# iwbn/flow-supervisor

Hardware: AMD Instinct MI355X
Metric: image-pairs/s fwd+bwd, 12 GRU iters, 436x1024 (higher is better)
Workload: dtype f32 (bf16x3 products); 1 GPU; RAFT full, 440x1024 (Sintel 436x1024 padded), 12 GRU iters, 4 pairs/GPU, train step = fwd + sequence loss + bwd + RCCL all-reduce + clip + AdamW; global_batch=4, parallelism=dp1, launch=hipGraph replay of the whole step

## Files before the change

### flow_supervisor_amd/_lib.py

```python
import ctypes
import functools
import os
from ctypes import POINTER, Structure, c_double, c_float, c_int, c_int64, c_void_p

import torch

_HERE = os.path.dirname(os.path.abspath(__file__))
LIB_PATH = os.environ.get("FSRAFT_LIB_PATH") or os.path.join(_HERE, "libfsraft.so")
_lib = None

c_float_p = c_void_p


class ConvDesc(Structure):
    _fields_ = [
        ("src", c_void_p * 3), ("srcC", c_int * 3), ("srcld", c_int * 3), ("nsrc", c_int),
        ("wpk", c_void_p), ("bias", c_void_p), ("wpk_split", c_void_p),
        ("B", c_int), ("H", c_int), ("W", c_int), ("KH", c_int), ("KW", c_int), ("N", c_int),
        ("dst", c_void_p * 3), ("dst_bs", c_int64 * 3), ("dst_ps", c_int64 * 3), ("dst_cs", c_int64 * 3),
        ("dst_n0", c_int * 3), ("dst_acc", c_int * 3), ("ndst", c_int),
        ("relu", c_int), ("alpha", c_float),
        ("epi", c_int),
        ("h", c_void_p), ("ldh", c_int), ("z", c_void_p), ("ldz", c_int),
        ("aux1", c_void_p), ("ld1", c_int), ("aux2", c_void_p), ("ld2", c_int), ("hid", c_int),
        ("pre", c_void_p), ("ldpre", c_int),
        ("rmask", c_void_p * 3), ("ldmask", c_int * 3), ("maskc", c_int * 3),
        ("wpk_frag", c_void_p), ("pad_h1", c_int), ("pad_w1", c_int),
        ("ws", c_void_p), ("ws_floats", c_int64),
    ]


class PackJob(Structure):
    _fields_ = [
        ("w", c_void_p * 3), ("rows", c_int * 3), ("npiece", c_int),
        ("wpk", c_void_p),
        ("cin_full", c_int), ("kh", c_int), ("kw", c_int),
        ("srcC", c_int * 3), ("srcOff", c_int * 3), ("nsrc", c_int),
        ("mode", c_int), ("flags", c_int),
        ("scale", c_float), ("accumulate", c_int),
    ]


_PP = POINTER(c_void_p)
_IP = POINTER(c_int)
_S = c_void_p

SIGNATURES = {
    "fsraft_corr_build": [c_void_p, c_void_p, _PP, c_int, c_int, c_int, c_int, c_int, _S],
    "fsraft_corr_unpool_bwd": [_PP, c_int, c_int, c_int, c_int, _S],
    "fsraft_corr_lookup_fwd": [_PP, c_int, c_void_p, c_int64, c_int64, c_int64, c_void_p, c_int, c_int, c_int, c_int, c_int, _S],
    "fsraft_corr_lookup_bwd": [_PP, c_int, c_void_p, c_int64, c_int64, c_int64, c_void_p, c_int, c_int, c_int, c_int, c_int, _S],
    "fsraft_altcorr_fwd": [c_void_p, c_void_p, c_void_p, c_void_p, c_int, c_int, c_int, c_int, c_int, c_int, c_int, c_int, _S],
    "fsraft_altcorr_bwd": [c_void_p, c_void_p, c_void_p, c_void_p, c_void_p, c_void_p, c_int, c_int, c_int, c_int, c_int, c_int, c_int, c_int, _S],
    "fsraft_upsample_fwd": [c_void_p, c_int64, c_int64, c_int64, c_void_p, c_void_p, c_int, c_int, c_int, _S],
    "fsraft_upsample_bwd": [c_void_p, c_int64, c_int64, c_int64, c_void_p, c_void_p, c_void_p, c_void_p, c_void_p, c_int, c_int, c_int, _S],
    "fsraft_upflow8_fwd": [c_void_p, c_void_p, c_int, c_int, c_int, c_int, _S],
    "fsraft_upflow8_bwd": [c_void_p, c_void_p, c_int, c_int, c_int, c_int, _S],
    "fsraft_conv_ktot": [_IP, c_int, c_int, c_int],
    "fsraft_conv_forward": [POINTER(ConvDesc), _S],
    "fsraft_conv_forward_stats": [POINTER(ConvDesc), c_void_p, c_void_p, c_int, POINTER(c_int), _S],
    "fsraft_conv_wgrad": [c_void_p, c_int, c_int, _PP, _IP, _IP, c_int, c_void_p, c_void_p, c_int, c_int, c_int, c_int, c_int, _S],
    "fsraft_conv_wgrad_multi": [_PP, c_int, c_int, c_int, _PP, _IP, _IP, c_int, c_void_p, c_void_p, c_int, c_int, c_int, c_int, c_int, _S],
    "fsraft_conv_small_fwd": [c_void_p, c_int, c_int, c_void_p, c_void_p, c_void_p, c_int64, c_int64, c_int64, c_int, c_int, c_int, c_int, c_int, c_int, _S],
    "fsraft_conv_small_wgrad": [_PP, _PP, c_int, c_int, c_int, c_int, c_void_p, c_void_p, c_int, c_int, c_int, c_int, c_int, c_int, _S],
    "fsraft_conv_small_dgrad": [c_void_p, c_int, c_void_p, c_void_p, c_int, c_void_p, c_int, c_int, c_int, c_int, c_int, c_int, c_int, c_int, _S],
    "fsraft_pack_conv_weights": [POINTER(PackJob), c_int, _S],
    "fsraft_pack_conv_weight": [c_void_p, c_void_p, c_int, c_int, c_int, c_int, _IP, c_int, c_int, c_int, _S],
    "fsraft_set_rec_mfma16": [c_int],
    "fsraft_set_build_kernel": [c_int],
    "fsraft_set_dvol_policy": [c_int],
    "fsraft_set_dvol_box": [c_int],
    "fsraft_set_ktile_exact": [c_int],
    "fsraft_set_lookup_policy": [c_int],
    "fsraft_set_upsample_kernel": [c_int],
    "fsraft_conv_workspace": [c_void_p, c_int64],
    "fsraft_set_arithmetic": [c_int],
    "fsraft_get_arithmetic": [],
    "fsraft_set_tuning": [c_int, c_int],
    "fsraft_adamw_flat": [c_void_p, c_void_p, c_void_p, c_void_p, c_int64, c_void_p, c_void_p, c_float, c_void_p, c_double, c_double, c_float,
                          c_float, c_void_p, c_void_p, _S],
    "fsraft_stream_capture_id": [_S, c_void_p],
    "fsraft_stem_slots": [],
    "fsraft_stem7x7s2_fwd": [c_void_p, c_void_p, c_void_p, c_void_p, c_int, c_int, c_int, c_int, _S],
    "fsraft_stem7x7s2_wgrad": [c_void_p, c_void_p, c_void_p, c_void_p, c_int, c_int, c_int, c_int, _S],
    "fsraft_set_lookup_qb": [c_int],
    "fsraft_set_build_split": [c_int],
    "fsraft_set_gemm_split": [c_int],
    "fsraft_gemm_tn_split": [c_void_p, c_int64, c_int64, c_void_p, c_int64, c_int64, c_void_p, c_int64, c_int64, c_int, c_int, c_int, c_int, c_float, c_int, _S],
    "fsraft_gemm_f32": [c_void_p, c_int64, c_int64, c_void_p, c_int64, c_int64, c_void_p, c_int64, c_int64, c_int, c_int, c_int, c_int, c_int, c_float, c_int, _S],
    "fsraft_nchw_to_nhwc": [c_void_p, c_void_p, c_int, c_int, c_int, c_int, c_int, c_int, _S],
    "fsraft_nhwc_to_nchw": [c_void_p, c_void_p, c_int, c_int, c_int, c_int, c_int, c_int, _S],
    "fsraft_im2col7": [c_void_p, c_int64, c_int64, c_int64, c_void_p, c_int, c_int, c_int, c_int, _S],
    "fsraft_col2im7": [c_void_p, c_int, c_void_p, c_int, c_int, c_int, c_int, _S],
    "fsraft_flow_to_nhwc": [c_void_p, c_int64, c_int64, c_int64, c_void_p, c_int, c_int, c_int, c_int, _S],
    "fsraft_nhwc_to_flow": [c_void_p, c_int, c_int, c_void_p, c_int, c_int, c_int, _S],
    "fsraft_relu_bwd": [c_void_p, c_int, c_void_p, c_int, c_int64, c_int, _S],
    "fsraft_gru_bwd1": [c_void_p, c_void_p, c_void_p, c_void_p, c_void_p, c_void_p, c_int, c_void_p, c_void_p, c_void_p, c_void_p, c_int64, c_int, _S],
    "fsraft_gru_bwd2": [c_void_p, c_void_p, c_void_p, c_void_p, c_int, c_void_p, c_void_p, c_int64, c_int, _S],
    "fsraft_col_sum": [c_void_p, c_int, c_int64, c_int, c_void_p, c_float, _S],
    "fsraft_softmax_rows": [c_void_p, c_int64, c_int, _S],
    "fsraft_softmax_rows_bwd": [c_void_p, c_void_p, c_int64, c_int, _S],
    "fsraft_softmax_rows_rec": [c_void_p, c_int64, c_int, _S],
    "fsraft_softmax_rows_bwd_rec": [c_void_p, c_void_p, c_int64, c_int, _S],
    "fsraft_softmax_rows_pos": [c_void_p, c_void_p, c_int64, c_int64, c_int, c_int, c_int, c_int, c_int, _S],
    "fsraft_softmax_rows_pos_bwd": [c_void_p, c_void_p, c_void_p, c_int64, c_int64, c_int, c_int, c_int, c_int, _S],
    "fsraft_gma_mix_fwd": [c_void_p, c_int, c_void_p, c_int, c_void_p, c_void_p, c_int, c_int64, c_int, _S],
    "fsraft_gma_mix_bwd": [c_void_p, c_int, c_void_p, c_int, c_void_p, c_void_p, c_int, c_void_p, c_int, c_void_p, c_int64, c_int, _S],
    "fsraft_inorm_relu_fwd": [c_void_p, c_void_p, c_void_p, c_int64, c_int, c_float, c_int, _S],
    "fsraft_inorm_relu_bwd": [c_void_p, c_void_p, c_void_p, c_void_p, c_int64, c_int, c_int, _S],
    "fsraft_affine_relu_fwd": [c_void_p, c_void_p, c_void_p, c_void_p, c_int64, c_int, c_int, c_int, _S],
    "fsraft_affine_relu_bwd": [c_void_p, c_void_p, c_void_p, c_void_p, c_void_p, c_void_p, c_void_p, c_int64, c_int, c_int, c_int, _S],
    "fsraft_sequence_loss": [_PP, _PP, POINTER(c_float), c_int, c_int, c_void_p, c_void_p, c_float, c_float, c_int, c_int, c_int, c_void_p, _S],
    "fsraft_corr_pool_pyramid": [_PP, c_int, c_int64, c_int, c_int, _S],
    "fsraft_corr_pool_pyramid_same": [_PP, c_int, c_int64, c_int, c_int, _S],
    "fsraft_corr_lookup_fwd_same": [_PP, c_int, c_void_p, c_int64, c_int64, c_int64, c_void_p, c_int, c_int, c_int, c_int, c_int, _S],
    "fsraft_corr_unpool_same_bwd": [_PP, c_int, c_int64, c_int, c_int, _S],
    "fsraft_corr_lookup_bwd_same": [_PP, c_int, c_void_p, c_int64, c_int64, c_int64, c_void_p, c_int, c_int, c_int, c_int, c_int, _S],
    "fsraft_corr_lookup_dcoords_same": [_PP, c_int, c_void_p, c_int64, c_int64, c_int64, c_void_p, c_int, c_void_p, c_int64, c_int64, c_int64,
                                        c_int, c_int, c_int, c_int, _S],
    "fsraft_set_norm_blocks": [c_int],
    "fsraft_get_tuning": [c_int],
    "fsraft_conv_last_route": [c_int],
    "fsraft_set_wgrad_wide": [c_int],
    "fsraft_conv_wgrad_last_tile": [],
    "fsraft_space_to_depth2": [c_void_p, c_void_p, c_int, c_int, c_int, c_int, c_int, _S],
    "fsraft_forward_interpolate": [c_void_p, c_void_p, c_int, c_int, _S],
    "fsraft_flow_metrics_scratch_bytes": [c_int, c_int, c_int],
    "fsraft_flow_metrics": [c_void_p, c_int64, c_int64, c_int64, c_void_p, c_int64, c_int64, c_int64, c_void_p, c_int64, c_int64,
                            c_int, c_int, c_int, c_void_p, c_void_p, c_void_p, c_int64, _S],
    "fsraft_inorm_relu_cl_fwd": [c_void_p, c_void_p, c_void_p, c_void_p, c_void_p, c_void_p, c_int, c_int, c_int, c_float, c_int, c_int, c_int, _S],
    "fsraft_inorm_relu_cl_bwd": [c_void_p, c_void_p, c_void_p, c_void_p, c_void_p, c_void_p, c_void_p, c_void_p, c_int, c_int, c_int,
                                 c_int, c_int, _S],
    "fsraft_affine_relu_cl_fwd": [c_void_p, c_void_p, c_void_p, c_void_p, c_void_p, c_int64, c_int, c_int, c_int, c_int, _S],
    "fsraft_affine_relu_cl_bwd": [c_void_p, c_void_p, c_void_p, c_void_p, c_void_p, c_void_p, c_void_p, c_void_p, c_void_p, c_int, c_int,
                                  c_int, c_int, c_int, _S],
    "fsraft_axpby": [c_void_p, c_void_p, c_float, c_float, c_int64, _S],
    "fsraft_sum_n": [_PP, c_int, c_void_p, c_int64, c_int, _S],
    "fsraft_bn_fold": [c_void_p, c_void_p, c_void_p, c_void_p, c_void_p, c_float, c_int, c_void_p, c_void_p, c_void_p, c_void_p, _S],
    "fsraft_bn_fold_bwd": [c_void_p, c_int, c_int, c_void_p, c_void_p, c_void_p, c_void_p, c_void_p, c_void_p, _S],
    "fsraft_vol_layout": [c_int, c_int, c_int, _IP],
    "fsraft_corr_build_tiled": [c_void_p, c_void_p, c_void_p, c_int, c_int, c_int, c_int, c_int, _S],
    "fsraft_corr_build_rec": [c_void_p, c_void_p, c_void_p, c_int, c_int, c_int, c_int, c_int, _S],
    "fsraft_corr_lookup_tiled_fwd": [c_void_p, c_int, c_void_p, c_int64, c_int64, c_int64, c_void_p, c_int, c_int, c_int, c_int, c_int, _S],
    "fsraft_corr_lookup_tiled_dcoords": [c_void_p, c_int, c_void_p, c_int64, c_int64, c_int64, c_void_p, c_void_p, c_int64, c_int64, c_int64,
                                         c_int, c_int, c_int, c_int, c_int, _S],
    "fsraft_corr_lookup_dcoords": [_PP, c_int, c_void_p, c_int64, c_int64, c_int64, c_void_p, c_int, c_void_p, c_int64, c_int64, c_int64,
                                   c_int, c_int, c_int, c_int, _S],
    "fsraft_corr_dvol_build": [_PP, _PP, POINTER(c_int64), c_int, c_void_p, c_int, c_int, c_int, c_int, c_int, c_int, c_int, c_int, c_int64,
                               c_int64, c_void_p, c_void_p, _S],
    "fsraft_set_alt_tile": [c_int],
    "fsraft_altcorr_fused_fwd": [c_void_p, _PP, c_int, c_void_p, c_int64, c_int64, c_int64, c_int, c_void_p, c_int, c_int, c_int, c_int, c_int, _S],
    "fsraft_altcorr_fused_dcoords": [c_void_p, _PP, c_int, c_void_p, c_int64, c_int64, c_int64, c_int, c_void_p, c_void_p, c_int64, c_int64,
                                     c_int64, c_int, c_int, c_int, c_int, c_int, _S],
    "fsraft_altcorr_mfma_fwd": [c_void_p, _PP, c_void_p, _PP, c_int, c_void_p, c_int64, c_int64, c_int64, c_int, c_void_p, c_int, c_int, c_int, c_int, c_int, _S],
    "fsraft_corr_f2cat": [c_void_p, c_void_p, c_int, c_int, c_int, c_int, c_int, _S],
    "fsraft_corr_dfmap2": [c_void_p, c_void_p, c_int, c_int, c_int, c_int, c_int, _S],
    "fsraft_corr_f2cat_rec": [c_void_p, c_void_p, c_int, c_int, c_int, c_int, c_int, _S],
    "fsraft_to_records": [c_void_p, c_int64, c_void_p, c_int64, c_int64, c_int, _S],
    "fsraft_gemm_rec_tn": [c_void_p, c_int64, c_int64, c_void_p, c_int64, c_int64, c_void_p, c_int64, c_int64, c_int, c_int, c_int, c_int,
                           c_float, c_int, c_int, _S],
    "fsraft_gemm_rec_nt": [c_void_p, c_int64, c_int64, c_void_p, c_int64, c_int64, c_void_p, c_int64, c_int64, c_int, c_int, c_int, c_int,
                           c_float, c_int, c_int, _S],
    "fsraft_gemm_rec_nt_list": [c_void_p, c_int64, c_int64, c_void_p, c_int64, c_int64, c_void_p, c_int64, c_int64, c_int, c_int, c_int, c_int,
                                c_float, c_int, c_int, c_void_p, c_void_p, c_int, c_int, _S],
    "fsraft_gemm_rec_tn_list": [c_void_p, c_int64, c_int64, c_void_p, c_int64, c_int64, c_void_p, c_int64, c_int64, c_int, c_int, c_int, c_int,
                                c_float, c_int, c_int, c_void_p, c_void_p, c_int, c_int, _S],
    "fsraft_corr_bwd_ktiles": [_PP, POINTER(c_int64), c_int, c_int, c_int, c_int, c_int, c_int, c_int, c_int64, c_int64, c_void_p, c_void_p,
                               c_int, c_void_p, c_void_p, c_void_p, c_int, c_void_p, _S],
}

CONV_ROUTES = {
    1: ("fwd.gemm32", "fp32"), 2: ("fwd.gemm64", "fp32"), 3: ("fwd.gemm64x128", "fp32"), 4: ("fwd.gemm128", "fp32"),
    5: ("fwd.gemm64x64", "fp32"), 6: ("fwd.gemm64x64k16", "fp32"), 7: ("fwd.gemm64x128k16", "fp32"),
    10: ("fwd.patch128x128", "bf16x3"), 11: ("fwd.patch256x128", "bf16x3"), 12: ("fwd.patch128x64", "bf16x3"),
    13: ("fwd.patch256x64", "bf16x3"), 20: ("fwd.halo21", "bf16x3"), 21: ("fwd.halo22", "bf16x3"),
    30: ("fwd.split64x256", "bf16x3"), 31: ("fwd.split256x64", "bf16x3"), 32: ("fwd.split256x128w16", "bf16x3"),
    33: ("fwd.split128x128w8", "bf16x3"), 34: ("fwd.split64x128", "bf16x3"), 35: ("fwd.split128x128", "bf16x3"),
}
CONV_ROUTES.update({c + 100: (n + "+ksplit", a) for c, (n, a) in list(CONV_ROUTES.items()) if c >= 30})
WGRAD_ROUTES = {
    1: ("wgrad.exact32", "fp32"), 2: ("wgrad.exact64x64", "fp32"), 3: ("wgrad.exact128", "fp32"),
    4: ("wgrad.split128", "bf16x3"), 5: ("wgrad.split128S", "bf16x3"), 6: ("wgrad.pack", "bf16x3"),
    7: ("wgrad.patch", "bf16x3"), 8: ("wgrad.multi", "bf16x3"), 9: ("wgrad.multi_w8", "bf16x3"),
}


def load():
    global _lib
    if _lib is not None:
        return _lib
    if not os.path.exists(LIB_PATH):
        raise RuntimeError(
            f"{LIB_PATH} not found: build it with `python -c 'import __graft_entry__ as g; g.build()'` "
            "(or `make -C flow_supervisor_amd/csrc`). There is no CPU/eager fallback for the RAFT hot path.")
    lib = ctypes.CDLL(LIB_PATH)
    for name, argtypes in SIGNATURES.items():
        fn = getattr(lib, name)
        fn.argtypes = argtypes
        fn.restype = c_int
    _lib = lib
    arith = os.environ.get("FSRAFT_ARITHMETIC")
    if arith is not None:
        lib.fsraft_set_arithmetic(int(arith))
    split = os.environ.get("FSRAFT_CONV_SPLIT")
    if split is not None:
        lib.fsraft_set_tuning(3, int(split))
    bsplit = os.environ.get("FSRAFT_BUILD_SPLIT")
    if bsplit is not None:
        lib.fsraft_set_build_split(int(bsplit))
    for kv in filter(None, os.environ.get("FSRAFT_TUNING", "").split(",")):
        key, val = (int(v) for v in kv.split("="))
        if lib.fsraft_set_tuning(key, val) != 0:
            raise RuntimeError(f"FSRAFT_TUNING: key {key} is not a tuning key of this libfsraft (include/fsraft_tuning.h)")
    wsplit = os.environ.get("FSRAFT_WGRAD_SPLIT")
    if wsplit is not None:
        lib.fsraft_set_tuning(4, int(wsplit))
    return lib


def stream():
    return c_void_p(torch.cuda.current_stream().cuda_stream)


def check(rc, what):
    if rc != 0:
        raise RuntimeError(f"libfsraft: {what} failed with status {rc} "
                           f"({'bad argument' if rc == 1 else 'kernel launch error'})")


def ptr(t):
    return c_void_p(t.data_ptr()) if t is not None else c_void_p(0)


def ptr_array(tensors):
    arr = (c_void_p * len(tensors))(*[t.data_ptr() for t in tensors])
    return ctypes.cast(arr, _PP), arr


def int_array(vals):
    return (c_int * len(vals))(*vals)


def require_cuda_f32(*tensors):
    dev = None
    for t in tensors:
        if t is None:
            continue
        if not t.is_cuda:
            raise RuntimeError("fsraft ops need CUDA (ROCm) tensors; the hot path has no CPU implementation")
        if t.dtype != torch.float32:
            raise RuntimeError(f"fsraft ops are fp32-only, got {t.dtype}")
        if dev is None:
            dev = t.device
        elif t.device != dev:
            raise RuntimeError(f"fsraft ops need all tensors on one device, got {dev} and {t.device}")
    if dev is not None and dev.index != torch.cuda.current_device():
        raise RuntimeError(f"fsraft op called with tensors on {dev} while cuda:{torch.cuda.current_device()} is the current device; "
                           f"wrap the call in `with torch.cuda.device({dev.index}):`")


def _first_cuda_device(values):
    for v in values:
        if isinstance(v, torch.Tensor):
            if v.is_cuda:
                return v.device
        elif isinstance(v, (list, tuple)):
            d = _first_cuda_device(v)
            if d is not None:
                return d
    return None


def on_tensor_device(fn):
    @functools.wraps(fn)
    def guarded(*args, **kwargs):
        dev = _first_cuda_device(args)
        if dev is None and kwargs:
# ... 7 lines not shown
```

### flow_supervisor_amd/core/extractor.py

```python
import torch
import torch.nn as nn
import torch.nn.functional as F

from .. import ops
from .._lib import on_tensor_device


class _InstNormRelu(torch.autograd.Function):

    @staticmethod
    def forward(ctx, x, eps, relu):
        from .. import _lib as L
        x = x.contiguous()
        N, C, H, W = x.shape
        y = torch.empty_like(x)
        stats = torch.empty(N * C, 2, device=x.device, dtype=torch.float32)
        L.check(L.load().fsraft_inorm_relu_fwd(L.ptr(x), L.ptr(y), L.ptr(stats), N * C, H * W, float(eps), int(relu),
                                               L.stream()), "inorm_relu_fwd")
        ctx.save_for_backward(x, stats)
        ctx.relu = relu
        return y

    @staticmethod
    def backward(ctx, g):
# ... 81 lines not shown
    @staticmethod
    def backward(ctx, g):
        return _as_cl(g)


class _ResLink:
    __slots__ = ("dres", "armed")

    def __init__(self):
        self.dres = None
        self.armed = False


class _InstNormReluCL(torch.autograd.Function):

    @staticmethod
    def forward(ctx, x, eps, relu, res=None, link=None, sums=None, s2d=False):
        from .. import _lib as L
        ctx.in_cl = _is_cl(x)
        ctx.link = link
        x = _as_cl(x)
        N, C, H, W = x.shape
        if res is not None:
            res = _as_cl(res)
        ctx.s2w = W if s2d else 0
        y = (torch.empty(N, H // 2, W // 2, 4 * C, device=x.device, dtype=torch.float32).permute(0, 3, 1, 2) if s2d
             else torch.empty_like(x))
        have = sums is not None and sums.acc is not None and tuple(sums.acc.shape) == (2, N * 8, C)
        acc = sums.acc if have else ops.zeros(2, N * 8, C, device=x.device)
        stats = torch.empty(N, C, 2, device=x.device, dtype=torch.float32)
        L.check(L.load().fsraft_inorm_relu_cl_fwd(L.ptr(x), L.ptr(res), L.ptr(y), L.ptr(acc[0]), L.ptr(acc[1]), L.ptr(stats), N, H * W,
                                                  C, float(eps), int(relu), int(have), ctx.s2w, L.stream()), "inorm_relu_cl_fwd")
        ctx.fused = res is not None
        ctx.save_for_backward(x, stats, y if ctx.fused else None)
        ctx.relu = relu
        return y

    @staticmethod
    def backward(ctx, g):
        from .. import _lib as L
        x, stats, out = ctx.saved_tensors
        N, C, H, W = x.shape
        g = _as_cl(g)
        dx = torch.empty_like(x)
        dres = torch.empty_like(x) if ctx.fused else None
        acc = ops.zeros(2, N * 8, C, device=x.device)
        L.check(L.load().fsraft_inorm_relu_cl_bwd(L.ptr(g), L.ptr(x), L.ptr(stats), L.ptr(out), L.ptr(acc[0]), L.ptr(acc[1]), L.ptr(dx),
                                                  L.ptr(dres), N, H * W, C, int(ctx.relu), ctx.s2w, L.stream()), "inorm_relu_cl_bwd")
        if ctx.link is not None and ctx.link.armed:
            ctx.link.dres, dres = dres, None
        return dx if ctx.in_cl else _as_nchw(dx), None, None, dres, None, None, None


class _FrozenBNReluCL(torch.autograd.Function):

    @staticmethod
    def forward(ctx, x, cbias, weight, bias, rm, rv, eps, relu, res=None, link=None, s2d=False):
        from .. import _lib as L
        ctx.in_cl = _is_cl(x)
        ctx.link = link
        x = _as_cl(x)
        N, C, H, W = x.shape
        ctx.s2w = W if s2d else 0
        if res is not None:
            res = _as_cl(res)
        fold = torch.empty(4, C, device=x.device, dtype=torch.float32)
        scale, shift, rs, rmc = fold[0], fold[1], fold[2], fold[3]
        L.check(L.load().fsraft_bn_fold(L.ptr(weight.detach().float().contiguous()), L.ptr(bias.detach().float().contiguous()),
                                        L.ptr(rm.float().contiguous()), L.ptr(rv.float().contiguous()),
                                        L.ptr(cbias.detach().float().contiguous()) if cbias is not None else None, float(eps), C,
                                        L.ptr(scale), L.ptr(shift), L.ptr(rs), L.ptr(rmc), L.stream()), "bn_fold")
        y = torch.empty(N, H // 2, W // 2, 4 * C, device=x.device, dtype=torch.float32).permute(0, 3, 1, 2) if s2d else torch.empty_like(x)
        L.check(L.load().fsraft_affine_relu_cl_fwd(L.ptr(x), L.ptr(res), L.ptr(scale), L.ptr(shift), L.ptr(y), N * H * W, C, int(relu),
                                                   H * W, ctx.s2w, L.stream()), "affine_relu_cl_fwd")
        ctx.fused = res is not None
        ctx.save_for_backward(x, scale, shift, rs, rmc, y if ctx.fused else None)
        ctx.relu = relu
        ctx.has_cbias = cbias is not None
        return y

    @staticmethod
    def backward(ctx, g):
        from .. import _lib as L
        x, scale, shift, rs, rm, out = ctx.saved_tensors
        N, C, H, W = x.shape
        g = _as_cl(g)
        dx = torch.empty_like(x)
        dres = torch.empty_like(x) if ctx.fused else None
        part = ops.zeros(2, N * 8, C, device=x.device)
        L.check(L.load().fsraft_affine_relu_cl_bwd(L.ptr(g), L.ptr(x), L.ptr(scale), L.ptr(shift), L.ptr(out), L.ptr(dx), L.ptr(dres),
                                                   L.ptr(part[0]), L.ptr(part[1]), N, H * W, C, int(ctx.relu), ctx.s2w, L.stream()),
                "affine_relu_cl_bwd")
        dpar = torch.empty(3, C, device=x.device, dtype=torch.float32)
        L.check(L.load().fsraft_bn_fold_bwd(L.ptr(part), N * 8, C, L.ptr(rs), L.ptr(rm), L.ptr(scale), L.ptr(dpar[0]), L.ptr(dpar[1]),
                                            L.ptr(dpar[2]) if ctx.has_cbias else None, L.stream()), "bn_fold_bwd")
        if ctx.link is not None and ctx.link.armed:
            ctx.link.dres, dres = dres, None
        return (dx if ctx.in_cl else _as_nchw(dx), dpar[2] if ctx.has_cbias else None, dpar[0], dpar[1], None, None, None, None, dres,
                None, None)


def _conv_key(conv):
    from .. import ops
    w = conv.weight
    return (w.data_ptr(), w._version, ops.exact_mode())


def _queue_conv_packs(plan, conv):
    from .. import ops
    wd = conv.weight.detach()
    N, C, KH, KW = wd.shape
    exact = ops.exact_mode()
    fs = plan.pack([wd], [C], 10)
    f = plan.pack([wd], [C], 0) if (exact or N <= 32) else fs
    ds = plan.pack([wd], [C], 11)
    d = plan.pack([wd], [C], 1) if (exact or C <= 32) else ds
    ff = plan.pack([wd], [C], 10, frag=True) if (KH, KW) == (3, 3) and 32 < C <= 64 else None
    df = plan.pack([wd], [C], 11, frag=True) if (KH, KW) == (3, 3) and 32 < N <= 64 else None
    return (f, fs, d, ds, ff, df)


def _prepare_packs(root):
    from .. import ops
    todo = []
    for m in root.modules():
        if isinstance(m, _Block) and _pair_shape_ok(m):
            w3, wsc = m.conv1.weight, m.downsample[0].weight
            key = (w3.data_ptr(), w3._version, wsc.data_ptr(), wsc._version, ops.exact_mode())
            c = m.__dict__.get("_fs_pair_packs")
            if (c is None or c[0] != key) and w3.is_cuda and w3.dtype == torch.float32:
                todo.append(("pair", m, key))
        if (isinstance(m, nn.Conv2d) and m.stride == (1, 1) and m.kernel_size in ((1, 1), (3, 3)) and m.groups == 1
                and m.weight.is_cuda and m.weight.dtype == torch.float32):
            c = m.__dict__.get("_fs_packs")
            key = _conv_key(m)
            if c is None or c[0] != key:
                todo.append(("conv", m, key))
    if not todo:
        return
    with torch.no_grad():
        plan = ops.PackPlan(todo[0][1].conv1.weight.device if todo[0][0] == "pair" else todo[0][1].weight.device)
        hs = []
        exact = ops.exact_mode()
        for kind, m, key in todo:
            if kind == "conv":
                hs.append(_queue_conv_packs(plan, m))
                continue
            w3, ws = m.conv1.weight.detach(), m.downsample[0].weight.detach()
            N, C = w3.shape[:2]
            a = plan.pack([w3], [4 * C], 10, cin_full=C, s2d=True)
            b = plan.pack([w3], [4 * C], 11, cin_full=C, s2d=True)
            a0 = plan.pack([w3], [4 * C], 0, cin_full=C, s2d=True) if (exact or N <= 32) else a
            b0 = plan.pack([w3], [4 * C], 1, cin_full=C, s2d=True) if (exact or 4 * C <= 32) else b
            Ns, Cs = ws.shape[:2]
            c_ = plan.pack([ws], [Cs], 10)
            d_ = plan.pack([ws], [Cs], 11)
            c0 = plan.pack([ws], [Cs], 0) if (exact or Ns <= 32) else c_
            d0 = plan.pack([ws], [Cs], 1) if (exact or Cs <= 32) else d_
            hs.append(((a0, a, b0, b), (c0, c_, d0, d_)))
        out = plan.run()
        for (kind, m, key), h in zip(todo, hs):
            if kind == "conv":
                m.__dict__["_fs_packs"] = (key,) + tuple(None if i is None else out[i] for i in h)
            else:
                m.__dict__["_fs_pair_packs"] = (key, tuple(out[i] for i in h[0]), tuple(out[i] for i in h[1]))


def _weight_packs(conv):
    c = conv.__dict__.get("_fs_packs")
    if c is None or c[0] != _conv_key(conv):
        _prepare_packs(conv)
        c = conv.__dict__["_fs_packs"]
    return c


class _ConvCL(torch.autograd.Function):

    @staticmethod
    def forward(ctx, x, weight, bias, packs, link=None, sums=None):
        from .. import ops
        ctx.link = link if _is_cl(x) else None
        if ctx.link is not None:
            ctx.link.armed = True
        x = _as_cl(x)
        B, C, H, W = x.shape
        N, _, KH, KW = weight.shape
        out = torch.empty(B, H, W, N, device=x.device, dtype=torch.float32)
        acc = ops.zeros(2, B * 8, N, device=x.device) if (sums is not None and bias is None and STATS_IN_EPILOGUE) else None
        carried = ops.conv_forward([ops.V(x.permute(0, 2, 3, 1), C)], packs[1], bias, B, H, W, KH, KW, N, [ops.Dst.nhwc(out)],
                                   wpk_split=packs[2], wpk_frag=packs[5], stats=acc)
        if sums is not None:
            sums.acc = acc if carried else None
        ctx.save_for_backward(x, weight)
        ctx.packs = packs
        ctx.has_bias = bias is not None
        return out.permute(0, 3, 1, 2)

    @staticmethod
    def backward(ctx, g):
        from .. import ops
        x, weight = ctx.saved_tensors
        B, C, H, W = x.shape
        N, _, KH, KW = weight.shape
        g = _as_cl(g)
        gv = ops.V(g.permute(0, 2, 3, 1), N)
        dx = dw = db = None
        if ctx.needs_input_grad[0]:
            dres = ctx.link.dres if ctx.link is not None else None
            if dres is not None and dres.shape == x.shape and _is_cl(dres) and dres.dtype == torch.float32:
                ctx.link.dres = None
                ops.conv_forward([gv], ctx.packs[3], None, B, H, W, KH, KW, C, [ops.Dst.nhwc(dres.permute(0, 2, 3, 1), acc=True)],
                                 wpk_split=ctx.packs[4], wpk_frag=ctx.packs[6])
                dx = dres
            else:
                if dres is not None:
                    ctx.link.dres = None
                dxb = torch.empty(B, H, W, C, device=x.device, dtype=torch.float32)
                ops.conv_forward([gv], ctx.packs[3], None, B, H, W, KH, KW, C, [ops.Dst.nhwc(dxb)], wpk_split=ctx.packs[4],
                                 wpk_frag=ctx.packs[6])
                dx = dxb.permute(0, 3, 1, 2)
                if dres is not None:
                    dx = dx + dres
        elif ctx.link is not None:
            ctx.link.dres = None
        want_b = ctx.has_bias and ctx.needs_input_grad[2]
        if ctx.needs_input_grad[1] or want_b:
            dwpk = ops.zeros(N, ops.conv_ktot([C], KH, KW), device=x.device)
            db = ops.zeros(N, device=x.device) if want_b else None
            ops.conv_wgrad(gv, [ops.V(x.permute(0, 2, 3, 1), C)], dwpk, B, H, W, KH, KW, dbias=db)
            dw = ops.unpack_weight_grad(dwpk, tuple(weight.shape), [C])
        return dx, dw, db, None, None, None


class _StemFn(torch.autograd.Function):

    @staticmethod
    def forward(ctx, x, w):
        from .. import ops
        x = x.contiguous()
        ctx.save_for_backward(x)
        return ops.stem_fwd(x, w.detach()).permute(0, 3, 1, 2)

    @staticmethod
    def backward(ctx, g):
        from .. import ops
        (x,) = ctx.saved_tensors
        return None, ops.stem_wgrad(x, _as_cl(g).permute(0, 2, 3, 1))


def _stem_ok(conv, x):
    import os
    return (STEM_KERNEL and conv.kernel_size == (7, 7) and conv.stride == (2, 2) and conv.padding == (3, 3)
            and conv.dilation == (1, 1) and conv.groups == 1 and conv.padding_mode == "zeros" and conv.in_channels == 3
            and conv.out_channels in (32, 64) and _fast(x) and not x.requires_grad and not torch.is_autocast_enabled()
            and x.shape[2] >= 7 and x.shape[3] >= 7)


STATS_IN_EPILOGUE = True
STEM_KERNEL = True
S2D_UNITS = True


class _NormSums:
    __slots__ = ("acc",)

    def __init__(self):
        self.acc = None


def _conv(conv, x, bias, link=None, stem_cl=False, sums=None):
    k = conv.kernel_size
    if (_is_cl(x) and x.is_cuda and x.dtype == torch.float32 and k in ((3, 3), (1, 1)) and conv.stride == (1, 1)
            and conv.padding == (k[0] // 2, k[1] // 2) and conv.dilation == (1, 1) and conv.groups == 1
            and conv.padding_mode == "zeros" and x.shape[1] % 4 == 0 and not torch.is_autocast_enabled()):
        return _ConvCL.apply(x, conv.weight, bias, _weight_packs(conv), link, sums)
    if stem_cl and bias is None and _stem_ok(conv, x):
        return _StemFn.apply(x, conv.weight)
    return F.conv2d(_ToNCHW.apply(x) if _is_cl(x) else x, conv.weight, bias, conv.stride, conv.padding, conv.dilation, conv.groups)


_S2D_TAP = ((0, 1), (1, 0), (1, 1))


def _s2d_weight(w3):
    N, C = w3.shape[:2]
    w = w3.new_zeros(N, 2, 2, C, 2, 2)
    for ky, (ty, sy) in enumerate(_S2D_TAP):
        for kx, (tx, sx) in enumerate(_S2D_TAP):
            w[:, sy, sx, :, ty, tx] = w3[:, :, ky, kx]
    return w.reshape(N, 4 * C, 2, 2)


def _s2d_weight_grad(dw, C):
    N = dw.shape[0]
    d = dw.reshape(N, 2, 2, C, 2, 2)
    out = dw.new_empty(N, C, 3, 3)
    for ky, (ty, sy) in enumerate(_S2D_TAP):
        for kx, (tx, sx) in enumerate(_S2D_TAP):
            out[:, :, ky, kx] = d[:, sy, sx, :, ty, tx]
    return out


def _pair_shape_ok(block):
    c1 = getattr(block, "conv1", None)
    ds = block.downsample[0] if getattr(block, "downsample", None) is not None else None
    return (block.n == 2 and c1 is not None and ds is not None and c1.kernel_size == (3, 3) and c1.stride == (2, 2)
            and c1.padding == (1, 1) and c1.dilation == (1, 1) and c1.groups == 1 and ds.kernel_size == (1, 1)
            and ds.stride == (2, 2) and ds.padding == (0, 0) and ds.groups == 1)


def _pair_packs(block):
    from .. import ops
    w3, wsc = block.conv1.weight, block.downsample[0].weight
    key = (w3.data_ptr(), w3._version, wsc.data_ptr(), wsc._version, ops.exact_mode())
    c = block.__dict__.get("_fs_pair_packs")
    if c is None or c[0] != key:
        _prepare_packs(block)
        c = block.__dict__["_fs_pair_packs"]
    return c


class _StridedPairFn(torch.autograd.Function):

    @staticmethod
    def forward(ctx, x, w3, wsc, packs, pre=False):
        from .. import ops
        x = _as_cl(x)
        ctx.pre = pre
        if pre:
            B, C4, h, w = x.shape
            C, H, W = C4 // 4, 2 * h, 2 * w
            xs = x.permute(0, 2, 3, 1)
        else:
            B, C, H, W = x.shape
            h, w = H // 2, W // 2
            xs = ops.space_to_depth2(x.permute(0, 2, 3, 1))
        N, Ns = w3.shape[0], wsc.shape[0]
        y1 = torch.empty(B, h, w, N, device=x.device, dtype=torch.float32)
        ys = torch.empty(B, h, w, Ns, device=x.device, dtype=torch.float32)
        p, q = packs[1], packs[2]
        ops.conv_forward([ops.V(xs, 4 * C)], p[0], None, B, h, w, 2, 2, N, [ops.Dst.nhwc(y1)], wpk_split=p[1])
        ops.conv_forward([ops.V(xs, C, 0)], q[0], None, B, h, w, 1, 1, Ns, [ops.Dst.nhwc(ys)], wpk_split=q[1])
        ctx.save_for_backward(xs, w3, wsc)
        ctx.packs = packs
        return y1.permute(0, 3, 1, 2), ys.permute(0, 3, 1, 2)

    @staticmethod
    def backward(ctx, g1, gs):
        from .. import ops
        xs, w3, wsc = ctx.saved_tensors
        B, h, w, C4 = xs.shape
        C, N, Ns = C4 // 4, w3.shape[0], wsc.shape[0]
        p, q = ctx.packs[1], ctx.packs[2]
        g1v = ops.V(_as_cl(g1).permute(0, 2, 3, 1), N)
        gsv = ops.V(_as_cl(gs).permute(0, 2, 3, 1), Ns)
        dx = dw3 = dwsc = None
        if ctx.needs_input_grad[0]:
            dxs = torch.empty(B, h, w, C4, device=xs.device, dtype=torch.float32)
            ops.conv_forward([g1v], p[2], None, B, h, w, 2, 2, C4, [ops.Dst.nhwc(dxs)], wpk_split=p[3], pad=(0, 0))
            ops.conv_forward([gsv], q[2], None, B, h, w, 1, 1, C, [ops.Dst.nhwc(dxs, 0, 0, True)], wpk_split=q[3])
            dx = (dxs if ctx.pre else ops.space_to_depth2(dxs, inverse=True)).permute(0, 3, 1, 2)
        items = []
        if ctx.needs_input_grad[1]:
            dwpk = ops.zeros(N, ops.conv_ktot([C4], 2, 2), device=xs.device)
            ops.conv_wgrad(g1v, [ops.V(xs, C4)], dwpk, B, h, w, 2, 2)
            dw3 = torch.empty(N, C, 3, 3, device=xs.device, dtype=torch.float32)
            items.append((dwpk, [dw3], [C4], [0], C, 2, 2, 1.0, True))
        if ctx.needs_input_grad[2]:
            dwpk = ops.zeros(Ns, ops.conv_ktot([C], 1, 1), device=xs.device)
            ops.conv_wgrad(gsv, [ops.V(xs, C, 0)], dwpk, B, h, w, 1, 1)
            dwsc = torch.empty(Ns, C, 1, 1, device=xs.device, dtype=torch.float32)
            items.append((dwpk, [dwsc], [C], [0], C, 1, 1, 1.0, False))
        ops.unpack_weight_grads(items, xs.device)
        return dx, dw3, dwsc, None, None


def _norm_act(norm, y, cbias, relu, res=None):
    if isinstance(norm, nn.InstanceNorm2d):
        return _InstNormReluCL.apply(y, norm.eps, relu, res)
    return _FrozenBNReluCL.apply(y, cbias, norm.weight, norm.bias, norm.running_mean, norm.running_var, norm.eps, relu, res)


def _pair_ok_shape(block, C, H, W):
    import os
    return (S2D_UNITS and _pair_shape_ok(block) and H % 2 == 0
            and W % 2 == 0 and C % 4 == 0 and _cl_norm_ok(torch.empty(0, block.conv1.out_channels)))


def _pair_ok(block, x):
    return _pair_ok_shape(block, x.shape[1], x.shape[2], x.shape[3])


S2D_EMIT = True


class _S2D:
    __slots__ = ("t",)

    def __init__(self, t):
        self.t = t


def _conv_norm(conv, norm, x, relu, to_cl=False, res=None, link=None, res_link=None, s2d=False):
    fused = x.is_cuda and x.dtype == torch.float32 and not torch.is_autocast_enabled()
    if isinstance(norm, nn.InstanceNorm2d) and not norm.affine and not norm.track_running_stats:
        if fused:
            sums = _NormSums() if (to_cl or _is_cl(x)) else None
            y = _conv(conv, x, None, link, stem_cl=to_cl, sums=sums)
            if (to_cl or _is_cl(x)) and _cl_norm_ok(y):
                return _InstNormReluCL.apply(y, norm.eps, relu, res, res_link, sums, s2d)
            assert not s2d
            y = _InstNormRelu.apply(y, norm.eps, relu)
            return y if res is None else F.relu(res + y)
        y = F.conv2d(x, conv.weight, None, conv.stride, conv.padding, conv.dilation, conv.groups) if conv.bias is not None else conv(x)
        y = norm(y)
    elif isinstance(norm, nn.BatchNorm2d) and not norm.training and norm.track_running_stats and norm.affine and fused:
        y = _conv(conv, x, None, link, stem_cl=to_cl)
        if (to_cl or _is_cl(x)) and _cl_norm_ok(y):
            return _FrozenBNReluCL.apply(y, conv.bias, norm.weight, norm.bias, norm.running_mean, norm.running_var, norm.eps, relu, res,
                                         res_link, s2d)
        assert not s2d
        y = _FrozenBNRelu.apply(y, conv.bias, norm.weight, norm.bias, norm.running_mean, norm.running_var, norm.eps, relu)
        return y if res is None else F.relu(res + y)
    else:
        y = norm(conv(x))
    assert not s2d, "space-to-depth output is a feature of the fused channels_last norm kernels"
    y = F.relu(y, inplace=True) if relu else y
    return y if res is None else F.relu(res + y)


def _make_norm(kind, ch, groups):
    if kind == "group":
        return nn.GroupNorm(num_groups=groups, num_channels=ch)
    if kind == "batch":
        return nn.BatchNorm2d(ch)
    if kind == "instance":
        return nn.InstanceNorm2d(ch)
    if kind == "none":
        return nn.Sequential()
    raise ValueError(kind)


class _Block(nn.Module):

    def __init__(self, cin, cout, norm_fn, stride, bottleneck):
        super().__init__()
        mid = cout // 4
        if bottleneck:
            spec = [(cin, mid, 1, 1), (mid, mid, 3, stride), (mid, cout, 1, 1)]
        else:
            spec = [(cin, cout, 3, stride), (cout, cout, 3, 1)]
        groups = cout // 8
        self.n = len(spec)
        for i, (a, b, k, s) in enumerate(spec, 1):
            setattr(self, f"conv{i}", nn.Conv2d(a, b, kernel_size=k, padding=k // 2, stride=s))
        for i, (a, b, k, s) in enumerate(spec, 1):
            setattr(self, f"norm{i}", _make_norm(norm_fn, b, groups))
        self.relu = nn.ReLU(inplace=True)
        self.downsample = None
        if stride != 1:
            short = _make_norm(norm_fn, cout, groups)
            setattr(self, f"norm{self.n + 1}", short)
            self.downsample = nn.Sequential(nn.Conv2d(cin, cout, kernel_size=1, stride=stride), short)

    def forward(self, x, emit_for=None):
        if isinstance(x, _S2D):
            y1, ys = _StridedPairFn.apply(x.t, self.conv1.weight, self.downsample[0].weight, _pair_packs(self), True)
            y = _norm_act(self.norm1, y1, self.conv1.bias, True)
            xs = _norm_act(self.downsample[1], ys, self.downsample[0].bias, False)
            return _conv_norm(self.conv2, self.norm2, y, True, to_cl=True, res=xs)
        cl = _is_cl(x)
        if cl and self.downsample is not None and _pair_ok(self, x):
            y1, ys = _StridedPairFn.apply(x, self.conv1.weight, self.downsample[0].weight, _pair_packs(self))
            y = _norm_act(self.norm1, y1, self.conv1.bias, True)
            xs = _norm_act(self.downsample[1], ys, self.downsample[0].bias, False)
            return _conv_norm(self.conv2, self.norm2, y, True, to_cl=True, res=xs)
        if cl and self.downsample is not None:
            x = _ToNCHW.apply(x)
        y = x
        link = _ResLink() if (cl and self.downsample is None and self.n >= 2 and torch.is_grad_enabled() and x.requires_grad) else None
        if self.downsample is not None:
            x = _conv_norm(self.downsample[0], self.downsample[1], x, False, to_cl=cl)
        for i in range(1, self.n):
            y = _conv_norm(getattr(self, f"conv{i}"), getattr(self, f"norm{i}"), y, True, to_cl=cl, link=link if i == 1 else None)
        last = getattr(self, f"conv{self.n}")
        emit = bool(cl and S2D_EMIT and emit_for is not None and self.downsample is None and _is_cl(y) and _cl_norm_ok(torch.empty(0, last.out_channels))
                    and _pair_ok_shape(emit_for, last.out_channels, y.shape[2], y.shape[3])
                    and isinstance(getattr(self, f"norm{self.n}"), (nn.InstanceNorm2d, nn.BatchNorm2d)))
        out = _conv_norm(last, getattr(self, f"norm{self.n}"), y, True, to_cl=cl, res=x, res_link=link, s2d=emit)
        return _S2D(out) if emit else out


class ResidualBlock(_Block):
    def __init__(self, in_planes, planes, norm_fn="group", stride=1):
# ... 88 lines not shown
```

### flow_supervisor_amd/csrc/conv_common.hpp

```cpp
#pragma once
#include "gemm_core.hpp"
#include "gemm_core_split.hpp"
#include "gemm_rec.hpp"
#include <cstddef>
#include <type_traits>

struct ConvKnobs {
  int conv_tile = 0;
  int wgrad_tile = 0;
  int wgrad_blocks = 512;
  int conv_split = 1;
  int wgrad_split = 2;
  int conv_buf = 1;
  int xcd_swizzle = 0;
  int wgrad_buf = 1;
  int conv_n256 = 0;
  int wgrad_multi = 1;
  int wgrad_blocks_multi = 2048;
  int conv_uniform = 1;
  int conv_w8 = 1;
  int conv_w8_min = 64;
  int wgrad_w8 = 0;
  int wgrad_pack = 1;
  int wgrad_blocks_pack = 1024;
  int conv_n64 = 1;
  int conv_n64_min_m = 65536;
  int conv_halo = 1;
  int conv_halo_min_m = 65536;
  int wgrad_xcd = 1;
  int conv_patch = 1;
  int wgrad_patch = 1;
  int conv_patch64 = 1;
  int wgrad_patch1 = 8192;
  int conv_patch_min_m = 8192;
  int conv_ksplit = -1;
};
__attribute__((visibility("hidden"))) extern ConvKnobs knob;
__attribute__((visibility("hidden"))) extern __thread int t_route[2];

namespace {
struct Src { const float* p; int C; int ld; };
struct Dst { float* p; int64_t bs, ps, cs; int n0; int accumulate; };

struct ConvArgs {
  Src src[3]; int nsrc;
  const float* wpk; int Ktot;
  const float* bias;
  int B, H, W, KH, KW, N;
  int PH, PW;
  Dst dst[3]; int ndst;
  int relu; float alpha;
  const float* h; int ldh;
  const float* z; int ldz;
  float* aux1; int ld1;
  float* aux2; int ld2;
  int hid;
  const float* pre; int ldpre;
  const float* rmask[3]; int ldmask[3]; int maskc[3];
  float* st_sum; float* st_sq; int st_slots;
  int swz;
  int ksplit;
};

constexpr int KTAB_MAX = 512;
struct ConvArgsT {
  ConvArgs a;
  const float* ubase; int uld;
  unsigned ktab[KTAB_MAX];
};

enum { EPI_PLAIN = 0, EPI_ZR = 2, EPI_Q = 3 };

#define FS_RSRC_FLAGS 0x00020000
#define FS_OOB 0x80000000u

__device__ __forceinline__ unsigned uni(unsigned v) { return __builtin_amdgcn_readfirstlane(v); }
template <class T>
__device__ __forceinline__ const T* uni_ptr(const T* p) {
  const uint64_t u = reinterpret_cast<uint64_t>(p);
  return reinterpret_cast<const T*>((uint64_t)uni((unsigned)(u >> 32)) << 32 | uni((unsigned)u));
}
__device__ __forceinline__ __amdgpu_buffer_rsrc_t make_rsrc(const void* p, unsigned bytes) {
  const uint64_t u = reinterpret_cast<uint64_t>(p);
  const unsigned lo = __builtin_amdgcn_readfirstlane((unsigned)u), hi = __builtin_amdgcn_readfirstlane((unsigned)(u >> 32));
  void* q = reinterpret_cast<void*>((uint64_t)hi << 32 | lo);
  return __builtin_amdgcn_make_buffer_rsrc(q, 0, __builtin_amdgcn_readfirstlane(bytes), FS_RSRC_FLAGS);
}

using SWCfg128 = SplitTnCfg<128, 128, 2, 2, 2>;
using SWCfg128S = SplitTnCfg<128, 128, 2, 2, 1>;
using SWCfg128W8 = SplitTnCfg<128, 128, 2, 4, 1, 512>;
using SWCfgPack = SplitTnCfg<64, 192, 2, 2, 1>;
using SWCfgW256 = SplitTnCfg<256, 256, 2, 4, 2, 512>;
using SWCfgW128 = SplitTnCfg<128, 256, 2, 4, 2, 512>;
using Cfg128 = GemmCfg<128, 128, 32, 2, 2, 2, 2>;
using Cfg64 = GemmCfg<128, 64, 32, 4, 1, 2, 2>;
using CfgM64 = GemmCfg<64, 128, 32, 1, 4, 2, 2>;
using Cfg6464 = GemmCfg<64, 64, 32, 2, 2, 2, 2>;
using WCfg6464 = GemmCfg<64, 64, 32, 2, 2, 0, 0>;
using Cfg6464K16 = GemmCfg<64, 64, 16, 2, 2, 2, 2>;
using CfgM64K16 = GemmCfg<64, 128, 16, 1, 4, 2, 2>;

using SCfg128 = SplitCfg<128, 128, 2, 2>;
using SCfgN256 = SplitCfg<64, 256, 1, 4, 2, true>;
using SCfg256W16 = SplitCfg<256, 128, 4, 4, 2, true, 1024>;
using SCfg128W8 = SplitCfg<128, 128, 2, 4, 2, true, 512>;
using SCfg256N64 = SplitCfg<256, 64, 4, 2, 2, true, 512>;
using SCfgM64 = SplitCfg<64, 128, 1, 4, 2, true>;
using Cfg32 = GemmCfg<128, 32, 32, 4, 1, 2, 2>;
using WCfg128 = GemmCfg<128, 128, 32, 2, 2, 0, 0>;
using WCfg32 = GemmCfg<32, 128, 32, 1, 4, 0, 0>;

template <class Cfg>
constexpr int route_gemm() {
  return std::is_same_v<Cfg, Cfg32> ? 1 : std::is_same_v<Cfg, Cfg64> ? 2 : std::is_same_v<Cfg, CfgM64> ? 3 :
         std::is_same_v<Cfg, Cfg128> ? 4 : std::is_same_v<Cfg, Cfg6464> ? 5 : std::is_same_v<Cfg, Cfg6464K16> ? 6 :
         std::is_same_v<Cfg, CfgM64K16> ? 7 : 0;
}
template <class Cfg>
constexpr int route_split() {
  return std::is_same_v<Cfg, SCfgN256> ? 30 : std::is_same_v<Cfg, SCfg256N64> ? 31 : std::is_same_v<Cfg, SCfg256W16> ? 32 :
         std::is_same_v<Cfg, SCfg128W8> ? 33 : std::is_same_v<Cfg, SCfgM64> ? 34 : std::is_same_v<Cfg, SCfg128> ? 35 : 0;
}

int conv_ktot(const int* C, int nsrc, int taps) {
  int k = 0;
  for (int s = 0; s < nsrc; ++s) k += taps * (((C[s] + 31) / 32) * 32);
  return k;
}

template <class F>
void with_epi(int epi, F&& f) {
  if (epi == EPI_PLAIN) f(std::integral_constant<int, EPI_PLAIN>{});
  else if (epi == EPI_ZR) f(std::integral_constant<int, EPI_ZR>{});
  else f(std::integral_constant<int, EPI_Q>{});
}

bool fill_srcs(Src (&dst)[3], const float* const* p, const int* C, const int* ld, int nsrc) {
  for (int s = 0; s < 3; ++s) {
    dst[s] = Src{s < nsrc ? p[s] : p[0], s < nsrc ? C[s] : 0, s < nsrc ? ld[s] : 4};
    if (s < nsrc && (!p[s] || ld[s] % 4 != 0)) return false;
  }
  return true;
}

int64_t wgrad_chunk(int target, int64_t tiles, int64_t M, int words) {
  int64_t want = (target + tiles - 1) / tiles;
  if (want < 1) want = 1;
  int64_t chunk = (M + want - 1) / want;
  if (chunk < 256) chunk = 256;
  if (chunk > 32 * (words - 2)) chunk = 32 * (words - 2);
  return (chunk + 31) / 32 * 32;
}

}
```

### flow_supervisor_amd/csrc/conv_igemm.hip

```cpp
#include "conv_common.hpp"

namespace {

__device__ __forceinline__ void tile_of_block(int swz, int& bx, int& by) {
  if (!swz) return;
  const int nx = gridDim.x, T = nx * gridDim.y, i = by * nx + bx;
  const int x = i & 7, q = T >> 3, r = T & 7;
  const int t = x * q + (x < r ? x : r) + (i >> 3);
  bx = t % nx; by = t / nx;
}

template <class Cfg>
struct ConvALoader {
  static constexpr int BM = Cfg::BM, BK = Cfg::BK, LD = Cfg::LDA;
  static constexpr int F4 = BK / 4;
  static constexpr int NF4 = BM * F4 / 256;
  static constexpr int NREG = NF4 * 4;
  static constexpr int NCH = NF4;
  const float* p0; const float* p1; const float* p2;
  int C0, C1, C2, ld0, ld1, ld2;
  int cpt0, cpt1, cpt2;
  int taps, KW, PH, PW, H, W;
  int py[NF4], px[NF4];
  int64_t pb[NF4];
// ... 138 lines not shown
  int64_t row_bytes;
  int rows_valid;
  __device__ __forceinline__ void fetch_chunk(int kt, float (&r)[NREG], int j) const {
    const int e = threadIdx.x + 256 * j;
    const int row = e >> 3, part = e & 7;
    const char* src = (row < rows_valid && kt >= 0) ? base + row * row_bytes + (int64_t)kt * 128 + part * 16
                                                    : reinterpret_cast<const char*>(g_fsraft_zero16);
    const f32x4 v = gload4(src);
    r[4 * j + 0] = v[0]; r[4 * j + 1] = v[1]; r[4 * j + 2] = v[2]; r[4 * j + 3] = v[3];
  }
  __device__ __forceinline__ void stage_chunk(char* tile, const float* r4, int j) const {
    stage_copy<Cfg::PITCH>(tile, threadIdx.x + 256 * j, r4);
  }
};

template <class Cfg, int EPI>
__device__ __forceinline__ void conv_epilogue(const ConvArgs& a, f32x16 (&acc)[Cfg::TM][Cfg::TN], int m0, int n0) {
  const int HW = a.H * a.W;
  const int M = a.B * HW;
  const int lane = threadIdx.x & 63, wave = threadIdx.x >> 6;
#pragma unroll
  for (int nt = 0; nt < Cfg::TN; ++nt) {
    const int n = n0 + acc_col<Cfg>(nt);
    const bool nok = n < a.N;
    const float bias = (nok && a.bias) ? a.bias[n] : 0.f;
    int di = 0;
    if (a.ndst > 1 && n >= a.dst[1].n0) di = 1;
    if (a.ndst > 2 && n >= a.dst[2].n0) di = 2;
    float* dp = di == 0 ? a.dst[0].p : di == 1 ? a.dst[1].p : a.dst[2].p;
    const int64_t dbs = di == 0 ? a.dst[0].bs : di == 1 ? a.dst[1].bs : a.dst[2].bs;
    const int64_t dps = di == 0 ? a.dst[0].ps : di == 1 ? a.dst[1].ps : a.dst[2].ps;
    const int64_t dcs = di == 0 ? a.dst[0].cs : di == 1 ? a.dst[1].cs : a.dst[2].cs;
    const int dn0 = di == 0 ? a.dst[0].n0 : di == 1 ? a.dst[1].n0 : a.dst[2].n0;
    const bool dacc = (di == 0 ? a.dst[0].accumulate : di == 1 ? a.dst[1].accumulate : a.dst[2].accumulate) != 0;
    const float* mk = di == 0 ? a.rmask[0] : di == 1 ? a.rmask[1] : a.rmask[2];
    const int ldm = di == 0 ? a.ldmask[0] : di == 1 ? a.ldmask[1] : a.ldmask[2];
    const int mkc = di == 0 ? a.maskc[0] : di == 1 ? a.maskc[1] : a.maskc[2];
#pragma unroll
    for (int mt = 0; mt < Cfg::TM; ++mt) {
      const int mbase = m0 + (wave / Cfg::WN) * (Cfg::TM * 32) + mt * 32 + 4 * (lane >> 5);
      const int b0 = mbase / HW, pix0 = mbase - b0 * HW;
      if (EPI == EPI_PLAIN) {
#pragma unroll
        for (int hb = 0; hb < 2; ++hb) {
          int off[8];
#pragma unroll
          for (int q = 0; q < 8; ++q) {
            const int r = hb * 8 + q;
            const int d = (r & 3) + 8 * (r >> 2);
            int pix = pix0 + d, b = b0;
            if (pix >= HW) { pix -= HW; ++b; }
            const bool ok = nok && (mbase + d < M);
            off[q] = ok ? (int)(b * dbs + pix * dps + (n - dn0) * dcs) : -1;
          }
          float old[8];
#pragma unroll
          for (int q = 0; q < 8; ++q) old[q] = (dacc && off[q] >= 0) ? dp[off[q]] : 0.f;
#pragma unroll
          for (int q = 0; q < 8; ++q) {
            float v = (acc[mt][nt][hb * 8 + q] + bias) * a.alpha;
            if (a.relu) v = fmaxf(v, 0.f);
            v += old[q];
            if (off[q] >= 0 && mk && n - dn0 < mkc) {
              const int r = hb * 8 + q;
              const int64_t m = mbase + (r & 3) + 8 * (r >> 2);
              if (mk[m * ldm + (n - dn0)] <= 0.f) v = 0.f;
            }
            if (off[q] >= 0) dp[off[q]] = v;
          }
        }
      } else if (EPI == EPI_ZR) {
        const bool isz = n < a.hid;
        const int c = isz ? n : n - a.hid;
        float hh[16];
        bool ok[16];
#pragma unroll
        for (int r = 0; r < 16; ++r) {
          const int m = mbase + (r & 3) + 8 * (r >> 2);
          ok[r] = nok && m < M;
          hh[r] = (ok[r] && !isz) ? a.h[(int64_t)m * a.ldh + c] : 0.f;
        }
#pragma unroll
        for (int r = 0; r < 16; ++r) {
          const int64_t m = mbase + (r & 3) + 8 * (r >> 2);
          const float pre = (a.pre && ok[r]) ? a.pre[m * a.ldpre + n] : 0.f;
          const float sg = 1.0f / (1.0f + expf(-(acc[mt][nt][r] + bias + pre)));
          if (ok[r]) {
            if (isz) {
              a.dst[0].p[m * a.dst[0].ps + c] = sg;
            } else {
              a.aux2[m * a.ld2 + c] = sg;
              a.aux1[m * a.ld1 + c] = sg * hh[r];
            }
          }
        }
      } else {
        float hh[16], zz[16];
        bool ok[16];
#pragma unroll
        for (int r = 0; r < 16; ++r) {
          const int64_t m = mbase + (r & 3) + 8 * (r >> 2);
          ok[r] = nok && m < M;
          hh[r] = ok[r] ? a.h[m * a.ldh + n] : 0.f;
          zz[r] = ok[r] ? a.z[m * a.ldz + n] : 0.f;
        }
#pragma unroll
        for (int r = 0; r < 16; ++r) {
          const int64_t m = mbase + (r & 3) + 8 * (r >> 2);
          const float pre = (a.pre && ok[r]) ? a.pre[m * a.ldpre + n] : 0.f;
          const float q = tanhf(acc[mt][nt][r] + bias + pre);
          if (ok[r]) {
            a.aux1[m * a.ld1 + n] = q;
            a.dst[0].p[m * a.dst[0].ps + n] = (1.f - zz[r]) * hh[r] + zz[r] * q;
          }
        }
      }
    }
  }
}

template <class Cfg, int EPI, int NTW = Cfg::NT, bool PATCH = false>
__device__ __forceinline__ void conv_epilogue_lds(const ConvArgs& a, f32x16 (&acc)[Cfg::TM][Cfg::TN], int m0, int n0,
                                                  float* __restrict__ tile, bool owner = true, int pb = 0, int py0 = 0, int px0 = 0,
                                                  int64_t mofs = 0) {
  constexpr int LD = Cfg::BN + 4;
  const int HW = a.H * a.W;
  const int M = a.B * HW;
  const int lane = threadIdx.x & 63, wave = threadIdx.x >> 6;
  auto row_m = [&](int row) -> int64_t {
    if constexpr (PATCH) {
      const int y = py0 + (row >> 5), x = px0 + (row & 31);
      return (y < a.H && x < a.W) ? (int64_t)(pb * a.H + y) * a.W + x : -1;
    } else {
      return m0 + row < M ? (int64_t)m0 + row : -1;
    }
  };
  __syncthreads();
#pragma unroll
  for (int nt = 0; nt < Cfg::TN; ++nt) {
    const int nl = acc_col<Cfg>(nt);
    const float bias = (n0 + nl < a.N && a.bias) ? a.bias[n0 + nl] : 0.f;
#pragma unroll
    for (int mt = 0; mt < Cfg::TM; ++mt) {
      const int rbase = (wave / Cfg::WN) * (Cfg::TM * 32) + mt * 32 + 4 * (lane >> 5);
#pragma unroll
      for (int r = 0; r < 16; ++r) tile[(rbase + (r & 3) + 8 * (r >> 2)) * LD + nl] = acc[mt][nt][r] + bias;
    }
  }
  __syncthreads();
  constexpr int C4 = Cfg::BN / 4;
  constexpr int RPP = NTW / C4;
  (void)owner;
  const int c4 = threadIdx.x % C4, rsub = threadIdx.x / C4;
  const int n = n0 + c4 * 4;
  const bool stats = PATCH && EPI == EPI_PLAIN && a.st_sum != nullptr;
  if (n >= a.N && !stats) return;
  if (EPI == EPI_PLAIN) {
    f32x4 ssum = {0.f, 0.f, 0.f, 0.f}, ssq = {0.f, 0.f, 0.f, 0.f};
    if (n < a.N) {
    int di = 0;
    if (a.ndst > 1 && n >= a.dst[1].n0) di = 1;
    if (a.ndst > 2 && n >= a.dst[2].n0) di = 2;
    float* dp = di == 0 ? a.dst[0].p : di == 1 ? a.dst[1].p : a.dst[2].p;
    const int64_t dps = di == 0 ? a.dst[0].ps : di == 1 ? a.dst[1].ps : a.dst[2].ps;
    const int dn0 = di == 0 ? a.dst[0].n0 : di == 1 ? a.dst[1].n0 : a.dst[2].n0;
    const bool dacc = (di == 0 ? a.dst[0].accumulate : di == 1 ? a.dst[1].accumulate : a.dst[2].accumulate) != 0;
    const float* mk = di == 0 ? a.rmask[0] : di == 1 ? a.rmask[1] : a.rmask[2];
    const int ldm = di == 0 ? a.ldmask[0] : di == 1 ? a.ldmask[1] : a.ldmask[2];
    const int mkc = di == 0 ? a.maskc[0] : di == 1 ? a.maskc[1] : a.maskc[2];
    const int nv = a.N - n < 4 ? a.N - n : 4;
#pragma unroll 4
    for (int row = rsub; row < Cfg::BM; row += RPP) {
      const int64_t m = row_m(row);
      if (m < 0) { if (PATCH) continue; else break; }
      f32x4 v = *reinterpret_cast<const f32x4*>(tile + row * LD + c4 * 4);
      float* o = dp + (int64_t)(m + mofs) * dps + (n - dn0);
#pragma unroll
      for (int i = 0; i < 4; ++i) {
        v[i] *= a.alpha;
        if (a.relu) v[i] = fmaxf(v[i], 0.f);
      }
      if (nv == 4) {
        if (stats) { ssum += v; ssq += v * v; }
        if (dacc) {
          const f32x4 old = gload4(o);
#pragma unroll
          for (int i = 0; i < 4; ++i) v[i] += old[i];
        }
        if (mk) {
          const f32x4 y = gload4(mk + (int64_t)m * ldm + (n - dn0));
#pragma unroll
          for (int i = 0; i < 4; ++i) if (n - dn0 + i < mkc && y[i] <= 0.f) v[i] = 0.f;
        }
        gstore4(o, v);
      } else {
        for (int i = 0; i < nv; ++i) {
          float r = dacc ? gload1(o + i) + v[i] : v[i];
          if (mk && n - dn0 + i < mkc && gload1(mk + (int64_t)m * ldm + (n - dn0) + i) <= 0.f) r = 0.f;
          gstore1(o + i, r);
        }
      }
    }
    }
    if constexpr (PATCH) {
      if (stats) {
        __syncthreads();
        float* red = tile;
        *reinterpret_cast<f32x4*>(red + (rsub * Cfg::BN) + c4 * 4) = ssum;
        *reinterpret_cast<f32x4*>(red + ((RPP + rsub) * Cfg::BN) + c4 * 4) = ssq;
        __syncthreads();
        if (threadIdx.x < Cfg::BN && n0 + (int)threadIdx.x < a.N) {
          float t1 = 0.f, t2 = 0.f;
#pragma unroll 4
          for (int g = 0; g < RPP; ++g) { t1 += red[g * Cfg::BN + threadIdx.x]; t2 += red[(RPP + g) * Cfg::BN + threadIdx.x]; }
          const int64_t o = ((int64_t)pb * a.st_slots + (int)(blockIdx.y % (unsigned)a.st_slots)) * a.N + n0 + threadIdx.x;
          atomicAdd(a.st_sum + o, t1);
          atomicAdd(a.st_sq + o, t2);
        }
      }
    }
  } else if (EPI == EPI_ZR) {
    const bool isz = n < a.hid;
    const int c = isz ? n : n - a.hid;
#pragma unroll 4
    for (int row = rsub; row < Cfg::BM; row += RPP) {
      const int64_t mr = row_m(row);
      if (mr < 0 && !PATCH) break;
      const int64_t m = mr < 0 ? 0 : mr;
      f32x4 v = *reinterpret_cast<const f32x4*>(tile + row * LD + c4 * 4);
      if (a.pre) v += gload4(a.pre + m * a.ldpre + n);
      f32x4 hh = {0.f, 0.f, 0.f, 0.f};
      if (!isz) hh = gload4(a.h + m * a.ldh + c);
#pragma unroll
      for (int i = 0; i < 4; ++i) v[i] = 1.0f / (1.0f + expf(-v[i]));
      if (mr < 0) continue;
      if (isz) {
        *reinterpret_cast<f32x4*>(a.dst[0].p + m * a.dst[0].ps + c) = v;
      } else {
        *reinterpret_cast<f32x4*>(a.aux2 + m * a.ld2 + c) = v;
        f32x4 rh;
#pragma unroll
        for (int i = 0; i < 4; ++i) rh[i] = v[i] * hh[i];
        *reinterpret_cast<f32x4*>(a.aux1 + m * a.ld1 + c) = rh;
      }
    }
  } else {
#pragma unroll 4
    for (int row = rsub; row < Cfg::BM; row += RPP) {
      const int64_t m = row_m(row);
      if (m < 0) { if (PATCH) continue; else break; }
      f32x4 v = *reinterpret_cast<const f32x4*>(tile + row * LD + c4 * 4);
      if (a.pre) v += gload4(a.pre + m * a.ldpre + n);
      const f32x4 hh = gload4(a.h + m * a.ldh + n);
      const f32x4 zz = gload4(a.z + m * a.ldz + n);
      f32x4 hn;
#pragma unroll
      for (int i = 0; i < 4; ++i) {
        v[i] = tanhf(v[i]);
        hn[i] = (1.f - zz[i]) * hh[i] + zz[i] * v[i];
      }
      *reinterpret_cast<f32x4*>(a.aux1 + m * a.ld1 + n) = v;
      *reinterpret_cast<f32x4*>(a.dst[0].p + m * a.dst[0].ps + n) = hn;
    }
  }
}

__device__ __forceinline__ bool epilogue_rows_ok(const ConvArgs& a) {
  bool ok = true;
  for (int i = 0; i < a.ndst; ++i)
    ok = ok && a.dst[i].cs == 1 && (a.dst[i].ps & 3) == 0 && (a.dst[i].n0 & 3) == 0 && ((uintptr_t)a.dst[i].p & 15) == 0 &&
         a.dst[i].bs == a.dst[i].ps * (int64_t)(a.H * a.W);
  return ok;
}

bool epilogue_rows_ok_host(const ConvArgs& a) {
  bool ok = true;
  for (int i = 0; i < a.ndst; ++i)
    ok = ok && a.dst[i].cs == 1 && (a.dst[i].ps & 3) == 0 && (a.dst[i].n0 & 3) == 0 && ((uintptr_t)a.dst[i].p & 15) == 0 &&
         a.dst[i].bs == a.dst[i].ps * (int64_t)(a.H * a.W);
  return ok;
}

template <class Cfg, int EPI>
__global__ __launch_bounds__(256) void conv_igemm_kernel(ConvArgs a) {
  __shared__ __attribute__((aligned(16))) float lds[Cfg::LDS_FLOATS];
  const int HW = a.H * a.W;
  const int M = a.B * HW;
  const int n0 = blockIdx.x * Cfg::BN, m0 = blockIdx.y * Cfg::BM;
  ConvALoader<Cfg> la;
  la.p0 = a.src[0].p; la.C0 = a.src[0].C; la.ld0 = a.src[0].ld; la.cpt0 = (a.src[0].C + 31) / 32 * (32 / Cfg::BK);
  la.p1 = a.src[1].p; la.C1 = a.src[1].C; la.ld1 = a.src[1].ld; la.cpt1 = a.nsrc > 1 ? (a.src[1].C + 31) / 32 * (32 / Cfg::BK) : 0;
  la.p2 = a.src[2].p; la.C2 = a.src[2].C; la.ld2 = a.src[2].ld; la.cpt2 = a.nsrc > 2 ? (a.src[2].C + 31) / 32 * (32 / Cfg::BK) : 0;
  if (a.nsrc < 2) { la.p1 = a.src[0].p; la.C1 = 0; la.ld1 = 4; la.cpt1 = 1; }
  if (a.nsrc < 3) { la.p2 = a.src[0].p; la.C2 = 0; la.ld2 = 4; la.cpt2 = 1; }
  la.taps = a.KH * a.KW; la.KW = a.KW; la.PH = a.PH; la.PW = a.PW; la.H = a.H; la.W = a.W;
#pragma unroll
  for (int j = 0; j < ConvALoader<Cfg>::NF4; ++j) {
    const int row = (threadIdx.x + 256 * j) / ConvALoader<Cfg>::F4;
    const int m = m0 + row;
    if (m < M) {
      const int b = m / HW, pix = m % HW;
      la.py[j] = pix / a.W; la.px[j] = pix % a.W; la.pb[j] = (int64_t)b * HW;
    } else {
      la.py[j] = -1; la.px[j] = 0; la.pb[j] = 0;
    }
  }
  RowMajorTileLoader<Cfg::BN, Cfg::BK, Cfg::LDB> lb{a.wpk + (int64_t)n0 * a.Ktot, a.Ktot, a.N - n0, a.Ktot};
  f32x16 acc[Cfg::TM][Cfg::TN];
#pragma unroll
  for (int i = 0; i < Cfg::TM; ++i)
#pragma unroll
    for (int j = 0; j < Cfg::TN; ++j)
#pragma unroll
      for (int r = 0; r < 16; ++r) acc[i][j][r] = 0.f;
  gemm_mainloop<Cfg>(lds, a.Ktot / Cfg::BK, la, lb, acc);
  conv_epilogue<Cfg, EPI>(a, acc, m0, n0);
}

template <class Cfg, int EPI, int BUF = 0>
__global__ __launch_bounds__(Cfg::NT) void conv_igemm_split_kernel(const std::conditional_t<BUF != 0, ConvArgsT, ConvArgs> args) {
  static_assert(Cfg::NT == 256 || BUF != 0, "wider workgroups use the buffer-addressed loaders");
  __shared__ __attribute__((aligned(16))) char lds[Cfg::LDS_ALLOC];
  const ConvArgs& a = [&]() -> const ConvArgs& { if constexpr (BUF != 0) return args.a; else return args; }();
  const int HW = a.H * a.W;
  const int M = a.B * HW;
  int bx = blockIdx.x, by = blockIdx.y;
  tile_of_block(a.swz, bx, by);
  const int n0 = bx * Cfg::BN, m0 = by * Cfg::BM;
  f32x16 acc[Cfg::TM][Cfg::TN];
#pragma unroll
  for (int i = 0; i < Cfg::TM; ++i)
#pragma unroll
    for (int j = 0; j < Cfg::TN; ++j)
#pragma unroll
      for (int r = 0; r < 16; ++r) acc[i][j][r] = 0.f;
  if constexpr (BUF != 0) {
    const int PH = a.PH, PW = a.PW, taps = a.KH * a.KW;
    const auto* ktab = (const unsigned __attribute__((address_space(4)))*)(
        (const char __attribute__((address_space(4)))*)__builtin_amdgcn_kernarg_segment_ptr() + offsetof(ConvArgsT, ktab));
    int kt0 = 0, KTs = a.Ktot / 32;
    if (a.ksplit > 1) {
      const int per = (KTs + a.ksplit - 1) / a.ksplit;
      kt0 = (int)blockIdx.z * per;
      KTs = min(per, KTs - kt0);
      ktab += kt0 * (BUF >= 2 ? 2 : 1);
    }
    unsigned tapmask[Cfg::NCH_A], pofs[Cfg::NCH_A];
#pragma unroll
    for (int j = 0; j < Cfg::NCH_A; ++j) {
      const int m = m0 + ((threadIdx.x + Cfg::NT * j) >> 3);
      unsigned mask = 0;
      if (m < M) {
        const int pix = m % HW, y = pix / a.W, x = pix % a.W;
        for (int t = 0; t < taps; ++t) {
          const int yy = y + t / a.KW - PH, xx = x + t % a.KW - PW;
          if ((unsigned)yy < (unsigned)a.H && (unsigned)xx < (unsigned)a.W) mask |= 1u << t;
        }
      }
      tapmask[j] = mask; pofs[j] = m < M ? m : 0;
    }
    BufWeightLoader<Cfg> lb;
    lb.base = uni_ptr(reinterpret_cast<const char*>(a.wpk) + (int64_t)n0 * a.Ktot * 4 + (int64_t)kt0 * 128);
    lb.nbytes = 0x7fffffffu;
#pragma unroll
    for (int j = 0; j < BufWeightLoader<Cfg>::NCH; ++j) {
      const int e = threadIdx.x + Cfg::NT * j;
      lb.voff[j] = (e >> 3) < a.N - n0 ? (unsigned)((e >> 3) * a.Ktot * 4 + (e & 7) * 16) : FS_OOB;
    }
    if constexpr (BUF >= 2) {
      BufConvALoaderU<Cfg> la;
      la.base = uni_ptr(args.ubase); la.ktab = ktab; la.kq16 = (threadIdx.x & 7) * 16;
      const unsigned ldb = uni((unsigned)args.uld * 4u);
#pragma unroll
      for (int j = 0; j < Cfg::NCH_A; ++j) { la.tapmask[j] = tapmask[j]; la.voff0[j] = pofs[j] * ldb + la.kq16; }
      split_mainloop<Cfg, BufConvALoaderU<Cfg>, BufWeightLoader<Cfg>, true>(lds, KTs, la, lb, acc);
    } else {
      BufConvALoader<Cfg> la;
      la.ld0x4 = uni(a.src[0].ld * 4); la.ld1x4 = uni(a.src[1].ld * 4); la.ld2x4 = uni(a.src[2].ld * 4);
      la.b0 = uni_ptr(a.src[0].p - (int64_t)(PH * a.W + PW) * a.src[0].ld); la.nb0 = 0x7fffffffu;
      la.b1 = uni_ptr(a.src[1].p - (int64_t)(PH * a.W + PW) * a.src[1].ld); la.nb1 = 0x7fffffffu;
      la.b2 = uni_ptr(a.src[2].p - (int64_t)(PH * a.W + PW) * a.src[2].ld); la.nb2 = 0x7fffffffu;
      la.ktab = ktab;
      la.kq16 = (threadIdx.x & 7) * 16;
#pragma unroll
      for (int j = 0; j < Cfg::NCH_A; ++j) { la.tapmask[j] = tapmask[j]; la.pofs[j] = pofs[j]; }
      split_mainloop<Cfg, BufConvALoader<Cfg>, BufWeightLoader<Cfg>, true>(lds, KTs, la, lb, acc);
    }
    if constexpr (EPI == EPI_PLAIN && Cfg::LDS_ALLOC >= Cfg::BM * (Cfg::BN + 4) * 4) {
      if (a.ksplit > 1) {
        conv_epilogue_lds<Cfg, EPI_PLAIN>(a, acc, m0, n0, reinterpret_cast<float*>(lds), true, 0, 0, 0, (int64_t)blockIdx.z * M);
        return;
      }
    }
  } else {
  SplitConvALoader<Cfg> la;
  la.p0 = a.src[0].p; la.C0 = a.src[0].C; la.ld0 = a.src[0].ld; la.cpt0 = (a.src[0].C + 31) / 32;
  la.p1 = a.src[1].p; la.C1 = a.src[1].C; la.ld1 = a.src[1].ld; la.cpt1 = a.nsrc > 1 ? (a.src[1].C + 31) / 32 : 0;
  la.p2 = a.src[2].p; la.C2 = a.src[2].C; la.ld2 = a.src[2].ld; la.cpt2 = a.nsrc > 2 ? (a.src[2].C + 31) / 32 : 0;
  if (a.nsrc < 2) { la.p1 = a.src[0].p; la.C1 = 0; la.ld1 = 4; la.cpt1 = 1; }
  if (a.nsrc < 3) { la.p2 = a.src[0].p; la.C2 = 0; la.ld2 = 4; la.cpt2 = 1; }
  la.taps = a.KH * a.KW; la.KW = a.KW; la.PH = a.PH; la.PW = a.PW; la.H = a.H; la.W = a.W;
// ... 46 lines not shown
    const int ku = __builtin_amdgcn_readfirstlane(kt < KT ? kt : KT - 1);
    const __amdgpu_buffer_rsrc_t rs = make_rsrc(wbase, 0x7fffffffu);
#pragma unroll
    for (int nt = 0; nt < TN; ++nt) {
      const int nb = wn * TN + nt;
      const unsigned soff = (unsigned)((ku * NB + (nb < NB ? nb : 0)) * 4096);
      const unsigned voff = nb < NB ? (unsigned)lane * 16u : FS_OOB;
#pragma unroll
      for (int q = 0; q < 4; ++q) f.v[nt][q] = __builtin_amdgcn_raw_buffer_load_b128(rs, voff, soff + 1024u * q, 0);
    }
  };
  BFrag f[4];
  fetch_b(0, f[0]);
  fetch_b(1, f[1]);
  fetch_b(2, f[2]);

  {
    const float* img = uni_ptr(a.x + (int64_t)b * a.H * a.W * a.ldx);
    const __amdgpu_buffer_rsrc_t rs = make_rsrc(img, 0x7fffffffu);
    float rh[NCHH * 4];
#pragma unroll
    for (int j = 0; j < NCHH; ++j) {
      const int e = threadIdx.x + 256 * j;
      const int row = e / (CG * 8), rem = e % (CG * 8), ch = (rem >> 3) * 32 + (rem & 7) * 4;
      const int y = y0 - 1 + row / HALO_PW, x = x0 - 1 + row % HALO_PW;
      const bool ok = row < HALO_ROWS && (unsigned)y < (unsigned)a.H && (unsigned)x < (unsigned)a.W && ch < a.C;
      const unsigned voff = ok ? (unsigned)((y * a.W + x) * a.ldx + ch) * 4u : FS_OOB;
      const f32x4 f = __builtin_bit_cast(f32x4, __builtin_amdgcn_raw_buffer_load_b128(rs, voff, 0, 0));
      rh[4 * j + 0] = f[0]; rh[4 * j + 1] = f[1]; rh[4 * j + 2] = f[2]; rh[4 * j + 3] = f[3];
    }
#pragma unroll
    for (int j = 0; j < NCHH; ++j) {
      const int e = threadIdx.x + 256 * j;
      const int row = e / (CG * 8), rem = e % (CG * 8);
      if (row < HALO_ROWS) stage_convert<128>(lds + (rem >> 3) * PLANE, row * 8 + (rem & 7), rh + 4 * j);
    }
  }
  __syncthreads();

  f32x16 acc[2][TN];
#pragma unroll
  for (int i = 0; i < 2; ++i)
#pragma unroll
    for (int j = 0; j < TN; ++j)
#pragma unroll
      for (int r = 0; r < 16; ++r) acc[i][j][r] = 0.f;

  auto compute = [&](int kt, const BFrag& f) {
    const int ku = __builtin_amdgcn_readfirstlane(kt);
    const int tap = ku / CG, g = ku - tap * CG, dy = tap / 3, dx = tap - dy * 3;
    const char* Ap = lds + g * PLANE;
    const int rowa = (2 * wm + dy) * HALO_PW + dx + l31;
#pragma unroll
    for (int s = 0; s < 2; ++s) {
      bf16x8 ah[2], al[2];
#pragma unroll
      for (int mt = 0; mt < 2; ++mt) {
        const int row = rowa + mt * HALO_PW;
        ah[mt] = *reinterpret_cast<const bf16x8*>(Ap + slot_offset<128>(row, 2 * s + lh));
        al[mt] = *reinterpret_cast<const bf16x8*>(Ap + slot_offset<128>(row, 4 + 2 * s + lh));
      }
#pragma unroll
      for (int mt = 0; mt < 2; ++mt)
#pragma unroll
        for (int nt = 0; nt < TN; ++nt) {
          const bf16x8 bh = __builtin_bit_cast(bf16x8, f.v[nt][s]), bl = __builtin_bit_cast(bf16x8, f.v[nt][2 + s]);
          acc[mt][nt] = __builtin_amdgcn_mfma_f32_32x32x16_bf16(al[mt], bh, acc[mt][nt], 0, 0, 0);
          acc[mt][nt] = __builtin_amdgcn_mfma_f32_32x32x16_bf16(ah[mt], bl, acc[mt][nt], 0, 0, 0);
          acc[mt][nt] = __builtin_amdgcn_mfma_f32_32x32x16_bf16(ah[mt], bh, acc[mt][nt], 0, 0, 0);
        }
    }
  };
  for (int kt = 0; kt < KT; kt += 4) {
#pragma unroll
    for (int i = 0; i < 4; ++i)
      if (kt + i < KT) {
        fetch_b(kt + i + 3, f[(i + 3) & 3]);
        compute(kt + i, f[i]);
      }
  }

  if (a.st_sum) {
    __syncthreads();
    float* red = reinterpret_cast<float*>(lds);
#pragma unroll
    for (int nt = 0; nt < TN; ++nt) {
      float s1 = 0.f, s2 = 0.f;
#pragma unroll
      for (int mt = 0; mt < 2; ++mt) {
        const int py = y0 + 2 * wm + mt;
#pragma unroll
        for (int r = 0; r < 16; ++r) {
          const int px = x0 + (r & 3) + 8 * (r >> 2) + 4 * lh;
          const float v = (py < a.H && px < a.W) ? acc[mt][nt][r] : 0.f;
          s1 += v; s2 += v * v;
        }
      }
      s1 += __shfl_xor(s1, 32, 64); s2 += __shfl_xor(s2, 32, 64);
      const int col = wn * (32 * TN) + nt * 32 + l31;
      if (lh == 0) { red[(wm * 2 + 0) * (64 * TN) + col] = s1; red[(wm * 2 + 1) * (64 * TN) + col] = s2; }
    }
    __syncthreads();
    if ((int)threadIdx.x < 64 * TN && (int)threadIdx.x < a.N) {
      const int col = threadIdx.x;
      const int slot = (int)((blockIdx.y * gridDim.x + blockIdx.x) % (unsigned)a.st_slots);
      const int64_t o = ((int64_t)b * a.st_slots + slot) * a.N + col;
      atomicAdd(a.st_sum + o, red[col] + red[2 * (64 * TN) + col]);
      atomicAdd(a.st_sq + o, red[(64 * TN) + col] + red[3 * (64 * TN) + col]);
    }
  }
  float* outb = a.out + (int64_t)b * a.obs;
#pragma unroll
  for (int mt = 0; mt < 2; ++mt) {
    const int py = y0 + 2 * wm + mt;
    if (py >= a.H) continue;
#pragma unroll
    for (int nt = 0; nt < TN; ++nt) {
      const int n = wn * (32 * TN) + nt * 32 + l31;
      if (n >= a.N) continue;
      const float bv = a.bias ? a.bias[n] : 0.f;
      float old[16];
#pragma unroll
      for (int r = 0; r < 16; ++r) {
        const int px = x0 + (r & 3) + 8 * (r >> 2) + 4 * lh, pc = px < a.W ? px : a.W - 1;
        old[r] = a.acc ? outb[(int64_t)(py * a.W + pc) * a.ops + n] : 0.f;
      }
#pragma unroll
      for (int r = 0; r < 16; ++r) {
        const int px = x0 + (r & 3) + 8 * (r >> 2) + 4 * lh;
        if (px >= a.W) continue;
        float v = acc[mt][nt][r] + bv;
        if (a.relu) v = fmaxf(v, 0.f);
        outb[(int64_t)(py * a.W + px) * a.ops + n] = v + old[r];
      }
    }
  }
}

template <int CG, int TN>
int launch_halo(const HaloArgs& h, hipStream_t s) {
  dim3 grid(ceil_div(h.W, HALO_TW), ceil_div(h.H, HALO_TH), h.B);
  hipLaunchKernelGGL((conv3x3_halo_kernel<CG, TN>), grid, dim3(256), 0, s, h);
  return fs_launch_status();
}

bool build_ktab(const ConvArgs& a, ConvArgsT& t) {
  const int taps = a.KH * a.KW, KT = a.Ktot / 32;
  const int64_t M = (int64_t)a.B * a.H * a.W;
  if (KT > KTAB_MAX || taps > 15) return false;
  int kt = 0;
  for (int s = 0; s < a.nsrc; ++s) {
    const int C = a.src[s].C, ld = a.src[s].ld, cpt = (C + 31) / 32;
    if (M * ld * 4 >= (int64_t)FS_OOB) return false;
    for (int i = 0; i < taps * cpt; ++i, ++kt) {
        const int tap = i / cpt, c = i % cpt;
        const int64_t soff = ((int64_t)((tap / a.KW) * a.W + tap % a.KW) * ld + c * 32) * 4;
        if (soff % 16 != 0 || soff / 16 > 0xffff) return false;
        const int crem = C - c * 32 < 32 ? C - c * 32 : 32;
        t.ktab[kt] = (unsigned)(soff / 16) | (unsigned)tap << 16 | (unsigned)s << 20 | (unsigned)crem << 22;
      }
  }
  if (kt != KT) return false;
  t.a = a;
  return true;
}

bool build_ktab_uniform(const ConvArgs& a, ConvArgsT& t) {
  const int taps = a.KH * a.KW, KT = a.Ktot / 32, PH = a.PH, PW = a.PW;
  const int64_t M = (int64_t)a.B * a.H * a.W;
  if (!knob.conv_uniform || 2 * KT > KTAB_MAX || taps > 15) return false;
  const int ld = a.src[0].ld;
  const float* lo = a.src[0].p;
  for (int s = 0; s < a.nsrc; ++s) {
    if (a.src[s].ld != ld) return false;
    if (a.src[s].p < lo) lo = a.src[s].p;
  }
  const float* base = lo - (int64_t)(PH * a.W + PW) * ld;
  int kt = 0;
  for (int s = 0; s < a.nsrc; ++s) {
    const int C = a.src[s].C, cpt = (C + 31) / 32;
    const int64_t delta = (a.src[s].p - lo) * 4;
    for (int tap = 0; tap < taps; ++tap)
      for (int c = 0; c < cpt; ++c, ++kt) {
        const int64_t soff = delta + ((int64_t)((tap / a.KW) * a.W + tap % a.KW) * ld + c * 32) * 4;
        if (soff + M * ld * 4 + 256 >= (int64_t)FS_OOB) return false;
        const int crem = C - c * 32 < 32 ? C - c * 32 : 32;
        t.ktab[2 * kt] = (unsigned)soff;
        t.ktab[2 * kt + 1] = (unsigned)tap | (unsigned)crem << 4;
      }
  }
  if (kt != KT) return false;
  t.a = a; t.ubase = base; t.uld = ld;
  return true;
}


template <int EPI>
__global__ __launch_bounds__(256) void conv_finish_kernel(const ConvArgs a, const float* __restrict__ ws, int S, int ldw) {
  const int HW = a.H * a.W;
  const int64_t M = (int64_t)a.B * HW;
  const int C4 = (a.N + 3) / 4;
  for (int64_t e = (int64_t)blockIdx.x * 256 + threadIdx.x; e < M * C4; e += (int64_t)gridDim.x * 256) {
    const int64_t m = e / C4;
    const int n = (int)(e % C4) * 4;
    const int nv = a.N - n < 4 ? a.N - n : 4;
    f32x4 v = {0.f, 0.f, 0.f, 0.f};
    if (a.bias) {
#pragma unroll
      for (int i = 0; i < 4; ++i) v[i] = i < nv ? a.bias[n + i] : 0.f;
    }
    for (int s = 0; s < S; ++s) {
      const f32x4 p = gload4(ws + ((int64_t)s * M + m) * ldw + n);
#pragma unroll
      for (int i = 0; i < 4; ++i) v[i] += p[i];
    }
    if (EPI == EPI_PLAIN) {
      int di = 0;
      if (a.ndst > 1 && n >= a.dst[1].n0) di = 1;
      if (a.ndst > 2 && n >= a.dst[2].n0) di = 2;
      float* dp = di == 0 ? a.dst[0].p : di == 1 ? a.dst[1].p : a.dst[2].p;
      const int64_t dbs = di == 0 ? a.dst[0].bs : di == 1 ? a.dst[1].bs : a.dst[2].bs;
      const int64_t dps = di == 0 ? a.dst[0].ps : di == 1 ? a.dst[1].ps : a.dst[2].ps;
      const int64_t dcs = di == 0 ? a.dst[0].cs : di == 1 ? a.dst[1].cs : a.dst[2].cs;
      const int dn0 = di == 0 ? a.dst[0].n0 : di == 1 ? a.dst[1].n0 : a.dst[2].n0;
      const bool dacc = (di == 0 ? a.dst[0].accumulate : di == 1 ? a.dst[1].accumulate : a.dst[2].accumulate) != 0;
      const float* mk = di == 0 ? a.rmask[0] : di == 1 ? a.rmask[1] : a.rmask[2];
      const int ldm = di == 0 ? a.ldmask[0] : di == 1 ? a.ldmask[1] : a.ldmask[2];
      const int mkc = di == 0 ? a.maskc[0] : di == 1 ? a.maskc[1] : a.maskc[2];
      const int64_t b = m / HW, pix = m - b * HW;
      float* o = dp + b * dbs + pix * dps + (int64_t)(n - dn0) * dcs;
      for (int i = 0; i < nv; ++i) {
        float r = v[i] * a.alpha;
        if (a.relu) r = fmaxf(r, 0.f);
        if (dacc) r += o[i * dcs];
        if (mk && n - dn0 + i < mkc && mk[m * ldm + (n - dn0) + i] <= 0.f) r = 0.f;
        o[i * dcs] = r;
      }
    } else if (EPI == EPI_ZR) {
      const bool isz = n < a.hid;
      const int c = isz ? n : n - a.hid;
      if (a.pre) v += gload4(a.pre + m * a.ldpre + n);
#pragma unroll
      for (int i = 0; i < 4; ++i) v[i] = 1.0f / (1.0f + expf(-v[i]));
      if (isz) {
        *reinterpret_cast<f32x4*>(a.dst[0].p + m * a.dst[0].ps + c) = v;
      } else {
        const f32x4 hh = gload4(a.h + m * a.ldh + c);
        *reinterpret_cast<f32x4*>(a.aux2 + m * a.ld2 + c) = v;
        f32x4 rh;
#pragma unroll
        for (int i = 0; i < 4; ++i) rh[i] = v[i] * hh[i];
        *reinterpret_cast<f32x4*>(a.aux1 + m * a.ld1 + c) = rh;
      }
    } else {
      if (a.pre) v += gload4(a.pre + m * a.ldpre + n);
      const f32x4 hh = gload4(a.h + m * a.ldh + n);
      const f32x4 zz = gload4(a.z + m * a.ldz + n);
      f32x4 hn;
#pragma unroll
      for (int i = 0; i < 4; ++i) {
        v[i] = tanhf(v[i]);
        hn[i] = (1.f - zz[i]) * hh[i] + zz[i] * v[i];
      }
      *reinterpret_cast<f32x4*>(a.aux1 + m * a.ld1 + n) = v;
      *reinterpret_cast<f32x4*>(a.dst[0].p + m * a.dst[0].ps + n) = hn;
    }
  }
}

thread_local float* t_reg_ws = nullptr;
thread_local int64_t t_reg_ws_floats = 0;
thread_local float* g_conv_ws = nullptr;
thread_local int64_t g_conv_ws_floats = 0;

int pick_ksplit(int64_t tiles, int KT, int N, int64_t M, int ldw, int bm) {
  int S = 1;
  if (knob.conv_ksplit >= 2) S = knob.conv_ksplit;
  else if (knob.conv_ksplit == -1 && bm == 64 && tiles <= 150 && N <= 256 && KT >= 16) S = (int)((400 + tiles - 1) / tiles);
  else if (knob.conv_ksplit == -1 && bm == 128 && tiles <= 120 && N <= 256 && KT >= (N <= 128 ? 36 : 48)) S = tiles <= 115 ? (int)(230 / tiles) : 2;
  if (S > KT / 6) S = KT / 6;
  if (S > 6) S = 6;
  while (S > 1 && (int64_t)S * M * ldw > g_conv_ws_floats) --S;
  if (S > 1) {
    const int per = (KT + S - 1) / S;
    S = (KT + per - 1) / per;
  }
  return S < 2 ? 1 : S;
}

template <class Cfg>
int launch_conv_split(const ConvArgs& a, int epi, hipStream_t s) {
  const int M = a.B * a.H * a.W;
  dim3 grid(ceil_div(a.N, Cfg::BN), ceil_div(M, Cfg::BM));
  ConvArgsT t;
  const int swz = knob.xcd_swizzle || (grid.x >= 2 && (int64_t)grid.x * grid.y >= 2048);
  const bool buf = knob.conv_buf == 2 || (knob.conv_buf == 1 && Cfg::BM == 64) || Cfg::BN == 256 || Cfg::NT != 256;
  if constexpr (Cfg::LDS_ALLOC >= Cfg::BM * (Cfg::BN + 4) * 4) {
    const int ldw = (a.N + 3) / 4 * 4;
    const bool gru_ok = epi == EPI_PLAIN || (a.N % 4 == 0 && (!a.pre || a.ldpre % 4 == 0));
    const int S = (buf && g_conv_ws && gru_ok && (Cfg::BM == 64 || (Cfg::BM == 128 && Cfg::NT == 512) || knob.conv_ksplit >= 2)) ? pick_ksplit((int64_t)grid.x * grid.y, a.Ktot / 32, a.N, M, ldw, Cfg::BM) : 1;
    if (S > 1) {
      const bool uni_tab = build_ktab_uniform(a, t);
      if (uni_tab || build_ktab(a, t)) {
        ConvArgs& p = t.a;
        p.swz = 0;
        p.ksplit = S;
        p.dst[0] = Dst{g_conv_ws, (int64_t)a.H * a.W * ldw, ldw, 1, 0, 0};
        p.dst[1] = p.dst[2] = p.dst[0];
        p.ndst = 1; p.bias = nullptr; p.relu = 0; p.alpha = 1.0f;
        for (int i = 0; i < 3; ++i) p.rmask[i] = nullptr;
        dim3 g3(grid.x, grid.y, S);
        t_route[0] = route_split<Cfg>() + 100;
        if (uni_tab) hipLaunchKernelGGL((conv_igemm_split_kernel<Cfg, EPI_PLAIN, 2>), g3, dim3(Cfg::NT), 0, s, t);
        else hipLaunchKernelGGL((conv_igemm_split_kernel<Cfg, EPI_PLAIN, 1>), g3, dim3(Cfg::NT), 0, s, t);
        int rc = fs_launch_status();
        if (rc) return rc;
        const int64_t work = (int64_t)M * (ldw / 4);
        const int fb = (int)((work + 255) / 256 < 4096 ? (work + 255) / 256 : 4096);
        with_epi(epi, [&](auto e) { hipLaunchKernelGGL(conv_finish_kernel<decltype(e)::value>, dim3(fb), dim3(256), 0, s, a, g_conv_ws, S, ldw); });
        return fs_launch_status();
      }
    }
  }
  if (buf && build_ktab_uniform(a, t)) {
    t.a.swz = swz;
    t_route[0] = route_split<Cfg>();
    with_epi(epi, [&](auto e) { hipLaunchKernelGGL((conv_igemm_split_kernel<Cfg, decltype(e)::value, 2>), grid, dim3(Cfg::NT), 0, s, t); });
    return fs_launch_status();
  }
  if (buf && build_ktab(a, t)) {
    t.a.swz = swz;
    t_route[0] = route_split<Cfg>();
    with_epi(epi, [&](auto e) { hipLaunchKernelGGL((conv_igemm_split_kernel<Cfg, decltype(e)::value, 1>), grid, dim3(Cfg::NT), 0, s, t); });
    return fs_launch_status();
  }
  if constexpr (Cfg::NT != 256) {
    return -1;
  } else {
  t_route[0] = route_split<Cfg>();
  with_epi(epi, [&](auto e) { hipLaunchKernelGGL((conv_igemm_split_kernel<Cfg, decltype(e)::value>), grid, dim3(256), 0, s, a); });
  return fs_launch_status();
  }
}

template <class Cfg>
int launch_conv_split_plain(const ConvArgs& a, hipStream_t s) {
  const int M = a.B * a.H * a.W;
  dim3 grid(ceil_div(a.N, Cfg::BN), ceil_div(M, Cfg::BM));
  ConvArgsT t;
  if (build_ktab_uniform(a, t)) {
    t_route[0] = route_split<Cfg>();
    hipLaunchKernelGGL((conv_igemm_split_kernel<Cfg, EPI_PLAIN, 2>), grid, dim3(Cfg::NT), 0, s, t);
    return fs_launch_status();
  }
  if (build_ktab(a, t)) {
    t_route[0] = route_split<Cfg>();
    hipLaunchKernelGGL((conv_igemm_split_kernel<Cfg, EPI_PLAIN, 1>), grid, dim3(Cfg::NT), 0, s, t);
    return fs_launch_status();
  }
  return -1;
}

template <class Cfg>
int launch_conv(const ConvArgs& a, int epi, hipStream_t s) {
  const int M = a.B * a.H * a.W;
  dim3 grid(ceil_div(a.N, Cfg::BN), ceil_div(M, Cfg::BM));
  t_route[0] = route_gemm<Cfg>();
  with_epi(epi, [&](auto e) { hipLaunchKernelGGL((conv_igemm_kernel<Cfg, decltype(e)::value>), grid, dim3(256), 0, s, a); });
  return fs_launch_status();
}

#include "conv_patch.inc"

}

extern "C" int fsraft_conv_ktot(const int* srcC, int nsrc, int KH, int KW) {
  if (!srcC || nsrc < 1 || nsrc > 3) return -1;
  return conv_ktot(srcC, nsrc, KH * KW);
}

namespace {
struct StatReq { float* sum; float* sq; int slots; bool done; };
thread_local StatReq t_stat{nullptr, nullptr, 0, false};
template <class Args>
void attach_stats(Args& p, bool want) {
  if (want) { p.st_sum = t_stat.sum; p.st_sq = t_stat.sq; p.st_slots = t_stat.slots; }
}
}

extern "C" int fsraft_conv_forward(const fsraft_conv_desc* d, hipStream_t stream) {
  if (!d || d->nsrc < 1 || d->nsrc > 3 || d->ndst < 1 || d->ndst > 3 || !d->wpk || d->N < 1) return FS_ERR_ARG;
  const bool want_stats = t_stat.sum != nullptr && d->epi == EPI_PLAIN && d->ndst == 1 && !d->relu && d->alpha == 1.0f && !d->dst_acc[0] &&
                          !d->rmask[0] && !d->bias && d->dst_n0[0] == 0 && d->N % 4 == 0;
  if (d->ws && (((uintptr_t)d->ws & 15) || d->ws_floats < 0)) return FS_ERR_ARG;
  t_route[0] = 0;
  g_conv_ws = d->ws ? d->ws : t_reg_ws;
  g_conv_ws_floats = d->ws ? d->ws_floats : t_reg_ws_floats;
  ConvArgs a{};
  if (!fill_srcs(a.src, d->src, d->srcC, d->srcld, d->nsrc)) return FS_ERR_ARG;
  for (int s = 0; s < d->nsrc; ++s) if (d->srcC[s] < 1) return FS_ERR_ARG;
  a.nsrc = d->nsrc;
  a.wpk = d->wpk; a.Ktot = conv_ktot(d->srcC, d->nsrc, d->KH * d->KW); a.bias = d->bias;
  a.B = d->B; a.H = d->H; a.W = d->W; a.KH = d->KH; a.KW = d->KW; a.N = d->N;
  a.PH = d->pad_h1 ? d->pad_h1 - 1 : d->KH / 2; a.PW = d->pad_w1 ? d->pad_w1 - 1 : d->KW / 2;
  if (a.PH < 0 || a.PH >= d->KH || a.PW < 0 || a.PW >= d->KW) return FS_ERR_ARG;
  for (int i = 0; i < 3; ++i) {
    const int j = i < d->ndst ? i : 0;
    a.dst[i] = Dst{d->dst[j], d->dst_bs[j], d->dst_ps[j], d->dst_cs[j], d->dst_n0[j], d->dst_acc[j]};
    if (i < d->ndst && !d->dst[i]) return FS_ERR_ARG;
  }
  a.ndst = d->ndst; a.relu = d->relu; a.alpha = d->alpha;
  a.h = d->h; a.ldh = d->ldh; a.z = d->z; a.ldz = d->ldz; a.aux1 = d->aux1; a.ld1 = d->ld1; a.aux2 = d->aux2; a.ld2 = d->ld2;
  a.hid = d->hid;
  a.pre = d->epi == EPI_PLAIN ? nullptr : d->pre; a.ldpre = d->ldpre;
  if (a.pre && (d->ldpre % 4 != 0 || ((uintptr_t)d->pre & 15))) return FS_ERR_ARG;
  for (int i = 0; i < 3; ++i) {
    const bool on = d->epi == EPI_PLAIN && i < d->ndst && d->rmask[i] != nullptr;
    a.rmask[i] = on ? d->rmask[i] : nullptr; a.ldmask[i] = d->ldmask[i]; a.maskc[i] = d->maskc[i];
    if (on && (d->ldmask[i] % 4 != 0 || ((uintptr_t)d->rmask[i] & 15))) return FS_ERR_ARG;
  }
  a.swz = knob.xcd_swizzle;
  if (d->epi == EPI_ZR && (!d->h || !d->aux1 || !d->aux2 || d->hid * 2 != d->N)) return FS_ERR_ARG;
  if (d->epi == EPI_Q && (!d->h || !d->z || !d->aux1)) return FS_ERR_ARG;
  if (d->epi != EPI_PLAIN && d->epi != EPI_ZR && d->epi != EPI_Q) return FS_ERR_ARG;
  if (knob.conv_patch && knob.conv_patch64 && knob.conv_split == 1 && d->wpk_split && d->epi == EPI_PLAIN && d->KH == 3 && d->KW == 3 &&
      d->N > 32 && d->N <= 64 && (int64_t)d->B * d->H * d->W >= knob.conv_patch_min_m) {
    ConvArgs p = a;
    p.wpk = d->wpk_split;
    attach_stats(p, want_stats);
    const int rc = launch_conv_patch(p, d->epi, stream);
    if (rc >= 0) { t_stat.done = want_stats; return rc; }
  }
  if (knob.conv_halo && knob.conv_split == 1 && d->wpk_frag && d->epi == EPI_PLAIN && d->nsrc == 1 && d->KH == 3 && d->KW == 3 &&
      a.PH == 1 && a.PW == 1 &&
      d->srcC[0] % 4 == 0 && d->srcC[0] > 32 && d->srcC[0] <= 64 && d->N <= 128 && d->N > 32 && d->ndst == 1 &&
      d->dst_cs[0] == 1 && d->dst_n0[0] == 0 && !(d->dst_acc[0] && d->relu) && !a.rmask[0] && d->alpha == 1.0f &&
      (int64_t)d->B * d->H * d->W >= knob.conv_halo_min_m && (int64_t)d->H * d->W * d->srcld[0] * 4 < 0x7fffffff) {
    HaloArgs h{d->src[0], d->srcld[0], d->srcC[0], reinterpret_cast<const char*>(d->wpk_frag), d->bias,
               d->dst[0], d->dst_bs[0], d->dst_ps[0], d->N, d->B, d->H, d->W, d->relu, d->dst_acc[0], nullptr, nullptr, 0};
    attach_stats(h, want_stats);
    t_stat.done = want_stats;
    t_route[0] = d->N > 64 ? 21 : 20;
    return d->N > 64 ? launch_halo<2, 2>(h, stream) : launch_halo<2, 1>(h, stream);
  }
  if (d->N <= 32 && d->epi == EPI_PLAIN) return launch_conv<Cfg32>(a, d->epi, stream);
  if (d->N <= 64 && d->epi == EPI_PLAIN && !(knob.conv_split && d->wpk_split && knob.conv_buf)) return launch_conv<Cfg64>(a, d->epi, stream);
  const int M = d->B * d->H * d->W;
  if (knob.conv_split && d->wpk_split && d->N > 32) {
    a.wpk = d->wpk_split;
    const bool narrow = knob.conv_buf != 0 || (int64_t)ceil_div(d->N, 128) * ceil_div(M, 128) < 400;
    if (knob.conv_patch && knob.conv_split == 1 && d->KH * d->KW > 1 && d->N > 64 && M >= knob.conv_patch_min_m) {
      ConvArgs p = a;
      attach_stats(p, want_stats);
      const int rc = launch_conv_patch(p, d->epi, stream);
      if (rc >= 0) { t_stat.done = want_stats; return rc; }
    }
    if (knob.conv_split == 5 || (knob.conv_split == 1 && knob.conv_n256 && d->N >= 256 &&
                              ceil_div(d->N, 256) * 256 <= ceil_div(d->N, 128) * 128))
      return launch_conv_split<SCfgN256>(a, d->epi, stream);
    if (knob.conv_split == 1 && knob.conv_n64 && d->N <= 64 && d->epi == EPI_PLAIN && M >= knob.conv_n64_min_m) {
      const int rc = launch_conv_split_plain<SCfg256N64>(a, stream);
      if (rc >= 0) return rc;
    }
    if (knob.conv_split == 1 && ((knob.conv_w8 == 1 && d->N >= 192 && d->N <= 512 && M >= 16384) || knob.conv_w8 == 2) && d->N >= 192) {
      const int rc = launch_conv_split<SCfg256W16>(a, d->epi, stream);
      if (rc >= 0) return rc;
    }
    if (knob.conv_w8 && knob.conv_split == 1 && (int64_t)ceil_div(d->N, 128) * ceil_div(M, 128) >= knob.conv_w8_min) {
      const int rc = launch_conv_split<SCfg128W8>(a, d->epi, stream);
      if (rc >= 0) return rc;
    }
    if (knob.conv_split == 3) return launch_conv_split<SCfgM64>(a, d->epi, stream);
    if (knob.conv_split == 4) return launch_conv_split<SCfg128>(a, d->epi, stream);
    return narrow ? launch_conv_split<SCfgM64>(a, d->epi, stream) : launch_conv_split<SCfg128>(a, d->epi, stream);
  }
  if (knob.conv_tile == 3) return launch_conv<Cfg6464>(a, d->epi, stream);
  if (knob.conv_tile == 4) return launch_conv<Cfg6464K16>(a, d->epi, stream);
  if (knob.conv_tile == 5) return launch_conv<CfgM64K16>(a, d->epi, stream);
  if (knob.conv_tile == 2) return launch_conv<CfgM64>(a, d->epi, stream);
  if (knob.conv_tile == 1) return launch_conv<Cfg128>(a, d->epi, stream);
  if ((int64_t)ceil_div(d->N, 128) * ceil_div(M, 128) < 512) return launch_conv<CfgM64>(a, d->epi, stream);
  return launch_conv<Cfg128>(a, d->epi, stream);
}

extern "C" int fsraft_conv_forward_stats(const fsraft_conv_desc* d, float* sum, float* sq, int slots, int* done, hipStream_t stream) {
  if (!sum || !sq || slots < 1 || !done) return FS_ERR_ARG;
  t_stat = StatReq{sum, sq, slots, false};
  const int rc = fsraft_conv_forward(d, stream);
  *done = (rc == FS_OK && t_stat.done) ? 1 : 0;
  t_stat = StatReq{nullptr, nullptr, 0, false};
  return rc;
}


extern "C" int fsraft_conv_workspace(float* ws, int64_t floats) {
  if (ws && (((uintptr_t)ws & 15) || floats < 0)) return FS_ERR_ARG;
  t_reg_ws = ws;
  t_reg_ws_floats = ws ? floats : 0;
  return FS_OK;
}
```

### flow_supervisor_amd/csrc/conv_pack.hip

```cpp
#include "conv_common.hpp"

namespace {

struct PackArgs {
  float* w;
  float* wpk;
  int Cout, Cin, taps;
  int C[3]; int nsrc;
  int Ktot, rows;
  int mode, accumulate;
  int split;
};

__device__ __forceinline__ void store_packed(const PackArgs& a, int64_t e, float v) {
  if (!a.split) { a.wpk[e] = v; return; }
  const __bf16 h = (__bf16)v;
  const __bf16 l = (__bf16)(v - (float)h);
  __bf16* rec = reinterpret_cast<__bf16*>(a.wpk) + (e >> 5) * 64;
  rec[e & 31] = h;
  rec[32 + (e & 31)] = l;
}

__global__ __launch_bounds__(256) void pack_weight_kernel(PackArgs a) {
  const int64_t total = (int64_t)a.rows * a.Ktot;
  for (int64_t e = (int64_t)blockIdx.x * 256 + threadIdx.x; e < total; e += (int64_t)gridDim.x * 256) {
    const int n = (int)(e / a.Ktot);
    int k = (int)(e % a.Ktot);
    if (a.mode == 1) {
      const int cpad = ((a.Cout + 31) / 32) * 32;
      const int tp = k / cpad, c = k % cpad;
      float v = 0.f;
      if (c < a.Cout && n < a.Cin) v = a.w[((int64_t)c * a.Cin + n) * a.taps + (a.taps - 1 - tp)];
      store_packed(a, e, v);
    } else {
      int s = 0, coff = 0;
      for (; s < a.nsrc; ++s) {
        const int span = a.taps * (((a.C[s] + 31) / 32) * 32);
        if (k < span) break;
        k -= span; coff += a.C[s];
      }
      const int cpad = ((a.C[s] + 31) / 32) * 32;
      const int t = k / cpad, c = k % cpad;
      const bool ok = c < a.C[s] && n < a.Cout;
      if (a.mode == 0) {
        store_packed(a, e, ok ? a.w[((int64_t)n * a.Cin + coff + c) * a.taps + t] : 0.f);
      } else if (ok) {
        float* d = a.w + ((int64_t)n * a.Cin + coff + c) * a.taps + t;
        *d = a.accumulate ? *d + a.wpk[e] : a.wpk[e];
      }
    }
  }
}

using PackJob = fsraft_pack_job;
constexpr int PACK_JOBS = 16;
struct PackJobs { fsraft_pack_job j[PACK_JOBS]; };

__device__ __forceinline__ float* pack_elem(const PackJob& j, int n, int s, int c, int t) {
  int p = 0;
  while (p + 1 < j.npiece && n >= j.rows[p]) { n -= j.rows[p]; ++p; }
  float* w = j.w[p];
  if (j.flags & 2) {
    const int C = j.cin_full;
    const int sp = c / C, c0 = c % C;
    const int ky = 2 * (t >> 1) + (sp >> 1) - 1, kx = 2 * (t & 1) + (sp & 1) - 1;
    if (ky < 0 || kx < 0) return nullptr;
    return w + ((int64_t)n * C + c0) * 9 + ky * 3 + kx;
  }
  return w + ((int64_t)n * j.cin_full + j.srcOff[s] + c) * (j.kh * j.kw) + t;
}

__device__ __forceinline__ void pack_store(const PackJob& j, int Ktot, int rows, int n, int k, float v) {
  const int64_t e = (int64_t)n * Ktot + k;
  if (j.mode < 10) { j.wpk[e] = v; return; }
  const __bf16 h = (__bf16)v;
  const __bf16 l = (__bf16)(v - (float)h);
  __bf16* out = reinterpret_cast<__bf16*>(j.wpk);
  if (!(j.flags & 1)) {
    __bf16* rec = out + (e >> 5) * 64;
    rec[e & 31] = h;
    rec[32 + (e & 31)] = l;
    return;
  }
  const int nb = (rows + 31) / 32, kt = k >> 5, q = k & 31;
  const int64_t base = (((int64_t)kt * nb + (n >> 5)) * 2) ;
  const int sidx = (q >> 4) & 1, kh2 = (q >> 3) & 1, dw = (q >> 1) & 3, half = q & 1;
  const int64_t dh = ((((base + 0) * 2 + sidx) * 2 + kh2) * 32 + (n & 31)) * 4 + dw;
  const int64_t dl = ((((base + 1) * 2 + sidx) * 2 + kh2) * 32 + (n & 31)) * 4 + dw;
  out[dh * 2 + half] = h;
  out[dl * 2 + half] = l;
}

__global__ __launch_bounds__(256) void pack_jobs_kernel(PackJobs tab) {
  const PackJob& j = tab.j[blockIdx.y];
  const int taps = j.kh * j.kw;
  int cout = 0;
  for (int p = 0; p < j.npiece; ++p) cout += j.rows[p];
  if (j.mode == 3) {
    for (int e = blockIdx.x * 256 + threadIdx.x; e < cout; e += gridDim.x * 256) {
      int n = e, p = 0;
      while (p + 1 < j.npiece && n >= j.rows[p]) { n -= j.rows[p]; ++p; }
      j.wpk[e] = j.w[p][n];
    }
    return;
  }
  int cin = 0;
  for (int s = 0; s < j.nsrc; ++s) cin += j.srcC[s];
  const int m = j.mode % 10;
  int Ktot, rows;
  if (m == 1) { Ktot = taps * ((cout + 31) / 32 * 32); rows = cin; }
  else { Ktot = 0; for (int s = 0; s < j.nsrc; ++s) Ktot += taps * ((j.srcC[s] + 31) / 32 * 32); rows = cout; }
  const int rows_out = (j.flags & 1) ? (rows + 31) / 32 * 32 : rows;
  const int64_t total = (int64_t)rows_out * Ktot;
  for (int64_t e = (int64_t)blockIdx.x * 256 + threadIdx.x; e < total; e += (int64_t)gridDim.x * 256) {
    const int n = (int)(e / Ktot);
    int k = (int)(e % Ktot);
    if (m == 1) {
      const int cpad = (cout + 31) / 32 * 32;
      const int tp = k / cpad, c = k % cpad;
      float v = 0.f;
      if (c < cout && n < rows) {
        int s = 0, cs = n;
        while (s + 1 < j.nsrc && cs >= j.srcC[s]) { cs -= j.srcC[s]; ++s; }
        const float* q = pack_elem(j, c, s, cs, taps - 1 - tp);
        if (q) v = *q;
      }
      pack_store(j, Ktot, rows, n, k, v);
    } else {
      const int k0 = k;
      int s = 0;
      for (; s < j.nsrc; ++s) {
        const int span = taps * ((j.srcC[s] + 31) / 32 * 32);
        if (k < span) break;
        k -= span;
      }
      const int cpad = (j.srcC[s] + 31) / 32 * 32;
      const int t = k / cpad, c = k % cpad;
      const bool ok = c < j.srcC[s] && n < rows;
      float* q = ok ? pack_elem(j, n, s, c, t) : nullptr;
      if (m == 0) pack_store(j, Ktot, rows, n, k0, q ? *q : 0.f);
      else if (q) *q = j.accumulate ? *q + j.scale * j.wpk[e] : j.scale * j.wpk[e];
    }
  }
}

}

extern "C" int fsraft_pack_conv_weights(const fsraft_pack_job* jobs, int njobs, hipStream_t stream) {
  if (njobs < 0 || (njobs && !jobs)) return FS_ERR_ARG;
  for (int i = 0; i < njobs; ++i) {
    const fsraft_pack_job& j = jobs[i];
    const int m = j.mode;
    if (!(m == 0 || m == 1 || m == 2 || m == 3 || m == 10 || m == 11) || !j.wpk || j.npiece < 1 || j.npiece > 3) return FS_ERR_ARG;
    for (int p = 0; p < j.npiece; ++p) if (!j.w[p] || j.rows[p] < 1) return FS_ERR_ARG;
    if (m == 3) continue;
    if (j.nsrc < 1 || j.nsrc > 3 || j.kh < 1 || j.kw < 1 || j.cin_full < 1) return FS_ERR_ARG;
    if ((j.flags & 1) && m < 10) return FS_ERR_ARG;
    if ((j.flags & 2) && (j.kh != 2 || j.kw != 2 || j.nsrc != 1 || j.srcC[0] != 4 * j.cin_full || j.srcOff[0] != 0)) return FS_ERR_ARG;
    if (!(j.flags & 2)) for (int s = 0; s < j.nsrc; ++s) if (j.srcC[s] < 1 || j.srcOff[s] < 0 || j.srcOff[s] + j.srcC[s] > j.cin_full) return FS_ERR_ARG;
  }
  for (int i0 = 0; i0 < njobs; i0 += PACK_JOBS) {
    PackJobs tab{};
    const int n = njobs - i0 < PACK_JOBS ? njobs - i0 : PACK_JOBS;
    int64_t most = 0;
    for (int i = 0; i < n; ++i) {
      tab.j[i] = jobs[i0 + i];
      const fsraft_pack_job& j = tab.j[i];
      int64_t cout = 0, cin = 0;
      for (int p = 0; p < j.npiece; ++p) cout += j.rows[p];
      for (int s = 0; s < j.nsrc; ++s) cin += (j.srcC[s] + 31) / 32 * 32;
      const int64_t tot = j.mode == 3 ? cout : ((cout + 31) / 32 * 32) * ((cin + 31) / 32 * 32) * j.kh * j.kw;
      most = tot > most ? tot : most;
    }
    int blocks = (int)((most + 1023) / 1024);
    blocks = blocks < 1 ? 1 : (blocks > 512 ? 512 : blocks);
    hipLaunchKernelGGL(pack_jobs_kernel, dim3(blocks, n), dim3(256), 0, stream, tab);
  }
  return fs_launch_status();
}

extern "C" int fsraft_pack_conv_weight(float* w_oihw, float* wpk, int Cout, int Cin, int KH, int KW, const int* srcC,
                                       int nsrc, int mode, int accumulate, hipStream_t stream) {
  if (!w_oihw || !wpk || mode < 0 || (mode > 2 && mode != 10 && mode != 11)) return FS_ERR_ARG;
  PackArgs a{};
  a.split = mode >= 10;
  if (mode >= 10) mode -= 10;
  if (a.split && mode > 1) return FS_ERR_ARG;
  a.w = w_oihw; a.wpk = wpk; a.Cout = Cout; a.Cin = Cin; a.taps = KH * KW; a.mode = mode; a.accumulate = accumulate;
  if (mode == 1) {
    a.nsrc = 1; a.C[0] = Cout; a.C[1] = a.C[2] = 0;
    a.Ktot = a.taps * (((Cout + 31) / 32) * 32);
    a.rows = Cin;
  } else {
    if (!srcC || nsrc < 1 || nsrc > 3) return FS_ERR_ARG;
    int tot = 0;
    for (int s = 0; s < 3; ++s) { a.C[s] = s < nsrc ? srcC[s] : 0; tot += a.C[s]; }
    if (tot != Cin) return FS_ERR_ARG;
    a.nsrc = nsrc;
    a.Ktot = conv_ktot(srcC, nsrc, a.taps);
    a.rows = Cout;
  }
  const int64_t total = (int64_t)a.rows * a.Ktot;
  int blocks = (int)((total + 255) / 256 < 4096 ? (total + 255) / 256 : 4096);
  hipLaunchKernelGGL(pack_weight_kernel, dim3(blocks), dim3(256), 0, stream, a);
  return fs_launch_status();
}
```

### flow_supervisor_amd/csrc/conv_patch.inc

```
constexpr int PT_TW = 32, PT_BN = 128;
constexpr int PT_GMAX = 32;

struct PatchArgs {
  ConvArgs a;
  int ngroups;
  int tx;
  unsigned gtab[PT_GMAX];
  int cpt[3];
};

template <int EPI, int KH, int KW, int PT_TH, int BN = PT_BN>
__global__ __launch_bounds__(PT_TH * 64) void conv_patch_kernel(const PatchArgs args) {
  constexpr int PT_NT = PT_TH * 64, TN = BN / 64;
  using PCfg = SplitCfg<PT_TH * 32, BN, PT_TH / 2, 2, 2, true, PT_NT>;
  constexpr int TAPS = KH * KW, PHh = KH / 2, PWh = KW / 2;
  constexpr int PH = PT_TH + KH - 1, PW = PT_TW + KW - 1, ROWS = PH * PW;
  constexpr int PPITCH = 144;
  constexpr int PT_PLANE = ROWS * PPITCH;
  constexpr int PT_NCHP = (ROWS * 8 + PT_NT - 1) / PT_NT;
  constexpr int EPI_BYTES = PT_TH * 32 * (BN + 4) * 4, RING = 2 * PT_PLANE + 2 * BN * 128;
  __shared__ __attribute__((aligned(16))) char lds[RING > EPI_BYTES ? RING : EPI_BYTES];
  const ConvArgs& a = args.a;
  const int lane = threadIdx.x & 63, wave = __builtin_amdgcn_readfirstlane((int)(threadIdx.x >> 6));
  const int wm = wave >> 1, wn = wave & 1, l31 = lane & 31, lh = lane >> 5;
  const int n0 = blockIdx.x * BN;
  const int tile = blockIdx.y, tpi = args.tx * ((a.H + PT_TH - 1) / PT_TH);
  const int b = tile / tpi, trem = tile % tpi;
  const int y0 = (trem / args.tx) * PT_TH, x0 = (trem % args.tx) * PT_TW;
  const auto* gtab = (const unsigned __attribute__((address_space(4)))*)(
      (const char __attribute__((address_space(4)))*)__builtin_amdgcn_kernarg_segment_ptr() + offsetof(PatchArgs, gtab));
  const int NG = args.ngroups;

  unsigned ppix[PT_NCHP];
  const unsigned part16 = (threadIdx.x & 7) * 16;
#pragma unroll
  for (int j = 0; j < PT_NCHP; ++j) {
    const int row = (threadIdx.x + PT_NT * j) >> 3;
    const int y = y0 - PHh + row / PW, x = x0 - PWh + row % PW;
    const bool ok = row < ROWS && (unsigned)y < (unsigned)a.H && (unsigned)x < (unsigned)a.W;
    ppix[j] = ok ? (unsigned)((b * a.H + y) * a.W + x) : 0x7fffffffu;
  }
  constexpr int NCHW = BN * 8 / PT_NT;
  unsigned vbw[NCHW];
#pragma unroll
  for (int j = 0; j < NCHW; ++j) {
    const int e = threadIdx.x + PT_NT * j;
    vbw[j] = (e >> 3) < a.N - n0 ? (unsigned)((e >> 3) * a.Ktot * 4 + (e & 7) * 16) : FS_OOB;
  }
  const char* wbase = uni_ptr(reinterpret_cast<const char*>(a.wpk) + (int64_t)n0 * a.Ktot * 4);

  struct Group { const float* base; unsigned ld4, soff, crem4; int kt0, step; };
  auto group = [&](int g) {
    const unsigned e = gtab[__builtin_amdgcn_readfirstlane(g < NG ? g : NG - 1)];
    const unsigned src = e & 3u, c = (e >> 2) & 255u, crem = (e >> 10) & 63u;
    const bool s1 = src >= 1, s2 = src >= 2;
    Group r;
    r.base = uni_ptr(a.src[0].p + (s1 ? a.src[1].p - a.src[0].p : 0) + (s2 ? a.src[2].p - a.src[1].p : 0));
    r.ld4 = uni((unsigned)(a.src[0].ld + (s1 ? a.src[1].ld - a.src[0].ld : 0) + (s2 ? a.src[2].ld - a.src[1].ld : 0)) * 4u);
    r.soff = c * 128u; r.crem4 = crem * 4u;
    r.kt0 = (int)(e >> 16);
    r.step = args.cpt[0] + (s1 ? args.cpt[1] - args.cpt[0] : 0) + (s2 ? args.cpt[2] - args.cpt[1] : 0);
    return r;
  };
  float rp[PT_NCHP * 4];
  auto fetch_patch = [&](const Group& gr) {
    const __amdgpu_buffer_rsrc_t rs = make_rsrc(gr.base, 0x7fffffffu);
    const unsigned cok = part16 < gr.crem4 ? 0u : 0x80000000u;
#pragma unroll
    for (int j = 0; j < PT_NCHP; ++j) {
      const unsigned voff = ppix[j] == 0x7fffffffu ? FS_OOB : ((ppix[j] * gr.ld4 + part16) | cok);
      const f32x4 f = __builtin_bit_cast(f32x4, __builtin_amdgcn_raw_buffer_load_b128(rs, voff, gr.soff, 0));
      rp[4 * j] = f[0]; rp[4 * j + 1] = f[1]; rp[4 * j + 2] = f[2]; rp[4 * j + 3] = f[3];
    }
  };
  auto stage_patch = [&](char* plane) {
#pragma unroll
    for (int j = 0; j < PT_NCHP; ++j) {
      const int e = threadIdx.x + PT_NT * j;
      if ((e >> 3) < ROWS) stage_convert<PPITCH>(plane, e, rp + 4 * j);
    }
  };
  const __amdgpu_buffer_rsrc_t rsW = make_rsrc(wbase, 0x7fffffffu);
  float rw[NCHW * 4];
  auto fetch_w = [&](int kt) {
    const int ku = __builtin_amdgcn_readfirstlane(kt);
#pragma unroll
    for (int j = 0; j < NCHW; ++j) {
      const f32x4 f = __builtin_bit_cast(f32x4, __builtin_amdgcn_raw_buffer_load_b128(rsW, ku < 0 ? FS_OOB : vbw[j], ku < 0 ? 0u : (unsigned)ku * 128u, 0));
      rw[4 * j] = f[0]; rw[4 * j + 1] = f[1]; rw[4 * j + 2] = f[2]; rw[4 * j + 3] = f[3];
    }
  };
  auto stage_w = [&](char* bt) {
#pragma unroll
    for (int j = 0; j < NCHW; ++j) stage_copy<128>(bt, threadIdx.x + PT_NT * j, rw + 4 * j);
  };

  f32x16 acc[2][TN];
#pragma unroll
  for (int i = 0; i < 2; ++i)
#pragma unroll
    for (int j = 0; j < TN; ++j)
#pragma unroll
      for (int r = 0; r < 16; ++r) acc[i][j][r] = 0.f;
  char* plane0 = lds;
  char* plane1 = lds + PT_PLANE;
  char* bt0 = lds + 2 * PT_PLANE;
  char* bt1 = bt0 + BN * 128;

  const int rb = wn * (BN / 2) + l31;
  const int la_off = (2 * wm * PW + l31) * PPITCH + lh * 16;
  auto compute = [&](const char* plane, const char* bt, int dy, int dx) {
    const char* Bs = bt + rb * 128;
#pragma unroll
    for (int s = 0; s < 2; ++s) {
      bf16x8 ah[2], al[2], bh[TN], bl[TN];
#pragma unroll
      for (int mt = 0; mt < 2; ++mt) {
        ah[mt] = *reinterpret_cast<const bf16x8*>(plane + la_off + ((dy + mt) * PW + dx) * PPITCH + (2 * s) * 16);
        al[mt] = *reinterpret_cast<const bf16x8*>(plane + la_off + ((dy + mt) * PW + dx) * PPITCH + (4 + 2 * s) * 16);
      }
      const int obh = slot_offset<128>(rb, 2 * s + lh) - rb * 128, obl = slot_offset<128>(rb, 4 + 2 * s + lh) - rb * 128;
#pragma unroll
      for (int nt = 0; nt < TN; ++nt) {
        bh[nt] = *reinterpret_cast<const bf16x8*>(Bs + nt * 32 * 128 + obh);
        bl[nt] = *reinterpret_cast<const bf16x8*>(Bs + nt * 32 * 128 + obl);
      }
#pragma unroll
      for (int mt = 0; mt < 2; ++mt)
#pragma unroll
        for (int nt = 0; nt < TN; ++nt) acc[mt][nt] = __builtin_amdgcn_mfma_f32_32x32x16_bf16(al[mt], bh[nt], acc[mt][nt], 0, 0, 0);
#pragma unroll
      for (int mt = 0; mt < 2; ++mt)
#pragma unroll
        for (int nt = 0; nt < TN; ++nt) acc[mt][nt] = __builtin_amdgcn_mfma_f32_32x32x16_bf16(ah[mt], bl[nt], acc[mt][nt], 0, 0, 0);
#pragma unroll
      for (int mt = 0; mt < 2; ++mt)
#pragma unroll
        for (int nt = 0; nt < TN; ++nt) acc[mt][nt] = __builtin_amdgcn_mfma_f32_32x32x16_bf16(ah[mt], bh[nt], acc[mt][nt], 0, 0, 0);
    }
  };

  Group gc = group(0);
  fetch_patch(gc);
  fetch_w(gc.kt0);
  stage_patch(plane0);
  stage_w(bt0);
  Group gn = group(1);
  if (NG > 1) fetch_patch(gn);
  fetch_w(TAPS > 1 ? gc.kt0 + gc.step : (NG > 1 ? gn.kt0 : -1));
  __syncthreads();
  for (int g = 0; g < NG; ++g) {
#pragma unroll
    for (int t = 0; t < TAPS; ++t) {
      const int i = g * TAPS + t;
      char* btc = (i & 1) ? bt1 : bt0;
      char* btn = (i & 1) ? bt0 : bt1;
      compute((g & 1) ? plane1 : plane0, btc, t / KW, t % KW);
      stage_w(btn);
      {
        const int t2 = t + 2;
        int kt;
        if (t2 < TAPS) kt = gc.kt0 + t2 * gc.step;
        else kt = g + 1 < NG ? gn.kt0 + (t2 - TAPS) * gn.step : -1;
        if (TAPS == 1) {
          const Group g2 = group(g + 2);
          kt = g + 2 < NG ? g2.kt0 : -1;
        }
        fetch_w(kt);
      }
      if (t == TAPS - 1 && g + 1 < NG) {
        stage_patch((g & 1) ? plane0 : plane1);
        gc = gn;
        gn = group(g + 2);
        if (g + 2 < NG) fetch_patch(gn);
      }
      __syncthreads();
    }
  }
  conv_epilogue_lds<PCfg, EPI, PT_NT, true>(a, acc, 0, n0, reinterpret_cast<float*>(lds), true, b, y0, x0);
}

template <int KH, int KW, int TH>
int launch_conv_patch_t(const PatchArgs& p, int epi, dim3 grid, hipStream_t s) {
  t_route[0] = (TH == 8 ? 11 : 10) + (KH == 3 && KW == 3 && p.a.N <= 64 ? 2 : 0);
  if constexpr (KH == 3 && KW == 3) {
    if (p.a.N <= 64) {
      hipLaunchKernelGGL((conv_patch_kernel<EPI_PLAIN, 3, 3, TH, 64>), grid, dim3(TH * 64), 0, s, p);
      return fs_launch_status();
    }
  }
  with_epi(epi, [&](auto e) { hipLaunchKernelGGL((conv_patch_kernel<decltype(e)::value, KH, KW, TH>), grid, dim3(TH * 64), 0, s, p); });
  return fs_launch_status();
}

int launch_conv_patch(const ConvArgs& a, int epi, hipStream_t s) {
  const bool k33 = a.KH == 3 && a.KW == 3, k15 = a.KH == 1 && a.KW == 5, k51 = a.KH == 5 && a.KW == 1;
  if (!(k33 || k15 || k51) || a.PH != a.KH / 2 || a.PW != a.KW / 2 || !epilogue_rows_ok_host(a)) return -1;
  PatchArgs p;
  p.a = a; p.a.swz = 0;
  int ng = 0, kt = 0;
  const int taps = a.KH * a.KW;
  for (int sidx = 0; sidx < 3; ++sidx) p.cpt[sidx] = 1;
  for (int sidx = 0; sidx < a.nsrc; ++sidx) {
    const int C = a.src[sidx].C, cpt = (C + 31) / 32;
    p.cpt[sidx] = cpt;
    if ((int64_t)a.B * a.H * a.W * a.src[sidx].ld * 4 >= (int64_t)0x7fffffff) return -1;
    for (int c = 0; c < cpt; ++c) {
      if (ng >= PT_GMAX || kt + c >= (1 << 16)) return -1;
      const int crem = C - c * 32 < 32 ? C - c * 32 : 32;
      p.gtab[ng++] = (unsigned)sidx | (unsigned)c << 2 | (unsigned)crem << 10 | (unsigned)(kt + c) << 16;
    }
    kt += taps * cpt;
  }
  if (kt * 32 != a.Ktot || ng < 1) return -1;
  for (int g = ng; g < PT_GMAX; ++g) p.gtab[g] = p.gtab[ng - 1];
  p.ngroups = ng;
  p.tx = ceil_div(a.W, PT_TW);
  const int bn = a.N <= 64 ? 64 : PT_BN;
  if (bn == 64 && !(k33 && epi == EPI_PLAIN)) return -1;
  const int64_t wg8 = (int64_t)ceil_div(a.N, bn) * p.tx * ceil_div(a.H, 8) * a.B;
  if (bn == 64 && wg8 >= 200 && knob.conv_patch64 == 1) return -1;
  if (wg8 >= 200 && !(bn == 64 && knob.conv_patch64 == 2)) {
    dim3 grid(ceil_div(a.N, bn), p.tx * ceil_div(a.H, 8) * a.B);
    if (k33) return launch_conv_patch_t<3, 3, 8>(p, epi, grid, s);
    if (k15) return launch_conv_patch_t<1, 5, 8>(p, epi, grid, s);
    return launch_conv_patch_t<5, 1, 8>(p, epi, grid, s);
  }
  const bool small_grid_33 = k33 && a.N > 128 && (int64_t)ceil_div(a.N, 128) * ceil_div(a.B * a.H * a.W, 128) > 120;
  if (knob.conv_patch != 2 && bn != 64 && !small_grid_33) return -1;
  dim3 grid(ceil_div(a.N, bn), p.tx * ceil_div(a.H, 4) * a.B);
  if (k33) return launch_conv_patch_t<3, 3, 4>(p, epi, grid, s);
  if (k15) return launch_conv_patch_t<1, 5, 4>(p, epi, grid, s);
  return launch_conv_patch_t<5, 1, 4>(p, epi, grid, s);
}
```

### flow_supervisor_amd/csrc/conv_tuning.hip

```cpp
#include "conv_common.hpp"
#include <climits>

ConvKnobs knob;
__thread int t_route[2] = {0, 0};

namespace {
const struct { int key; int ConvKnobs::*member; } KNOB_TABLE[] = {
    {FSRAFT_KEY_CONV_TILE, &ConvKnobs::conv_tile},
    {FSRAFT_KEY_WGRAD_TILE, &ConvKnobs::wgrad_tile},
    {FSRAFT_KEY_WGRAD_BLOCKS, &ConvKnobs::wgrad_blocks},
    {FSRAFT_KEY_CONV_ARITH, &ConvKnobs::conv_split},
    {FSRAFT_KEY_WGRAD_ARITH, &ConvKnobs::wgrad_split},
    {FSRAFT_KEY_CONV_BUF, &ConvKnobs::conv_buf},
    {FSRAFT_KEY_XCD_SWIZZLE, &ConvKnobs::xcd_swizzle},
    {FSRAFT_KEY_WGRAD_BUF, &ConvKnobs::wgrad_buf},
    {FSRAFT_KEY_CONV_N256, &ConvKnobs::conv_n256},
    {FSRAFT_KEY_WGRAD_MULTI, &ConvKnobs::wgrad_multi},
    {FSRAFT_KEY_WGRAD_BLOCKS_MULTI, &ConvKnobs::wgrad_blocks_multi},
    {FSRAFT_KEY_CONV_UNIFORM, &ConvKnobs::conv_uniform},
    {FSRAFT_KEY_CONV_W8, &ConvKnobs::conv_w8},
    {FSRAFT_KEY_CONV_W8_MIN, &ConvKnobs::conv_w8_min},
    {FSRAFT_KEY_WGRAD_W8, &ConvKnobs::wgrad_w8},
    {FSRAFT_KEY_WGRAD_PACK, &ConvKnobs::wgrad_pack},
    {FSRAFT_KEY_WGRAD_BLOCKS_PACK, &ConvKnobs::wgrad_blocks_pack},
    {FSRAFT_KEY_CONV_N64, &ConvKnobs::conv_n64},
    {FSRAFT_KEY_CONV_N64_MIN_M, &ConvKnobs::conv_n64_min_m},
    {FSRAFT_KEY_CONV_HALO, &ConvKnobs::conv_halo},
    {FSRAFT_KEY_CONV_HALO_MIN_M, &ConvKnobs::conv_halo_min_m},
    {FSRAFT_KEY_WGRAD_XCD, &ConvKnobs::wgrad_xcd},
    {FSRAFT_KEY_CONV_PATCH, &ConvKnobs::conv_patch},
    {FSRAFT_KEY_WGRAD_PATCH, &ConvKnobs::wgrad_patch},
    {FSRAFT_KEY_CONV_PATCH64, &ConvKnobs::conv_patch64},
    {FSRAFT_KEY_WGRAD_PATCH1, &ConvKnobs::wgrad_patch1},
    {FSRAFT_KEY_CONV_PATCH_MIN_M, &ConvKnobs::conv_patch_min_m},
    {FSRAFT_KEY_CONV_KSPLIT, &ConvKnobs::conv_ksplit},
};

int* knob_of(int key) {
  for (const auto& e : KNOB_TABLE)
    if (e.key == key) return &(knob.*e.member);
  return nullptr;
}
}

extern "C" int fsraft_set_tuning(int key, int value) {
  int* k = knob_of(key);
  if (!k) return FS_ERR_ARG;
  *k = value;
  return FS_OK;
}

extern "C" int fsraft_get_tuning(int key) {
  const int* k = knob_of(key);
  return k ? *k : INT_MIN;
}

extern "C" int fsraft_conv_last_route(int which) {
  return which == 0 || which == 1 ? t_route[which] : -1;
}

extern "C" int fsraft_set_arithmetic(int mode) {
  if (mode != 0 && mode != 1) return FS_ERR_ARG;
  knob.conv_split = mode ? 1 : 0;
  knob.wgrad_split = mode ? 2 : 0;
  fsraft_set_build_split(mode);
  fsraft_set_gemm_split(mode);
  return FS_OK;
}
extern "C" int fsraft_get_arithmetic(void) { return knob.conv_split != 0 ? 1 : 0; }
```

### flow_supervisor_amd/ops.py

```python
import ctypes
import math
import os

import torch
import torch.optim.optimizer as _optimizer_module

from . import _lib as L


def _lib():
    return L.load()


def parameters_updated(params):
    ps = [p for p in params if isinstance(p, torch.Tensor)]
    if ps:
        torch._C._autograd._unsafe_set_version_counter(ps, [p._version + 1 for p in ps])


def _after_optimizer_step(opt, args, kwargs):
    parameters_updated([p for g in opt.param_groups if g.get("fused") for p in g["params"]])


_optimizer_module.register_optimizer_step_post_hook(_after_optimizer_step)
# ... 856 lines not shown
    scratch = torch.empty(N * H * W * 18, device=flow.device, dtype=torch.float32)
    L.check(_lib().fsraft_upsample_bwd(L.ptr(flow), bs, cs, ps, L.ptr(mask_nhwc), L.ptr(dup), L.ptr(dmask),
                                       L.ptr(dflow), L.ptr(scratch), N, H, W, L.stream()), "upsample_bwd")
    return dflow, dmask


def upflow8_fwd(flow):
    L.require_cuda_f32(flow)
    flow = flow.contiguous()
    N, C, H, W = flow.shape
    up = torch.empty(N, C, 8 * H, 8 * W, device=flow.device, dtype=torch.float32)
    L.check(_lib().fsraft_upflow8_fwd(L.ptr(flow), L.ptr(up), N, C, H, W, L.stream()), "upflow8_fwd")
    return up


def upflow8_bwd(dup, H, W):
    dup = dup.contiguous()
    N, C = dup.shape[:2]
    dflow = torch.empty(N, C, H, W, device=dup.device, dtype=torch.float32)
    L.check(_lib().fsraft_upflow8_bwd(L.ptr(dup), L.ptr(dflow), N, C, H, W, L.stream()), "upflow8_bwd")
    return dflow


def nchw_to_nhwc(src, dst=None, coff=0, accumulate=False):
    L.require_cuda_f32(src)
    src = src.contiguous()
    B, C, H, W = src.shape
    if dst is None:
        dst = (torch.empty if C % 4 == 0 else torch.zeros)(B, H, W, (C + 3) // 4 * 4, device=src.device, dtype=torch.float32)
    ld = dst.shape[-1]
    L.check(_lib().fsraft_nchw_to_nhwc(L.ptr(src), L.ptr(dst), B, C, H * W, ld, coff, int(accumulate), L.stream()),
            "nchw_to_nhwc")
    return dst


def nhwc_to_nchw(src, C=None, coff=0, dst=None, accumulate=False):
    L.require_cuda_f32(src)
    B, H, W, ld = src.shape
    C = ld if C is None else C
    if dst is None:
        dst = torch.empty(B, C, H, W, device=src.device, dtype=torch.float32)
    L.check(_lib().fsraft_nhwc_to_nchw(L.ptr(src), L.ptr(dst), B, C, H * W, ld, coff, int(accumulate), L.stream()),
            "nhwc_to_nchw")
    return dst


def im2col7(flow, cols):
    B, _, H, W = flow.shape
    bs, cs, ps = _planar2_strides(flow)
    L.check(_lib().fsraft_im2col7(L.ptr(flow), bs, cs, ps, L.ptr(cols), cols.shape[-1], B, H, W, L.stream()), "im2col7")
    return cols


def col2im7(dcols, dflow, accumulate):
    B, _, H, W = dflow.shape
    L.check(_lib().fsraft_col2im7(L.ptr(dcols), dcols.shape[-1], L.ptr(dflow), B, H, W, int(accumulate), L.stream()),
            "col2im7")


def flow_to_nhwc(flow, dst, coff):
    B, _, H, W = flow.shape
    bs, cs, ps = _planar2_strides(flow)
    L.check(_lib().fsraft_flow_to_nhwc(L.ptr(flow), bs, cs, ps, L.ptr(dst), dst.shape[-1], coff, B, H * W, L.stream()),
            "flow_to_nhwc")


def nhwc_to_flow(src, coff, dflow, accumulate):
    B, _, H, W = dflow.shape
    L.check(_lib().fsraft_nhwc_to_flow(L.ptr(src), src.shape[-1], coff, L.ptr(dflow), B, H * W, int(accumulate),
                                       L.stream()), "nhwc_to_flow")


def relu_bwd_(g, y, C):
    M = g.numel() // g.shape[-1]
    L.check(_lib().fsraft_relu_bwd(L.ptr(g), g.shape[-1], L.ptr(y), y.shape[-1], M, C, L.stream()), "relu_bwd")


def gru_bwd1(dhn, z, q, h, dzr, dq, dh, hid, dzr_sum=None, dq_sum=None, dhn2=None):
    M = dhn.numel() // hid
    L.check(_lib().fsraft_gru_bwd1(L.ptr(dhn), L.ptr(dhn2), L.ptr(z), L.ptr(q), L.ptr(h), L.ptr(dzr), dzr.shape[-1], L.ptr(dq),
                                   L.ptr(dh), L.ptr(dzr_sum), L.ptr(dq_sum), M, hid, L.stream()), "gru_bwd1")


def gru_bwd2(drh, r, h, dzr, dh, hid, dzr_sum=None):
    M = drh.numel() // hid
    L.check(_lib().fsraft_gru_bwd2(L.ptr(drh), L.ptr(r), L.ptr(h), L.ptr(dzr), dzr.shape[-1], L.ptr(dh), L.ptr(dzr_sum), M, hid,
                                   L.stream()), "gru_bwd2")


def col_sum_(x, C, out, scale=1.0):
    M = x.numel() // x.shape[-1]
    L.check(_lib().fsraft_col_sum(L.ptr(x), x.shape[-1], M, C, L.ptr(out), float(scale), L.stream()), "col_sum")


def sum_n_(tensors, out, accumulate=False):
    n = tensors[0].numel()
    for t in tensors:
        L.require_cuda_f32(t)
        if t.numel() != n or not t.is_contiguous():
            raise ValueError("sum_n_: contiguous tensors of one size")
    if out.numel() < n or not out.is_contiguous():
        raise ValueError("sum_n_: out too small / not contiguous")
    pp, keep = L.ptr_array(tensors)
    L.check(_lib().fsraft_sum_n(pp, len(tensors), L.ptr(out), n, int(accumulate), L.stream()), "sum_n")
    return out


def axpby_(x, y, a=1.0, b=1.0):
    L.check(_lib().fsraft_axpby(L.ptr(x), L.ptr(y), float(a), float(b), x.numel(), L.stream()), "axpby")


def conv_ktot(srcC, KH, KW):
    return _lib().fsraft_conv_ktot(L.int_array(srcC), len(srcC), KH, KW)


def pack_weight(w, srcC, mode):
    L.require_cuda_f32(w)
    w = w.contiguous()
    Cout, Cin, KH, KW = w.shape
    if mode % 10 == 0:
        rows, kt = Cout, conv_ktot(srcC, KH, KW)
    else:
        rows, kt = Cin, conv_ktot([Cout], KH, KW)
    wpk = torch.empty(rows, kt, device=w.device, dtype=torch.float32)
    L.check(_lib().fsraft_pack_conv_weight(L.ptr(w), L.ptr(wpk), Cout, Cin, KH, KW, L.int_array(srcC), len(srcC), mode,
                                           0, L.stream()), "pack_conv_weight")
    return wpk


class PackPlan:

    def __init__(self, device):
        self.device = device
        self.jobs = []
        self.total = 0
        self.keep = []

    def _job(self, ws, cin_full, kh, kw, srcC, srcOff, mode, flags=0, scale=1.0, accumulate=False):
        j = L.PackJob()
        for i, w in enumerate(ws):
            L.require_cuda_f32(w)
            assert w.is_contiguous()
            j.w[i] = w.data_ptr()
            j.rows[i] = w.shape[0]
        j.npiece = len(ws)
        j.cin_full, j.kh, j.kw = cin_full, kh, kw
        for i, (c, o) in enumerate(zip(srcC, srcOff)):
            j.srcC[i], j.srcOff[i] = c, o
        j.nsrc = len(srcC)
        j.mode, j.flags, j.scale, j.accumulate = mode, flags, scale, int(accumulate)
        self.keep.append(ws)
        return j

    def pack(self, ws, srcC, mode, srcOff=None, kh=None, kw=None, cin_full=None, frag=False, s2d=False):
        w0 = ws[0]
        cin_full = w0.shape[1] if cin_full is None else cin_full
        kh = (2 if s2d else w0.shape[2]) if kh is None else kh
        kw = (2 if s2d else w0.shape[3]) if kw is None else kw
        srcOff = [sum(srcC[:i]) for i in range(len(srcC))] if srcOff is None else srcOff
        cout = sum(w.shape[0] for w in ws)
        if mode % 10 == 0:
            rows, kt = cout, conv_ktot(srcC, kh, kw)
        else:
            rows, kt = sum(srcC), conv_ktot([cout], kh, kw)
        if frag:
            rows = (rows + 31) // 32 * 32
        j = self._job(ws, cin_full, kh, kw, srcC, srcOff, mode, (1 if frag else 0) | (2 if s2d else 0))
        self.jobs.append((j, self.total, (rows, kt)))
        self.total += (rows * kt + 63) // 64 * 64
        return len(self.jobs) - 1

    def bias(self, bs):
        j = self._job(bs, 1, 1, 1, [1], [0], 3)
        n = sum(b.shape[0] for b in bs)
        self.jobs.append((j, self.total, (n,)))
        self.total += (n + 63) // 64 * 64
        return len(self.jobs) - 1

    def run(self):
        buf = torch.empty(max(self.total, 1), device=self.device, dtype=torch.float32)
        arr = (L.PackJob * max(len(self.jobs), 1))()
        outs = []
        for i, (j, off, shape) in enumerate(self.jobs):
            n = 1
            for v in shape:
                n *= v
            t = buf[off:off + n].view(shape)
            j.wpk = t.data_ptr()
            arr[i] = j
            outs.append(t)
        if self.jobs:
            L.check(_lib().fsraft_pack_conv_weights(arr, len(self.jobs), L.stream()), "pack_conv_weights")
        self.keep = []
        return outs


def unpack_weight_grads(items, device):
    if not items:
        return
    arr = (L.PackJob * len(items))()
    plan = PackPlan(device)
    for i, (dwpk, gs, srcC, srcOff, cin_full, kh, kw, scale, s2d) in enumerate(items):
        j = plan._job(gs, cin_full, kh, kw, srcC, srcOff, 2, 2 if s2d else 0, scale)
        j.wpk = dwpk.data_ptr()
        arr[i] = j
    L.check(_lib().fsraft_pack_conv_weights(arr, len(items), L.stream()), "unpack_conv_weights")


def exact_mode():
    return _lib().fsraft_get_tuning(3) == 0


def set_arithmetic(split):
    global SPLIT_VOLUME_BWD
    L.check(_lib().fsraft_set_arithmetic(1 if split else 0), "set_arithmetic")
    SPLIT_VOLUME_BWD = bool(split)


def pack_pair(w, srcC, dgrad=False):
    m = 1 if dgrad else 0
    split = pack_weight(w, srcC, 10 + m)
    rows = w.shape[1] if dgrad else w.shape[0]
    return (pack_weight(w, srcC, m) if (exact_mode() or rows <= 32) else split), split


def fragment_order(wps):
    N, ktot = wps.shape
    kt, nb = ktot // 32, (N + 31) // 32
    w = wps.contiguous().view(torch.int32)
    if nb * 32 != N:
        w = torch.cat([w, w.new_zeros(nb * 32 - N, ktot)])
    w = w.view(nb, 32, kt, 2, 2, 2, 4).permute(2, 0, 3, 4, 5, 1, 6).contiguous()
    return w.view(torch.float32).view(kt, nb, 4, 64, 4)


def unpack_weight_grad(dwpk, shape, srcC, out=None, accumulate=False):
    Cout, Cin, KH, KW = shape
    if out is None:
        out = torch.empty(shape, device=dwpk.device, dtype=torch.float32)
        accumulate = False
    L.check(_lib().fsraft_pack_conv_weight(L.ptr(out), L.ptr(dwpk), Cout, Cin, KH, KW, L.int_array(srcC), len(srcC), 2,
                                           int(accumulate), L.stream()), "unpack_conv_weight")
    return out


class V:
    __slots__ = ("t", "off", "C", "ld")

    def __init__(self, t, C=None, off=0):
        self.t, self.off, self.ld = t, off, t.shape[-1]
        self.C = (t.shape[-1] - off) if C is None else C
        assert off % 4 == 0 and self.ld % 4 == 0, "channel slices must stay 16-byte aligned"

    @property
    def ptr(self):
        return self.t.data_ptr() + 4 * self.off


class Dst:
    __slots__ = ("t", "off", "bs", "ps", "cs", "n0", "acc", "mask")

    def __init__(self, t, off, bs, ps, cs, n0=0, acc=False):
        self.t, self.off, self.bs, self.ps, self.cs, self.n0, self.acc = t, off, bs, ps, cs, n0, acc
        self.mask = None

    def masked(self, v):
        self.mask = v
        return self

    @staticmethod
    def nhwc(buf, coff=0, n0=0, acc=False):
        B, H, W, ld = buf.shape
        return Dst(buf, coff, H * W * ld, ld, 1, n0, acc)

    @staticmethod
    def nchw(buf, n0=0, acc=False):
        B, C, H, W = buf.shape
        return Dst(buf, 0, C * H * W, 1, H * W, n0, acc)


_CONV_WS = {}
CONV_WS_FLOATS = 24 << 20
CONV_WS_MAX_PIXELS = 16384


def _conv_workspace(device, pixels):
    if pixels > CONV_WS_MAX_PIXELS:
        return None
    key = (torch.device(device).index or 0, torch.cuda.current_stream(device).cuda_stream)
    ws = _CONV_WS.get(key)
    if ws is None:
        ws = _CONV_WS.setdefault(key, torch.empty(CONV_WS_FLOATS, device=device, dtype=torch.float32))
    return ws


def conv_forward(srcs, wpk, bias, B, H, W, KH, KW, N, dsts, relu=False, alpha=1.0, epi=0, h=None, z=None,
                 aux1=None, aux2=None, hid=0, wpk_split=None, pre=None, wpk_frag=None, pad=None, stats=None):
    d = L.ConvDesc()
    for i, v in enumerate(srcs):
        d.src[i] = v.ptr; d.srcC[i] = v.C; d.srcld[i] = v.ld
    d.nsrc = len(srcs)
    d.wpk = wpk.data_ptr()
    d.wpk_split = wpk_split.data_ptr() if wpk_split is not None else None
    d.wpk_frag = wpk_frag.data_ptr() if wpk_frag is not None else None
    if pad is not None:
        d.pad_h1, d.pad_w1 = pad[0] + 1, pad[1] + 1
    d.bias = bias.data_ptr() if bias is not None else None
    d.B, d.H, d.W, d.KH, d.KW, d.N = B, H, W, KH, KW, N
    for i, ds in enumerate(dsts):
        d.dst[i] = ds.t.data_ptr() + 4 * ds.off
        d.dst_bs[i], d.dst_ps[i], d.dst_cs[i] = ds.bs, ds.ps, ds.cs
        d.dst_n0[i] = ds.n0; d.dst_acc[i] = int(ds.acc)
        if ds.mask is not None:
            d.rmask[i] = ds.mask.ptr; d.ldmask[i] = ds.mask.ld; d.maskc[i] = ds.mask.C
    d.ndst = len(dsts)
    d.relu = int(relu); d.alpha = float(alpha); d.epi = epi
    if h is not None:
        d.h = h.data_ptr(); d.ldh = h.shape[-1]
    if z is not None:
        d.z = z.data_ptr(); d.ldz = z.shape[-1]
    if aux1 is not None:
        d.aux1 = aux1.data_ptr(); d.ld1 = aux1.shape[-1]
    if aux2 is not None:
        d.aux2 = aux2.data_ptr(); d.ld2 = aux2.shape[-1]
    d.hid = hid
    if pre is not None:
        d.pre = pre.data_ptr(); d.ldpre = pre.shape[-1]
    ws = _conv_workspace(dsts[0].t.device, B * H * W)
    if ws is not None:
        d.ws = ws.data_ptr(); d.ws_floats = ws.numel()
    t = TIMER
    e0 = t.begin() if t else None
    carried = None
    if stats is not None:
        done = ctypes.c_int(0)
        L.check(_lib().fsraft_conv_forward_stats(ctypes.byref(d), L.ptr(stats[0]), L.ptr(stats[1]), stats.shape[1] // B, ctypes.byref(done),
                                                 L.stream()), "conv_forward_stats")
        carried = bool(done.value)
    else:
        L.check(_lib().fsraft_conv_forward(ctypes.byref(d), L.stream()), "conv_forward")
    if t:
        cin = sum(v.C for v in srcs)
        t.end("conv_igemm", e0, 2.0 * B * H * W * N * cin * KH * KW, 4.0 * B * H * W * (cin + N),
              tag=f"{B}x{H}x{W} {KH}x{KW} {'+'.join(str(v.C) for v in srcs)}->{N} epi{epi}{' relu' if relu else ''}{' masked' if any(ds.mask is not None for ds in dsts) else ''}")
    return carried


def conv_wgrad(dy, srcs, dwpk, B, H, W, KH, KW, dbias=None):
    arr = (ctypes.c_void_p * len(srcs))(*[v.ptr for v in srcs])
    pp = ctypes.cast(arr, L._PP)
    e0w = TIMER.begin() if TIMER else None
    L.check(_lib().fsraft_conv_wgrad(ctypes.c_void_p(dy.ptr), dy.ld, dy.C, pp, L.int_array([v.C for v in srcs]),
                                     L.int_array([v.ld for v in srcs]), len(srcs), L.ptr(dwpk), L.ptr(dbias), B, H, W,
                                     KH, KW, L.stream()), "conv_wgrad")
    if TIMER:
        cin = sum(v.C for v in srcs)
        TIMER.end("conv_wgrad", e0w, 2.0 * B * H * W * dy.C * cin * KH * KW, 4.0 * B * H * W * (cin + dy.C),
                  tag=f"{B}x{H}x{W} {KH}x{KW} {'+'.join(str(v.C) for v in srcs)}->{dy.C} x1")


def conv_wgrad_multi(dys, srcs, dwpk, B, H, W, KH, KW, dbias=None):
    n, nsrc = len(dys), len(srcs[0])
    dy0 = dys[0]
    a_dy = (ctypes.c_void_p * n)(*[v.ptr for v in dys])
    a_src = (ctypes.c_void_p * (n * nsrc))(*[v.ptr for sl in srcs for v in sl])
    e0w = TIMER.begin() if TIMER else None
    L.check(_lib().fsraft_conv_wgrad_multi(ctypes.cast(a_dy, L._PP), n, dy0.ld, dy0.C, ctypes.cast(a_src, L._PP),
                                           L.int_array([v.C for v in srcs[0]]), L.int_array([v.ld for v in srcs[0]]), nsrc,
                                           L.ptr(dwpk), L.ptr(dbias), B, H, W, KH, KW, L.stream()), "conv_wgrad_multi")
    if TIMER:
        cin = sum(v.C for v in srcs[0])
        TIMER.end("conv_wgrad", e0w, 2.0 * n * B * H * W * dy0.C * cin * KH * KW, 4.0 * n * B * H * W * (cin + dy0.C),
                  tag=f"{B}x{H}x{W} {KH}x{KW} {'+'.join(str(v.C) for v in srcs[0])}->{dy0.C} x{n}")


def stem_fwd(x, w, bias=None):
    L.require_cuda_f32(x, w)
    B, C, H, W = x.shape
    N = w.shape[0]
    if C != 3 or tuple(w.shape[1:]) != (3, 7, 7) or not x.is_contiguous():
        raise RuntimeError("stem_fwd: x [B,3,H,W] contiguous and w [N,3,7,7] expected")
    out = torch.empty(B, (H - 1) // 2 + 1, (W - 1) // 2 + 1, N, device=x.device, dtype=torch.float32)
    t = TIMER
    e0 = t.begin() if t else None
    L.check(_lib().fsraft_stem7x7s2_fwd(L.ptr(x), L.ptr(w.contiguous()), L.ptr(bias), L.ptr(out), B, H, W, N, L.stream()), "stem7x7s2_fwd")
    if t:
        t.end("stem", e0, 2.0 * out.numel() * 147, 4.0 * (x.numel() + out.numel()))
    return out


def stem_wgrad(x, dy):
    L.require_cuda_f32(x, dy)
    B, C, H, W = x.shape
    N = dy.shape[-1]
    if not (x.is_contiguous() and dy.is_contiguous()) or tuple(dy.shape[:3]) != (B, (H - 1) // 2 + 1, (W - 1) // 2 + 1):
        raise RuntimeError("stem_wgrad: contiguous x [B,3,H,W] and dy [B,Ho,Wo,N] expected")
    lib = _lib()
    scratch = torch.empty(lib.fsraft_stem_slots() * 64 * 192, device=x.device, dtype=torch.float32)
    dw = torch.empty(N, 3, 7, 7, device=x.device, dtype=torch.float32)
    t = TIMER
    e0 = t.begin() if t else None
    L.check(lib.fsraft_stem7x7s2_wgrad(L.ptr(x), L.ptr(dy), L.ptr(dw), L.ptr(scratch), B, H, W, N, L.stream()), "stem7x7s2_wgrad")
    if t:
        t.end("stem", e0, 2.0 * dy.numel() * 147, 4.0 * (x.numel() + dy.numel()))
    return dw


def conv_small_fwd(x, w_oihw, bias, out_nchw):
    B, N, H, W = out_nchw.shape
    t = TIMER
    e0 = t.begin() if t else None
    L.check(_lib().fsraft_conv_small_fwd(ctypes.c_void_p(x.ptr), x.ld, x.C, L.ptr(w_oihw), L.ptr(bias), L.ptr(out_nchw),
                                         N * H * W, H * W, 1, N, B, H, W, 3, 3, L.stream()), "conv_small_fwd")
    if t:
        t.end("conv_small", e0, 2.0 * B * H * W * N * x.C * 9, 4.0 * B * H * W * (x.C + N))


def conv_small_wgrad(dys, xs, dwpk, dbias, B, H, W):
    n = len(dys)
    a_dy = (ctypes.c_void_p * n)(*[v.ptr for v in dys])
    a_x = (ctypes.c_void_p * n)(*[v.ptr for v in xs])
    L.check(_lib().fsraft_conv_small_wgrad(ctypes.cast(a_dy, L._PP), ctypes.cast(a_x, L._PP), n, dys[0].ld, xs[0].ld, xs[0].C,
                                           L.ptr(dwpk), L.ptr(dbias), dys[0].C, B, H, W, 3, 3, L.stream()), "conv_small_wgrad")


def conv_small_dgrad(dy, w_oihw, dst, mask, B, H, W):
    C = dst.C
    t = TIMER
    e0 = t.begin() if t else None
    L.check(_lib().fsraft_conv_small_dgrad(ctypes.c_void_p(dy.ptr), dy.ld, L.ptr(w_oihw), ctypes.c_void_p(dst.ptr), dst.ld,
                                           ctypes.c_void_p(mask.ptr) if mask is not None else None, mask.ld if mask is not None else 0,
                                           C, 2, B, H, W, 3, 3, L.stream()), "conv_small_dgrad")
    if t:
        t.end("conv_small", e0, 2.0 * B * H * W * 2 * C * 9, 4.0 * B * H * W * (C * (2 if mask is not None else 1) + 2))


def col_sum_v(v, out, scale=1.0):
    M = v.t.numel() // v.ld
    L.check(_lib().fsraft_col_sum(ctypes.c_void_p(v.ptr), v.ld, M, v.C, L.ptr(out), float(scale), L.stream()), "col_sum")


def flow_metrics_scratch_bytes(B, H, W):
    n = _lib().fsraft_flow_metrics_scratch_bytes(B, H, W)
    if n == 1:
        raise RuntimeError(f"libfsraft: flow_metrics_scratch_bytes({B}, {H}, {W}) failed with status 1 (bad argument)")
    return n


def flow_metrics(pred, gt, valid, sample_stats, acc=None, scratch=None):
    L.require_cuda_f32(pred, gt, valid)
    B, C, H, W = pred.shape
    if C != 2 or gt.shape != pred.shape or (valid is not None and valid.shape != (B, H, W)):
        raise RuntimeError(f"flow_metrics: pred {tuple(pred.shape)}, gt {tuple(gt.shape)}, "
                           f"valid {None if valid is None else tuple(valid.shape)}")
    if W > 1 and any(t.stride(-1) != 1 for t in (pred, gt, valid) if t is not None):
        raise RuntimeError("flow_metrics: pred, gt and valid need a unit x stride")
    for t, shape in ((sample_stats, (B, 8)), (acc, (8,))):
# ... 10 lines not shown
```

### include/fsraft.h

```cpp
#ifndef FSRAFT_H
#define FSRAFT_H

#include <stdint.h>

#ifdef __cplusplus
extern "C" {
#endif

#ifndef __HIP_PLATFORM_AMD__
typedef struct ihipStream_t* hipStream_t;
#endif

#define FSRAFT_OK 0
#define FSRAFT_ERR_ARG 1
#define FSRAFT_ERR_LAUNCH 2

int fsraft_corr_build(const float* fmap1, const float* fmap2, float* const* levels, int num_levels,
                      int B, int C, int H, int W, hipStream_t stream);

int fsraft_corr_pool_pyramid(float* const* levels, int num_levels, int64_t rows, int H2, int W2, hipStream_t stream);
int fsraft_corr_pool_pyramid_same(float* const* levels, int num_levels, int64_t rows, int H2, int W2, hipStream_t stream);
int fsraft_corr_lookup_fwd_same(float* const* levels, int num_levels, const float* coords, int64_t coords_bs,
                                int64_t coords_cs, int64_t coords_ps, float* out, int nhwc_out, int B, int H, int W,
                                int radius, hipStream_t stream);
int fsraft_corr_unpool_bwd(float* const* dlevels, int num_levels, int B, int H, int W, hipStream_t stream);
int fsraft_corr_unpool_same_bwd(float* const* dlevels, int num_levels, int64_t rows, int H2, int W2, hipStream_t stream);
int fsraft_corr_lookup_bwd_same(float* const* dlevels, int num_levels, const float* coords, int64_t coords_bs,
                                int64_t coords_cs, int64_t coords_ps, const float* dout, int nhwc_in, int B, int H, int W,
                                int radius, hipStream_t stream);
int fsraft_corr_lookup_dcoords_same(float* const* levels, int num_levels, const float* coords, int64_t coords_bs, int64_t coords_cs,
                                    int64_t coords_ps, const float* dout, int nhwc_in, float* dcoords, int64_t dbs, int64_t dcs,
                                    int64_t dps, int B, int H, int W, int radius, hipStream_t stream);

int fsraft_vol_layout(int H, int W, int num_levels, int* out);
int fsraft_corr_build_tiled(const float* fmap1, const float* fmap2, float* vol, int num_levels, int B, int C, int H, int W,
                            hipStream_t stream);
int fsraft_corr_build_rec(const void* f1r, const void* f2r, float* vol, int num_levels, int B, int C, int H, int W,
                          hipStream_t stream);
int fsraft_corr_lookup_tiled_fwd(const float* vol, int num_levels, const float* coords, int64_t coords_bs, int64_t coords_cs,
                                 int64_t coords_ps, float* out, int B, int H, int W, int radius, int add_grid, hipStream_t stream);
int fsraft_corr_lookup_tiled_dcoords(const float* vol, int num_levels, const float* coords, int64_t coords_bs, int64_t coords_cs,
                                     int64_t coords_ps, const float* dout, float* dcoords, int64_t dbs, int64_t dcs, int64_t dps,
                                     int B, int H, int W, int radius, int add_grid, hipStream_t stream);
int fsraft_corr_dvol_build(const float* const* dout, const float* const* coords, const int64_t* coords_str, int n, float* dvol,
                           int num_levels, int B, int H, int W, int radius, int accumulate, int records, int add_grid,
                           int64_t q0, int64_t nq, unsigned* qlist, const unsigned* wmask,
                           hipStream_t stream);
int fsraft_corr_f2cat(const float* fmap2, float* f2cat, int num_levels, int B, int C, int H, int W, hipStream_t stream);
int fsraft_corr_dfmap2(const float* d2cat, float* d2, int num_levels, int B, int C, int H, int W, hipStream_t stream);
int fsraft_corr_f2cat_rec(const float* fmap2, void* f2r, int num_levels, int B, int C, int H, int W, hipStream_t stream);

int fsraft_corr_lookup_fwd(float* const* levels, int num_levels, const float* coords, int64_t coords_bs,
                           int64_t coords_cs, int64_t coords_ps, float* out, int nhwc_out, int B, int H, int W,
                           int radius, hipStream_t stream);
int fsraft_corr_lookup_bwd(float* const* dlevels, int num_levels, const float* coords, int64_t coords_bs,
                           int64_t coords_cs, int64_t coords_ps, const float* dout, int nhwc_in, int B, int H, int W,
                           int radius, hipStream_t stream);
int fsraft_corr_lookup_dcoords(float* const* levels, int num_levels, const float* coords, int64_t coords_bs, int64_t coords_cs,
                               int64_t coords_ps, const float* dout, int nhwc_in, float* dcoords, int64_t dbs, int64_t dcs,
                               int64_t dps, int B, int H, int W, int radius, hipStream_t stream);

int fsraft_altcorr_fwd(const float* fmap1, const float* fmap2, const float* coords, float* corr, int B, int N, int H1,
                       int W1, int H2, int W2, int C, int radius, hipStream_t stream);
int fsraft_altcorr_bwd(const float* fmap1, const float* fmap2, const float* coords, const float* corr_grad,
                       float* fmap1_grad, float* fmap2_grad, int B, int N, int H1, int W1, int H2, int W2, int C,
                       int radius, hipStream_t stream);

int fsraft_altcorr_fused_fwd(const float* fmap1, const float* const* fmap2_levels, int num_levels, const float* coords,
                             int64_t coords_bs, int64_t coords_cs, int64_t coords_ps, int add_grid, float* out, int B, int H, int W,
                             int C, int radius, hipStream_t stream);
int fsraft_altcorr_fused_dcoords(const float* fmap1, const float* const* fmap2_levels, int num_levels, const float* coords,
                                 int64_t coords_bs, int64_t coords_cs, int64_t coords_ps, int add_grid, const float* dout,
                                 float* dcoords, int64_t dbs, int64_t dcs, int64_t dps, int B, int H, int W, int C, int radius,
                                 hipStream_t stream);

int fsraft_altcorr_mfma_fwd(const void* f1r, const void* const* f2r_levels, const float* fmap1, const float* const* fmap2_levels,
                            int num_levels, const float* coords, int64_t coords_bs, int64_t coords_cs, int64_t coords_ps,
                            int add_grid, float* out, int B, int H, int W, int C, int radius, hipStream_t stream);

int fsraft_upsample_fwd(const float* flow, int64_t flow_bs, int64_t flow_cs, int64_t flow_ps,
                        const float* mask_nhwc, float* up, int N, int H, int W, hipStream_t stream);
int fsraft_upsample_bwd(const float* flow, int64_t flow_bs, int64_t flow_cs, int64_t flow_ps,
                        const float* mask_nhwc, const float* dup, float* dmask_nhwc, float* dflow, float* scratch,
                        int N, int H, int W, hipStream_t stream);
int fsraft_upflow8_fwd(const float* flow, float* up, int N, int C, int H, int W, hipStream_t stream);
int fsraft_upflow8_bwd(const float* dup, float* dflow, int N, int C, int H, int W, hipStream_t stream);

typedef struct fsraft_conv_desc {
  const float* src[3]; int srcC[3]; int srcld[3]; int nsrc;
  const float* wpk; const float* bias;
  const float* wpk_split;
  int B, H, W, KH, KW, N;
  float* dst[3]; int64_t dst_bs[3]; int64_t dst_ps[3]; int64_t dst_cs[3];
  int dst_n0[3]; int dst_acc[3]; int ndst;
  int relu; float alpha;
  int epi;
  const float* h; int ldh; const float* z; int ldz;
  float* aux1; int ld1; float* aux2; int ld2; int hid;
  const float* pre; int ldpre;
  const float* rmask[3]; int ldmask[3]; int maskc[3];
  const float* wpk_frag;
  int pad_h1, pad_w1;
  float* ws; int64_t ws_floats;
} fsraft_conv_desc;

int fsraft_conv_ktot(const int* srcC, int nsrc, int KH, int KW);
int fsraft_conv_forward(const fsraft_conv_desc* d, hipStream_t stream);
int fsraft_conv_forward_stats(const fsraft_conv_desc* d, float* sum, float* sq, int slots, int* done, hipStream_t stream);
int fsraft_conv_wgrad(const float* dy, int ldy, int Cout, const float* const* src, const int* srcC,
                      const int* srcld, int nsrc, float* dwpk, float* dbias, int B, int H, int W, int KH, int KW,
                      hipStream_t stream);
int fsraft_conv_wgrad_multi(const float* const* dy, int nseg, int ldy, int Cout, const float* const* src,
                            const int* srcC, const int* srcld, int nsrc, float* dwpk, float* dbias, int B, int H, int W,
                            int KH, int KW, hipStream_t stream);
int fsraft_pack_conv_weight(float* w_oihw, float* wpk, int Cout, int Cin, int KH, int KW, const int* srcC,
                            int nsrc, int mode, int accumulate, hipStream_t stream);

typedef struct {
  float* w[3]; int rows[3]; int npiece;
  float* wpk;
  int cin_full, kh, kw;
  int srcC[3], srcOff[3], nsrc;
  int mode, flags;
  float scale; int accumulate;
} fsraft_pack_job;
int fsraft_pack_conv_weights(const fsraft_pack_job* jobs, int njobs, hipStream_t stream);

int fsraft_conv_small_fwd(const float* x, int ld, int C, const float* w_oihw, const float* bias, float* out, int64_t obs,
                          int64_t ocs, int64_t ops, int N, int B, int H, int W, int KH, int KW, hipStream_t stream);
int fsraft_conv_small_wgrad(const float* const* dy, const float* const* x, int nseg, int ldy, int ldx, int C, float* dwpk,
                            float* dbias, int N, int B, int H, int W, int KH, int KW, hipStream_t stream);
int fsraft_conv_small_dgrad(const float* dy, int ldy, const float* w_oihw, float* dx, int lddx, const float* relu_src, int ldm,
                            int C, int N, int B, int H, int W, int KH, int KW, hipStream_t stream);

int fsraft_conv_workspace(float* ws, int64_t floats);

int fsraft_set_arithmetic(int mode);
int fsraft_get_arithmetic(void);

int fsraft_gemm_f32(const float* A, int64_t lda, int64_t sA, const float* Bm, int64_t ldb, int64_t sB, float* C,
                    int64_t ldc, int64_t sC, int batch, int M, int N, int K, int trans_b, float alpha,
                    int accumulate, hipStream_t stream);

int fsraft_gemm_tn_split(const float* A, int64_t lda, int64_t sA, const float* Bm, int64_t ldb, int64_t sB, float* C,
                         int64_t ldc, int64_t sC, int batch, int M, int N, int K, float alpha, int accumulate,
                         hipStream_t stream);

int fsraft_to_records(const float* src, int64_t ld, void* dst, int64_t dst_ld, int64_t rows, int K, hipStream_t stream);
int fsraft_gemm_rec_nt(const void* A, int64_t lda, int64_t sA, const void* Bm, int64_t ldb, int64_t sB, float* C, int64_t ldc,
                       int64_t sC, int batch, int M, int N, int K, float alpha, int ksplit, int accumulate, hipStream_t stream);
int fsraft_gemm_rec_tn(const void* A, int64_t lda, int64_t sA, const void* Bm, int64_t ldb, int64_t sB, float* C, int64_t ldc,
                       int64_t sC, int batch, int M, int N, int K, float alpha, int ksplit, int accumulate, hipStream_t stream);

int fsraft_gemm_rec_nt_list(const void* A, int64_t lda, int64_t sA, const void* Bm, int64_t ldb, int64_t sB, float* C, int64_t ldc,
                            int64_t sC, int batch, int M, int N, int K, float alpha, int ksplit, int accumulate, const int* klist,
                            const int* kcount, int kl_stride, int kl_by_n, hipStream_t stream);
int fsraft_gemm_rec_tn_list(const void* A, int64_t lda, int64_t sA, const void* Bm, int64_t ldb, int64_t sB, float* C, int64_t ldc,
                            int64_t sC, int batch, int M, int N, int K, float alpha, int ksplit, int accumulate, const int* klist,
                            const int* kcount, int kl_stride, int kl_by_n, hipStream_t stream);
int fsraft_corr_bwd_ktiles(const float* const* coords, const int64_t* coords_str, int n, int num_levels, int B, int H, int W,
                           int radius, int add_grid, int64_t q0, int64_t nq, int* nt_list, int* nt_count, int nt_stride, unsigned* tn_bits,
                           int* tn_list, int* tn_count, int tn_stride, unsigned* wmask, hipStream_t stream);

int fsraft_softmax_rows(float* S, int64_t rows, int n, hipStream_t stream);
int fsraft_softmax_rows_bwd(const float* A, float* dA, int64_t rows, int n, hipStream_t stream);
int fsraft_softmax_rows_rec(float* S, int64_t rows, int n, hipStream_t stream);
int fsraft_softmax_rows_bwd_rec(const void* A_records, float* dA, int64_t rows, int n, hipStream_t stream);
int fsraft_softmax_rows_pos(float* S, const float* G, int64_t ldg, int64_t rows, int n, int h, int w, int content, int records,
                            hipStream_t stream);
int fsraft_softmax_rows_pos_bwd(const void* A, float* dA, float* dG, int64_t ldg, int64_t rows, int n, int h, int w, int records,
                                hipStream_t stream);
int fsraft_gma_mix_fwd(const float* x, int ldx, const float* y, int ldy, const float* gamma, float* dst, int ldd,
                       int64_t M, int C, hipStream_t stream);
int fsraft_gma_mix_bwd(const float* d, int ldd, const float* y, int ldy, const float* gamma, float* dx, int ldx,
                       float* dy, int lddy, float* dgamma, int64_t M, int C, hipStream_t stream);

int fsraft_inorm_relu_fwd(const float* x, float* y, float* stats, int64_t planes, int HW, float eps, int relu, hipStream_t stream);
int fsraft_inorm_relu_bwd(const float* g, const float* x, const float* stats, float* dx, int64_t planes, int HW, int relu,
                          hipStream_t stream);
int fsraft_affine_relu_fwd(const float* x, const float* scale, const float* shift, float* y, int64_t planes, int C, int HW,
                           int relu, hipStream_t stream);
int fsraft_affine_relu_bwd(const float* g, const float* x, const float* scale, const float* shift, float* dx, float* dsum_g,
                           float* dsum_gx, int64_t planes, int C, int HW, int relu, hipStream_t stream);

int fsraft_sequence_loss(const float* const* pred, float* const* dpred, const float* weights, int n, int metric_idx,
                         const float* gt, const float* valid, float max_flow, float eps, int B, int H, int W, float* out,
                         hipStream_t stream);

int fsraft_forward_interpolate(const float* flow, float* out, int H, int W, hipStream_t stream);

int fsraft_flow_metrics_scratch_bytes(int B, int H, int W);
int fsraft_flow_metrics(const float* pred, int64_t pred_bs, int64_t pred_cs, int64_t pred_rs,
                        const float* gt, int64_t gt_bs, int64_t gt_cs, int64_t gt_rs,
                        const float* valid, int64_t valid_bs, int64_t valid_rs, int B, int H, int W,
                        double* sample_stats, double* acc, void* scratch, int64_t scratch_bytes, hipStream_t stream);

int fsraft_inorm_relu_cl_fwd(const float* x, const float* res, float* y, float* sums, float* sumsq, float* stats, int B, int HW,
                             int C, float eps, int relu, int have_sums, int s2d_w, hipStream_t stream);
int fsraft_inorm_relu_cl_bwd(const float* g, const float* x, const float* stats, const float* out, float* s1, float* s2, float* dx,
                             float* dres, int B, int HW, int C, int relu, int s2d_w, hipStream_t stream);
int fsraft_affine_relu_cl_fwd(const float* x, const float* res, const float* scale, const float* shift, float* y, int64_t M, int C,
                              int relu, int HW, int s2d_w, hipStream_t stream);
int fsraft_affine_relu_cl_bwd(const float* g, const float* x, const float* scale, const float* shift, const float* out, float* dx,
                              float* dres, float* dsum_g, float* dsum_gx, int B, int HW, int C, int relu, int s2d_w, hipStream_t stream);

int fsraft_bn_fold(const float* weight, const float* bias, const float* rm, const float* rv, const float* cbias, float eps, int C,
                   float* scale, float* shift, float* rs, float* rmc, hipStream_t stream);
int fsraft_bn_fold_bwd(const float* part, int R, int C, const float* rs, const float* rmc, const float* scale, float* dweight,
                       float* dbias, float* dcbias, hipStream_t stream);

int fsraft_stem_slots(void);
int fsraft_stem7x7s2_fwd(const float* x, const float* w, const float* bias, float* out, int B, int H, int W, int N,
                         hipStream_t stream);
int fsraft_stem7x7s2_wgrad(const float* x, const float* dy, float* dw, float* scratch, int B, int H, int W, int N,
                           hipStream_t stream);

int fsraft_adamw_flat(float* p, float* g, float* m, float* v, int64_t n, float* step, const float* norm, float max_norm,
                      const float* lr, double beta1, double beta2, float eps, float weight_decay, float* state,
                      const unsigned char* skip64, hipStream_t stream);
int fsraft_stream_capture_id(hipStream_t stream, unsigned long long* id);

int fsraft_nchw_to_nhwc(const float* src, float* dst, int B, int C, int HW, int ld, int coff, int accumulate, hipStream_t s);
int fsraft_space_to_depth2(const float* src, float* dst, int B, int H, int W, int C, int inverse, hipStream_t s);
int fsraft_nhwc_to_nchw(const float* src, float* dst, int B, int C, int HW, int ld, int coff, int accumulate, hipStream_t s);
int fsraft_im2col7(const float* flow, int64_t bs, int64_t cs, int64_t ps, float* cols, int ld, int B, int H, int W, hipStream_t s);
int fsraft_col2im7(const float* dcols, int ld, float* dflow, int B, int H, int W, int accumulate, hipStream_t s);
int fsraft_flow_to_nhwc(const float* flow, int64_t bs, int64_t cs, int64_t ps, float* dst, int ld, int coff, int B, int HW, hipStream_t s);
int fsraft_nhwc_to_flow(const float* src, int ld, int coff, float* dflow, int B, int HW, int accumulate, hipStream_t s);
int fsraft_relu_bwd(float* g, int ldg, const float* y, int ldy, int64_t M, int C, hipStream_t s);
int fsraft_gru_bwd1(const float* dhn, const float* dhn2, const float* z, const float* q, const float* h, float* dzr, int ldzr, float* dq, float* dh, float* dzr_sum, float* dq_sum, int64_t M, int hid, hipStream_t s);
int fsraft_gru_bwd2(const float* drh, const float* r, const float* h, float* dzr, int ldzr, float* dh, float* dzr_sum, int64_t M, int hid, hipStream_t s);
int fsraft_col_sum(const float* x, int ld, int64_t M, int C, float* out, float scale, hipStream_t s);
int fsraft_axpby(const float* x, float* y, float a, float b, int64_t n, hipStream_t s);
int fsraft_sum_n(const float* const* src, int n, float* out, int64_t count, int accumulate, hipStream_t s);

#ifdef __cplusplus
}
#endif
#endif
```

### include/fsraft_tuning.h

```cpp
#ifndef FSRAFT_TUNING_H
#define FSRAFT_TUNING_H

#ifdef __cplusplus
extern "C" {
#endif

enum fsraft_tuning_key {
  FSRAFT_KEY_CONV_TILE = 0,
  FSRAFT_KEY_WGRAD_TILE = 1,
  FSRAFT_KEY_WGRAD_BLOCKS = 2,
  FSRAFT_KEY_CONV_ARITH = 3,
  FSRAFT_KEY_WGRAD_ARITH = 4,
  FSRAFT_KEY_CONV_BUF = 5,
  FSRAFT_KEY_XCD_SWIZZLE = 7,
  FSRAFT_KEY_WGRAD_BUF = 8,
  FSRAFT_KEY_CONV_N256 = 9,
  FSRAFT_KEY_WGRAD_MULTI = 10,
  FSRAFT_KEY_WGRAD_BLOCKS_MULTI = 11,
  FSRAFT_KEY_CONV_UNIFORM = 12,
  FSRAFT_KEY_CONV_W8 = 13,
  FSRAFT_KEY_CONV_W8_MIN = 14,
  FSRAFT_KEY_WGRAD_W8 = 15,
  FSRAFT_KEY_WGRAD_PACK = 16,
  FSRAFT_KEY_WGRAD_BLOCKS_PACK = 17,
  FSRAFT_KEY_CONV_N64 = 18,
  FSRAFT_KEY_CONV_N64_MIN_M = 19,
  FSRAFT_KEY_CONV_HALO = 20,
  FSRAFT_KEY_CONV_HALO_MIN_M = 21,
  FSRAFT_KEY_WGRAD_XCD = 22,
  FSRAFT_KEY_CONV_PATCH = 26,
  FSRAFT_KEY_WGRAD_PATCH = 27,
  FSRAFT_KEY_CONV_PATCH64 = 28,
  FSRAFT_KEY_WGRAD_PATCH1 = 29,
  FSRAFT_KEY_CONV_PATCH_MIN_M = 31,
  FSRAFT_KEY_CONV_KSPLIT = 32
};
int fsraft_set_tuning(int key, int value);
int fsraft_get_tuning(int key);
int fsraft_conv_last_route(int which);
int fsraft_set_wgrad_wide(int mode);
int fsraft_conv_wgrad_last_tile(void);
int fsraft_set_build_split(int on);
int fsraft_set_build_kernel(int which);
int fsraft_set_lookup_policy(int aux);
int fsraft_set_ktile_exact(int levels);
int fsraft_set_upsample_kernel(int v4);
int fsraft_set_dvol_box(int on);
int fsraft_set_dvol_policy(int policy);
int fsraft_set_gemm_split(int on);
int fsraft_set_lookup_qb(int qb);
int fsraft_set_norm_blocks(int target_workgroups);
int fsraft_set_rec_mfma16(int on);
int fsraft_set_alt_tile(int on);

#ifdef __cplusplus
}
#endif
#endif
```

Before: 110.4 image-pairs/s.

## Skip structurally-zero space-to-depth taps in stride-2 conv and add 96-column patch kernel

For the stride-2 3x3 conv rewritten as a 2x2 conv over space-to-depth input, a compacted weight pack is built that keeps only the 9 of 16 tap/subpixel blocks that are nonzero. The implicit-GEMM K-table is then built over just those live blocks, so the K loop shrinks by about 7/16. A second change adds a patch-kernel variant with 96 output columns for 3x3 convs with 65-96 output channels, so those layers no longer pad up to a wider tile. The cost is extra pack memory and routing complexity, and the live path gives up the k-split route and falls back to the dense path when the K-table cannot be built.

```diff
diff --git a/flow_supervisor_amd/_lib.py b/flow_supervisor_amd/_lib.py
--- a/flow_supervisor_amd/_lib.py
+++ b/flow_supervisor_amd/_lib.py
@@ -27,6 +27,7 @@
         ("rmask", c_void_p * 3), ("ldmask", c_int * 3), ("maskc", c_int * 3),
         ("wpk_frag", c_void_p), ("pad_h1", c_int), ("pad_w1", c_int),
         ("ws", c_void_p), ("ws_floats", c_int64),
+        ("wpk_live", c_void_p),
     ]
 
 
@@ -123,6 +124,11 @@
     "fsraft_conv_last_route": [c_int],
     "fsraft_set_wgrad_wide": [c_int],
     "fsraft_conv_wgrad_last_tile": [],
+    "fsraft_set_conv_live": [c_int],
+    "fsraft_conv_last_live_tiles": [],
+    "fsraft_set_conv_patch96": [c_int],
+    "fsraft_conv_last_patch_cols": [],
+    "fsraft_s2d_live_blocks": [c_int, _IP, _IP, c_int],
     "fsraft_space_to_depth2": [c_void_p, c_void_p, c_int, c_int, c_int, c_int, c_int, _S],
     "fsraft_forward_interpolate": [c_void_p, c_void_p, c_int, c_int, _S],
     "fsraft_flow_metrics_scratch_bytes": [c_int, c_int, c_int],
diff --git a/flow_supervisor_amd/core/extractor.py b/flow_supervisor_amd/core/extractor.py
--- a/flow_supervisor_amd/core/extractor.py
+++ b/flow_supervisor_amd/core/extractor.py
@@ -257,18 +257,19 @@
             b = plan.pack([w3], [4 * C], 11, cin_full=C, s2d=True)
             a0 = plan.pack([w3], [4 * C], 0, cin_full=C, s2d=True) if (exact or N <= 32) else a
             b0 = plan.pack([w3], [4 * C], 1, cin_full=C, s2d=True) if (exact or 4 * C <= 32) else b
+            al = plan.pack([w3], [4 * C], 10, cin_full=C, s2d=True, live=True) if (C % 32 == 0 and not exact) else None
             Ns, Cs = ws.shape[:2]
             c_ = plan.pack([ws], [Cs], 10)
             d_ = plan.pack([ws], [Cs], 11)
             c0 = plan.pack([ws], [Cs], 0) if (exact or Ns <= 32) else c_
             d0 = plan.pack([ws], [Cs], 1) if (exact or Cs <= 32) else d_
-            hs.append(((a0, a, b0, b), (c0, c_, d0, d_)))
+            hs.append(((a0, a, b0, b, al), (c0, c_, d0, d_)))
         out = plan.run()
         for (kind, m, key), h in zip(todo, hs):
             if kind == "conv":
                 m.__dict__["_fs_packs"] = (key,) + tuple(None if i is None else out[i] for i in h)
             else:
-                m.__dict__["_fs_pair_packs"] = (key, tuple(out[i] for i in h[0]), tuple(out[i] for i in h[1]))
+                m.__dict__["_fs_pair_packs"] = (key, tuple(None if i is None else out[i] for i in h[0]), tuple(out[i] for i in h[1]))
 
 
 def _weight_packs(conv):
@@ -444,7 +445,7 @@
         y1 = torch.empty(B, h, w, N, device=x.device, dtype=torch.float32)
         ys = torch.empty(B, h, w, Ns, device=x.device, dtype=torch.float32)
         p, q = packs[1], packs[2]
-        ops.conv_forward([ops.V(xs, 4 * C)], p[0], None, B, h, w, 2, 2, N, [ops.Dst.nhwc(y1)], wpk_split=p[1])
+        ops.conv_forward([ops.V(xs, 4 * C)], p[0], None, B, h, w, 2, 2, N, [ops.Dst.nhwc(y1)], wpk_split=p[1], wpk_live=p[4])
         ops.conv_forward([ops.V(xs, C, 0)], q[0], None, B, h, w, 1, 1, Ns, [ops.Dst.nhwc(ys)], wpk_split=q[1])
         ctx.save_for_backward(xs, w3, wsc)
         ctx.packs = packs
diff --git a/flow_supervisor_amd/csrc/conv_common.hpp b/flow_supervisor_amd/csrc/conv_common.hpp
--- a/flow_supervisor_amd/csrc/conv_common.hpp
+++ b/flow_supervisor_amd/csrc/conv_common.hpp
@@ -34,6 +34,8 @@
   int wgrad_patch1 = 8192;
   int conv_patch_min_m = 8192;
   int conv_ksplit = -1;
+  int conv_live = 1;
+  int conv_patch96 = 1;
 };
 __attribute__((visibility("hidden"))) extern ConvKnobs knob;
 __attribute__((visibility("hidden"))) extern __thread int t_route[2];
@@ -60,7 +62,24 @@
   float* st_sum; float* st_sq; int st_slots;
   int swz;
   int ksplit;
+  int live_c;
 };
+
+__host__ __device__ inline bool s2d_slot_live(int tap, int sp) {
+  return !(((tap >> 1) == 0 && (sp >> 1) == 0) || ((tap & 1) == 0 && (sp & 1) == 0));
+}
+__host__ __device__ inline int s2d_live_count(int C) { return (C < 32 || C % 32 != 0) ? 0 : 9 * (C / 32); }
+__host__ __device__ inline bool s2d_live_block(int C, int i, int& tap, int& chunk) {
+  const int cps = C / 32;
+  if (s2d_live_count(C) == 0 || i < 0) return false;
+  for (tap = 0; tap < 4; ++tap)
+    for (int sp = 0; sp < 4; ++sp) {
+      if (!s2d_slot_live(tap, sp)) continue;
+      if (i < cps) { chunk = sp * cps + i; return true; }
+      i -= cps;
+    }
+  return false;
+}
 
 constexpr int KTAB_MAX = 512;
 struct ConvArgsT {
diff --git a/flow_supervisor_amd/csrc/conv_igemm.hip b/flow_supervisor_amd/csrc/conv_igemm.hip
--- a/flow_supervisor_amd/csrc/conv_igemm.hip
+++ b/flow_supervisor_amd/csrc/conv_igemm.hip
@@ -314,6 +314,8 @@
   constexpr int RPP = NTW / C4;
   (void)owner;
   const int c4 = threadIdx.x % C4, rsub = threadIdx.x / C4;
+  const bool idle = NTW % C4 != 0 && rsub >= RPP;
+  const int row0 = idle ? Cfg::BM : rsub;
   const int n = n0 + c4 * 4;
   const bool stats = PATCH && EPI == EPI_PLAIN && a.st_sum != nullptr;
   if (n >= a.N && !stats) return;
@@ -332,7 +334,7 @@
     const int mkc = di == 0 ? a.maskc[0] : di == 1 ? a.maskc[1] : a.maskc[2];
     const int nv = a.N - n < 4 ? a.N - n : 4;
 #pragma unroll 4
-    for (int row = rsub; row < Cfg::BM; row += RPP) {
+    for (int row = row0; row < Cfg::BM; row += RPP) {
       const int64_t m = row_m(row);
       if (m < 0) { if (PATCH) continue; else break; }
       f32x4 v = *reinterpret_cast<const f32x4*>(tile + row * LD + c4 * 4);
@@ -368,8 +370,10 @@
       if (stats) {
         __syncthreads();
         float* red = tile;
-        *reinterpret_cast<f32x4*>(red + (rsub * Cfg::BN) + c4 * 4) = ssum;
-        *reinterpret_cast<f32x4*>(red + ((RPP + rsub) * Cfg::BN) + c4 * 4) = ssq;
+        if (!idle) {
+          *reinterpret_cast<f32x4*>(red + (rsub * Cfg::BN) + c4 * 4) = ssum;
+          *reinterpret_cast<f32x4*>(red + ((RPP + rsub) * Cfg::BN) + c4 * 4) = ssq;
+        }
         __syncthreads();
         if (threadIdx.x < Cfg::BN && n0 + (int)threadIdx.x < a.N) {
           float t1 = 0.f, t2 = 0.f;
@@ -385,7 +389,7 @@
     const bool isz = n < a.hid;
     const int c = isz ? n : n - a.hid;
 #pragma unroll 4
-    for (int row = rsub; row < Cfg::BM; row += RPP) {
+    for (int row = row0; row < Cfg::BM; row += RPP) {
       const int64_t mr = row_m(row);
       if (mr < 0 && !PATCH) break;
       const int64_t m = mr < 0 ? 0 : mr;
@@ -408,7 +412,7 @@
     }
   } else {
 #pragma unroll 4
-    for (int row = rsub; row < Cfg::BM; row += RPP) {
+    for (int row = row0; row < Cfg::BM; row += RPP) {
       const int64_t m = row_m(row);
       if (m < 0) { if (PATCH) continue; else break; }
       f32x4 v = *reinterpret_cast<const f32x4*>(tile + row * LD + c4 * 4);
@@ -761,8 +765,10 @@
   for (int s = 0; s < a.nsrc; ++s) {
     const int C = a.src[s].C, ld = a.src[s].ld, cpt = (C + 31) / 32;
     if (M * ld * 4 >= (int64_t)FS_OOB) return false;
-    for (int i = 0; i < taps * cpt; ++i, ++kt) {
-        const int tap = i / cpt, c = i % cpt;
+    const int nblk = a.live_c ? s2d_live_count(a.live_c) : taps * cpt;
+    for (int i = 0; i < nblk; ++i, ++kt) {
+        int tap = i / cpt, c = i % cpt;
+        if (a.live_c && !s2d_live_block(a.live_c, i, tap, c)) return false;
         const int64_t soff = ((int64_t)((tap / a.KW) * a.W + tap % a.KW) * ld + c * 32) * 4;
         if (soff % 16 != 0 || soff / 16 > 0xffff) return false;
         const int crem = C - c * 32 < 32 ? C - c * 32 : 32;
@@ -789,8 +795,10 @@
   for (int s = 0; s < a.nsrc; ++s) {
     const int C = a.src[s].C, cpt = (C + 31) / 32;
     const int64_t delta = (a.src[s].p - lo) * 4;
-    for (int tap = 0; tap < taps; ++tap)
-      for (int c = 0; c < cpt; ++c, ++kt) {
+    const int nblk = a.live_c ? s2d_live_count(a.live_c) : taps * cpt;
+    for (int i = 0; i < nblk; ++i, ++kt) {
+        int tap = i / cpt, c = i % cpt;
+        if (a.live_c && !s2d_live_block(a.live_c, i, tap, c)) return false;
         const int64_t soff = delta + ((int64_t)((tap / a.KW) * a.W + tap % a.KW) * ld + c * 32) * 4;
         if (soff + M * ld * 4 + 256 >= (int64_t)FS_OOB) return false;
         const int crem = C - c * 32 < 32 ? C - c * 32 : 32;
@@ -881,12 +889,14 @@
 thread_local int64_t t_reg_ws_floats = 0;
 thread_local float* g_conv_ws = nullptr;
 thread_local int64_t g_conv_ws_floats = 0;
-
-int pick_ksplit(int64_t tiles, int KT, int N, int64_t M, int ldw, int bm) {
+__thread int t_live_tiles = 0;
+__thread int t_patch_cols = 0;
+
+int pick_ksplit(int64_t tiles, int KT, int KTd, int N, int64_t M, int ldw, int bm) {
   int S = 1;
   if (knob.conv_ksplit >= 2) S = knob.conv_ksplit;
-  else if (knob.conv_ksplit == -1 && bm == 64 && tiles <= 150 && N <= 256 && KT >= 16) S = (int)((400 + tiles - 1) / tiles);
-  else if (knob.conv_ksplit == -1 && bm == 128 && tiles <= 120 && N <= 256 && KT >= (N <= 128 ? 36 : 48)) S = tiles <= 115 ? (int)(230 / tiles) : 2;
+  else if (knob.conv_ksplit == -1 && bm == 64 && tiles <= 150 && N <= 256 && KTd >= 16) S = (int)((400 + tiles - 1) / tiles);
+  else if (knob.conv_ksplit == -1 && bm == 128 && tiles <= 120 && N <= 256 && KTd >= (N <= 128 ? 36 : 48)) S = tiles <= 115 ? (int)(230 / tiles) : 2;
   if (S > KT / 6) S = KT / 6;
   if (S > 6) S = 6;
   while (S > 1 && (int64_t)S * M * ldw > g_conv_ws_floats) --S;
@@ -907,7 +917,8 @@
   if constexpr (Cfg::LDS_ALLOC >= Cfg::BM * (Cfg::BN + 4) * 4) {
     const int ldw = (a.N + 3) / 4 * 4;
     const bool gru_ok = epi == EPI_PLAIN || (a.N % 4 == 0 && (!a.pre || a.ldpre % 4 == 0));
-    const int S = (buf && g_conv_ws && gru_ok && (Cfg::BM == 64 || (Cfg::BM == 128 && Cfg::NT == 512) || knob.conv_ksplit >= 2)) ? pick_ksplit((int64_t)grid.x * grid.y, a.Ktot / 32, a.N, M, ldw, Cfg::BM) : 1;
+    const int S = (buf && g_conv_ws && gru_ok && (Cfg::BM == 64 || (Cfg::BM == 128 && Cfg::NT == 512) || knob.conv_ksplit >= 2)) ? pick_ksplit((int64_t)grid.x * grid.y, a.Ktot / 32, a.live_c ? a.live_c / 2 : a.Ktot / 32, a.N, M, ldw, Cfg::BM) : 1;
+    if (S > 1 && a.live_c) return -2;
     if (S > 1) {
       const bool uni_tab = build_ktab_uniform(a, t);
       if (uni_tab || build_ktab(a, t)) {
@@ -919,7 +930,7 @@
         p.ndst = 1; p.bias = nullptr; p.relu = 0; p.alpha = 1.0f;
         for (int i = 0; i < 3; ++i) p.rmask[i] = nullptr;
         dim3 g3(grid.x, grid.y, S);
-        t_route[0] = route_split<Cfg>() + 100;
+        t_route[0] = route_split<Cfg>() + 100; t_live_tiles = a.live_c ? a.Ktot / 32 : 0;
         if (uni_tab) hipLaunchKernelGGL((conv_igemm_split_kernel<Cfg, EPI_PLAIN, 2>), g3, dim3(Cfg::NT), 0, s, t);
         else hipLaunchKernelGGL((conv_igemm_split_kernel<Cfg, EPI_PLAIN, 1>), g3, dim3(Cfg::NT), 0, s, t);
         int rc = fs_launch_status();
@@ -933,20 +944,21 @@
   }
   if (buf && build_ktab_uniform(a, t)) {
     t.a.swz = swz;
-    t_route[0] = route_split<Cfg>();
+    t_route[0] = route_split<Cfg>(); t_live_tiles = a.live_c ? a.Ktot / 32 : 0;
     with_epi(epi, [&](auto e) { hipLaunchKernelGGL((conv_igemm_split_kernel<Cfg, decltype(e)::value, 2>), grid, dim3(Cfg::NT), 0, s, t); });
     return fs_launch_status();
   }
   if (buf && build_ktab(a, t)) {
     t.a.swz = swz;
-    t_route[0] = route_split<Cfg>();
+    t_route[0] = route_split<Cfg>(); t_live_tiles = a.live_c ? a.Ktot / 32 : 0;
     with_epi(epi, [&](auto e) { hipLaunchKernelGGL((conv_igemm_split_kernel<Cfg, decltype(e)::value, 1>), grid, dim3(Cfg::NT), 0, s, t); });
     return fs_launch_status();
   }
+  if (a.live_c) return -1;
   if constexpr (Cfg::NT != 256) {
     return -1;
   } else {
-  t_route[0] = route_split<Cfg>();
+  t_route[0] = route_split<Cfg>(); t_live_tiles = a.live_c ? a.Ktot / 32 : 0;
   with_epi(epi, [&](auto e) { hipLaunchKernelGGL((conv_igemm_split_kernel<Cfg, decltype(e)::value>), grid, dim3(256), 0, s, a); });
   return fs_launch_status();
   }
@@ -958,12 +970,12 @@
   dim3 grid(ceil_div(a.N, Cfg::BN), ceil_div(M, Cfg::BM));
   ConvArgsT t;
   if (build_ktab_uniform(a, t)) {
-    t_route[0] = route_split<Cfg>();
+    t_route[0] = route_split<Cfg>(); t_live_tiles = a.live_c ? a.Ktot / 32 : 0;
     hipLaunchKernelGGL((conv_igemm_split_kernel<Cfg, EPI_PLAIN, 2>), grid, dim3(Cfg::NT), 0, s, t);
     return fs_launch_status();
   }
   if (build_ktab(a, t)) {
-    t_route[0] = route_split<Cfg>();
+    t_route[0] = route_split<Cfg>(); t_live_tiles = a.live_c ? a.Ktot / 32 : 0;
     hipLaunchKernelGGL((conv_igemm_split_kernel<Cfg, EPI_PLAIN, 1>), grid, dim3(Cfg::NT), 0, s, t);
     return fs_launch_status();
   }
@@ -983,6 +995,9 @@
 
 }
 
+extern "C" int fsraft_conv_last_live_tiles(void) { return t_live_tiles; }
+extern "C" int fsraft_conv_last_patch_cols(void) { return t_patch_cols; }
+
 extern "C" int fsraft_conv_ktot(const int* srcC, int nsrc, int KH, int KW) {
   if (!srcC || nsrc < 1 || nsrc > 3) return -1;
   return conv_ktot(srcC, nsrc, KH * KW);
@@ -1002,7 +1017,7 @@
   const bool want_stats = t_stat.sum != nullptr && d->epi == EPI_PLAIN && d->ndst == 1 && !d->relu && d->alpha == 1.0f && !d->dst_acc[0] &&
                           !d->rmask[0] && !d->bias && d->dst_n0[0] == 0 && d->N % 4 == 0;
   if (d->ws && (((uintptr_t)d->ws & 15) || d->ws_floats < 0)) return FS_ERR_ARG;
-  t_route[0] = 0;
+  t_route[0] = 0; t_live_tiles = 0; t_patch_cols = 0;
   g_conv_ws = d->ws ? d->ws : t_reg_ws;
   g_conv_ws_floats = d->ws ? d->ws_floats : t_reg_ws_floats;
   ConvArgs a{};
@@ -1057,6 +1072,7 @@
   const int M = d->B * d->H * d->W;
   if (knob.conv_split && d->wpk_split && d->N > 32) {
     a.wpk = d->wpk_split;
+    const auto split_routes = [&](const ConvArgs& a) -> int {
     const bool narrow = knob.conv_buf != 0 || (int64_t)ceil_div(d->N, 128) * ceil_div(M, 128) < 400;
     if (knob.conv_patch && knob.conv_split == 1 && d->KH * d->KW > 1 && d->N > 64 && M >= knob.conv_patch_min_m) {
       ConvArgs p = a;
@@ -1073,15 +1089,25 @@
     }
     if (knob.conv_split == 1 && ((knob.conv_w8 == 1 && d->N >= 192 && d->N <= 512 && M >= 16384) || knob.conv_w8 == 2) && d->N >= 192) {
       const int rc = launch_conv_split<SCfg256W16>(a, d->epi, stream);
-      if (rc >= 0) return rc;
+      if (rc >= 0 || rc == -2) return rc;
     }
     if (knob.conv_w8 && knob.conv_split == 1 && (int64_t)ceil_div(d->N, 128) * ceil_div(M, 128) >= knob.conv_w8_min) {
       const int rc = launch_conv_split<SCfg128W8>(a, d->epi, stream);
-      if (rc >= 0) return rc;
+      if (rc >= 0 || rc == -2) return rc;
     }
     if (knob.conv_split == 3) return launch_conv_split<SCfgM64>(a, d->epi, stream);
     if (knob.conv_split == 4) return launch_conv_split<SCfg128>(a, d->epi, stream);
     return narrow ? launch_conv_split<SCfgM64>(a, d->epi, stream) : launch_conv_split<SCfg128>(a, d->epi, stream);
+    };
+    const int lc = d->srcC[0] / 4;
+    if (knob.conv_live && d->wpk_live && knob.conv_split == 1 && d->epi == EPI_PLAIN && d->nsrc == 1 && d->KH == 2 && d->KW == 2 &&
+        a.PH == 1 && a.PW == 1 && d->srcC[0] == 4 * lc && s2d_live_count(lc) > 0) {
+      ConvArgs l = a;
+      l.wpk = d->wpk_live; l.live_c = lc; l.Ktot = 32 * s2d_live_count(lc);
+      const int rc = split_routes(l);
+      if (rc >= 0) return rc;
+    }
+    return split_routes(a);
   }
   if (knob.conv_tile == 3) return launch_conv<Cfg6464>(a, d->epi, stream);
   if (knob.conv_tile == 4) return launch_conv<Cfg6464K16>(a, d->epi, stream);
diff --git a/flow_supervisor_amd/csrc/conv_pack.hip b/flow_supervisor_amd/csrc/conv_pack.hip
--- a/flow_supervisor_amd/csrc/conv_pack.hip
+++ b/flow_supervisor_amd/csrc/conv_pack.hip
@@ -110,6 +110,8 @@
   int Ktot, rows;
   if (m == 1) { Ktot = taps * ((cout + 31) / 32 * 32); rows = cin; }
   else { Ktot = 0; for (int s = 0; s < j.nsrc; ++s) Ktot += taps * ((j.srcC[s] + 31) / 32 * 32); rows = cout; }
+  const bool live = (j.flags & 4) != 0;
+  if (live) Ktot = 32 * s2d_live_count(j.cin_full);
   const int rows_out = (j.flags & 1) ? (rows + 31) / 32 * 32 : rows;
   const int64_t total = (int64_t)rows_out * Ktot;
   for (int64_t e = (int64_t)blockIdx.x * 256 + threadIdx.x; e < total; e += (int64_t)gridDim.x * 256) {
@@ -126,6 +128,11 @@
         if (q) v = *q;
       }
       pack_store(j, Ktot, rows, n, k, v);
+    } else if (live) {
+      int t = 0, chunk = 0;
+      s2d_live_block(j.cin_full, k >> 5, t, chunk);
+      float* q = n < rows ? pack_elem(j, n, 0, chunk * 32 + (k & 31), t) : nullptr;
+      pack_store(j, Ktot, rows, n, k, q ? *q : 0.f);
     } else {
       const int k0 = k;
       int s = 0;
@@ -157,6 +164,7 @@
     if (j.nsrc < 1 || j.nsrc > 3 || j.kh < 1 || j.kw < 1 || j.cin_full < 1) return FS_ERR_ARG;
     if ((j.flags & 1) && m < 10) return FS_ERR_ARG;
     if ((j.flags & 2) && (j.kh != 2 || j.kw != 2 || j.nsrc != 1 || j.srcC[0] != 4 * j.cin_full || j.srcOff[0] != 0)) return FS_ERR_ARG;
+    if ((j.flags & 4) && (!(j.flags & 2) || (j.flags & 1) || (m != 0 && m != 10) || s2d_live_count(j.cin_full) == 0)) return FS_ERR_ARG;
     if (!(j.flags & 2)) for (int s = 0; s < j.nsrc; ++s) if (j.srcC[s] < 1 || j.srcOff[s] < 0 || j.srcOff[s] + j.srcC[s] > j.cin_full) return FS_ERR_ARG;
   }
   for (int i0 = 0; i0 < njobs; i0 += PACK_JOBS) {
@@ -177,6 +185,17 @@
     hipLaunchKernelGGL(pack_jobs_kernel, dim3(blocks, n), dim3(256), 0, stream, tab);
   }
   return fs_launch_status();
+}
+
+extern "C" int fsraft_s2d_live_blocks(int C, int* taps, int* chunks, int cap) {
+  const int n = s2d_live_count(C);
+  for (int i = 0; i < n && i < cap; ++i) {
+    int t = 0, c = 0;
+    s2d_live_block(C, i, t, c);
+    if (taps) taps[i] = t;
+    if (chunks) chunks[i] = c;
+  }
+  return n;
 }
 
 extern "C" int fsraft_pack_conv_weight(float* w_oihw, float* wpk, int Cout, int Cin, int KH, int KW, const int* srcC,
diff --git a/flow_supervisor_amd/csrc/conv_patch.inc b/flow_supervisor_amd/csrc/conv_patch.inc
--- a/flow_supervisor_amd/csrc/conv_patch.inc
+++ b/flow_supervisor_amd/csrc/conv_patch.inc
@@ -11,8 +11,9 @@
 
 template <int EPI, int KH, int KW, int PT_TH, int BN = PT_BN>
 __global__ __launch_bounds__(PT_TH * 64) void conv_patch_kernel(const PatchArgs args) {
-  constexpr int PT_NT = PT_TH * 64, TN = BN / 64;
-  using PCfg = SplitCfg<PT_TH * 32, BN, PT_TH / 2, 2, 2, true, PT_NT>;
+  constexpr bool W81 = BN == 96;
+  constexpr int PT_NT = PT_TH * 64, WNW = W81 ? 1 : 2, TM = W81 ? 1 : 2, TN = BN / (32 * WNW);
+  using PCfg = SplitCfg<PT_TH * 32, BN, PT_TH / TM, WNW, 2, true, PT_NT>;
   constexpr int TAPS = KH * KW, PHh = KH / 2, PWh = KW / 2;
   constexpr int PH = PT_TH + KH - 1, PW = PT_TW + KW - 1, ROWS = PH * PW;
   constexpr int PPITCH = 144;
@@ -22,7 +23,7 @@
   __shared__ __attribute__((aligned(16))) char lds[RING > EPI_BYTES ? RING : EPI_BYTES];
   const ConvArgs& a = args.a;
   const int lane = threadIdx.x & 63, wave = __builtin_amdgcn_readfirstlane((int)(threadIdx.x >> 6));
-  const int wm = wave >> 1, wn = wave & 1, l31 = lane & 31, lh = lane >> 5;
+  const int wm = wave / WNW, wn = wave % WNW, l31 = lane & 31, lh = lane >> 5;
   const int n0 = blockIdx.x * BN;
   const int tile = blockIdx.y, tpi = args.tx * ((a.H + PT_TH - 1) / PT_TH);
   const int b = tile / tpi, trem = tile % tpi;
@@ -40,12 +41,13 @@
     const bool ok = row < ROWS && (unsigned)y < (unsigned)a.H && (unsigned)x < (unsigned)a.W;
     ppix[j] = ok ? (unsigned)((b * a.H + y) * a.W + x) : 0x7fffffffu;
   }
-  constexpr int NCHW = BN * 8 / PT_NT;
+  constexpr int NCHW = (BN * 8 + PT_NT - 1) / PT_NT;
+  constexpr bool W_RAGGED = BN * 8 % PT_NT != 0;
   unsigned vbw[NCHW];
 #pragma unroll
   for (int j = 0; j < NCHW; ++j) {
     const int e = threadIdx.x + PT_NT * j;
-    vbw[j] = (e >> 3) < a.N - n0 ? (unsigned)((e >> 3) * a.Ktot * 4 + (e & 7) * 16) : FS_OOB;
+    vbw[j] = ((e >> 3) < a.N - n0 && (e >> 3) < BN) ? (unsigned)((e >> 3) * a.Ktot * 4 + (e & 7) * 16) : FS_OOB;
   }
   const char* wbase = uni_ptr(reinterpret_cast<const char*>(a.wpk) + (int64_t)n0 * a.Ktot * 4);
 
@@ -92,12 +94,13 @@
   };
   auto stage_w = [&](char* bt) {
 #pragma unroll
-    for (int j = 0; j < NCHW; ++j) stage_copy<128>(bt, threadIdx.x + PT_NT * j, rw + 4 * j);
-  };
-
-  f32x16 acc[2][TN];
-#pragma unroll
-  for (int i = 0; i < 2; ++i)
+    for (int j = 0; j < NCHW; ++j)
+      if (!W_RAGGED || ((threadIdx.x + PT_NT * j) >> 3) < BN) stage_copy<128>(bt, threadIdx.x + PT_NT * j, rw + 4 * j);
+  };
+
+  f32x16 acc[TM][TN];
+#pragma unroll
+  for (int i = 0; i < TM; ++i)
 #pragma unroll
     for (int j = 0; j < TN; ++j)
 #pragma unroll
@@ -107,15 +110,15 @@
   char* bt0 = lds + 2 * PT_PLANE;
   char* bt1 = bt0 + BN * 128;
 
-  const int rb = wn * (BN / 2) + l31;
-  const int la_off = (2 * wm * PW + l31) * PPITCH + lh * 16;
+  const int rb = wn * (BN / WNW) + l31;
+  const int la_off = (TM * wm * PW + l31) * PPITCH + lh * 16;
   auto compute = [&](const char* plane, const char* bt, int dy, int dx) {
     const char* Bs = bt + rb * 128;
 #pragma unroll
     for (int s = 0; s < 2; ++s) {
-      bf16x8 ah[2], al[2], bh[TN], bl[TN];
-#pragma unroll
-      for (int mt = 0; mt < 2; ++mt) {
+      bf16x8 ah[TM], al[TM], bh[TN], bl[TN];
+#pragma unroll
+      for (int mt = 0; mt < TM; ++mt) {
         ah[mt] = *reinterpret_cast<const bf16x8*>(plane + la_off + ((dy + mt) * PW + dx) * PPITCH + (2 * s) * 16);
         al[mt] = *reinterpret_cast<const bf16x8*>(plane + la_off + ((dy + mt) * PW + dx) * PPITCH + (4 + 2 * s) * 16);
       }
@@ -126,15 +129,15 @@
         bl[nt] = *reinterpret_cast<const bf16x8*>(Bs + nt * 32 * 128 + obl);
       }
 #pragma unroll
-      for (int mt = 0; mt < 2; ++mt)
+      for (int mt = 0; mt < TM; ++mt)
 #pragma unroll
         for (int nt = 0; nt < TN; ++nt) acc[mt][nt] = __builtin_amdgcn_mfma_f32_32x32x16_bf16(al[mt], bh[nt], acc[mt][nt], 0, 0, 0);
 #pragma unroll
-      for (int mt = 0; mt < 2; ++mt)
+      for (int mt = 0; mt < TM; ++mt)
 #pragma unroll
         for (int nt = 0; nt < TN; ++nt) acc[mt][nt] = __builtin_amdgcn_mfma_f32_32x32x16_bf16(ah[mt], bl[nt], acc[mt][nt], 0, 0, 0);
 #pragma unroll
-      for (int mt = 0; mt < 2; ++mt)
+      for (int mt = 0; mt < TM; ++mt)
 #pragma unroll
         for (int nt = 0; nt < TN; ++nt) acc[mt][nt] = __builtin_amdgcn_mfma_f32_32x32x16_bf16(ah[mt], bh[nt], acc[mt][nt], 0, 0, 0);
     }
@@ -183,6 +186,7 @@
 template <int KH, int KW, int TH>
 int launch_conv_patch_t(const PatchArgs& p, int epi, dim3 grid, hipStream_t s) {
   t_route[0] = (TH == 8 ? 11 : 10) + (KH == 3 && KW == 3 && p.a.N <= 64 ? 2 : 0);
+  t_patch_cols = KH == 3 && KW == 3 && p.a.N <= 64 ? 64 : PT_BN;
   if constexpr (KH == 3 && KW == 3) {
     if (p.a.N <= 64) {
       hipLaunchKernelGGL((conv_patch_kernel<EPI_PLAIN, 3, 3, TH, 64>), grid, dim3(TH * 64), 0, s, p);
@@ -219,6 +223,12 @@
   const int bn = a.N <= 64 ? 64 : PT_BN;
   if (bn == 64 && !(k33 && epi == EPI_PLAIN)) return -1;
   const int64_t wg8 = (int64_t)ceil_div(a.N, bn) * p.tx * ceil_div(a.H, 8) * a.B;
+  if (k33 && epi == EPI_PLAIN && a.N > 64 && a.N <= 96 && (knob.conv_patch96 == 2 || (knob.conv_patch96 == 1 && wg8 >= 200))) {
+    dim3 grid(1, p.tx * ceil_div(a.H, 8) * a.B);
+    t_route[0] = 11; t_patch_cols = 96;
+    hipLaunchKernelGGL((conv_patch_kernel<EPI_PLAIN, 3, 3, 8, 96>), grid, dim3(512), 0, s, p);
+    return fs_launch_status();
+  }
   if (bn == 64 && wg8 >= 200 && knob.conv_patch64 == 1) return -1;
   if (wg8 >= 200 && !(bn == 64 && knob.conv_patch64 == 2)) {
     dim3 grid(ceil_div(a.N, bn), p.tx * ceil_div(a.H, 8) * a.B);
diff --git a/flow_supervisor_amd/csrc/conv_tuning.hip b/flow_supervisor_amd/csrc/conv_tuning.hip
--- a/flow_supervisor_amd/csrc/conv_tuning.hip
+++ b/flow_supervisor_amd/csrc/conv_tuning.hip
@@ -55,6 +55,20 @@
   return k ? *k : INT_MIN;
 }
 
+extern "C" int fsraft_set_conv_live(int mode) {
+  if (mode < -1 || mode > 1) return -2;
+  const int before = knob.conv_live;
+  if (mode >= 0) knob.conv_live = mode;
+  return before;
+}
+
+extern "C" int fsraft_set_conv_patch96(int mode) {
+  if (mode < -1 || mode > 2) return -2;
+  const int before = knob.conv_patch96;
+  if (mode >= 0) knob.conv_patch96 = mode;
+  return before;
+}
+
 extern "C" int fsraft_conv_last_route(int which) {
   return which == 0 || which == 1 ? t_route[which] : -1;
 }
diff --git a/flow_supervisor_amd/ops.py b/flow_supervisor_amd/ops.py
--- a/flow_supervisor_amd/ops.py
+++ b/flow_supervisor_amd/ops.py
@@ -1032,7 +1032,7 @@
         self.keep.append(ws)
         return j
 
-    def pack(self, ws, srcC, mode, srcOff=None, kh=None, kw=None, cin_full=None, frag=False, s2d=False):
+    def pack(self, ws, srcC, mode, srcOff=None, kh=None, kw=None, cin_full=None, frag=False, s2d=False, live=False):
         w0 = ws[0]
         cin_full = w0.shape[1] if cin_full is None else cin_full
         kh = (2 if s2d else w0.shape[2]) if kh is None else kh
@@ -1045,7 +1045,12 @@
             rows, kt = sum(srcC), conv_ktot([cout], kh, kw)
         if frag:
             rows = (rows + 31) // 32 * 32
-        j = self._job(ws, cin_full, kh, kw, srcC, srcOff, mode, (1 if frag else 0) | (2 if s2d else 0))
+        if live:
+            n = s2d_live_blocks(cin_full)[0]
+            if not (s2d and mode in (0, 10) and not frag and n):
+                raise ValueError("PackPlan.pack: live needs a space-to-depth forward pack with C % 32 == 0")
+            kt = 32 * n
+        j = self._job(ws, cin_full, kh, kw, srcC, srcOff, mode, (1 if frag else 0) | (2 if s2d else 0) | (4 if live else 0))
         self.jobs.append((j, self.total, (rows, kt)))
         self.total += (rows * kt + 63) // 64 * 64
         return len(self.jobs) - 1
@@ -1087,6 +1092,20 @@
     L.check(_lib().fsraft_pack_conv_weights(arr, len(items), L.stream()), "unpack_conv_weights")
 
 
+def s2d_live_blocks(C):
+    n = _lib().fsraft_s2d_live_blocks(C, None, None, 0)
+    taps, chunks = (ctypes.c_int * max(n, 1))(), (ctypes.c_int * max(n, 1))()
+    _lib().fsraft_s2d_live_blocks(C, taps, chunks, n)
+    return n, [(taps[i], chunks[i]) for i in range(n)]
+
+
+def set_conv_live(mode):
+    before = _lib().fsraft_set_conv_live(int(mode))
+    if before < 0:
+        raise ValueError(f"set_conv_live: unknown mode {mode}")
+    return before
+
+
 def exact_mode():
     return _lib().fsraft_get_tuning(3) == 0
 
@@ -1175,7 +1194,7 @@
 
 
 def conv_forward(srcs, wpk, bias, B, H, W, KH, KW, N, dsts, relu=False, alpha=1.0, epi=0, h=None, z=None,
-                 aux1=None, aux2=None, hid=0, wpk_split=None, pre=None, wpk_frag=None, pad=None, stats=None):
+                 aux1=None, aux2=None, hid=0, wpk_split=None, pre=None, wpk_frag=None, pad=None, stats=None, wpk_live=None):
     d = L.ConvDesc()
     for i, v in enumerate(srcs):
         d.src[i] = v.ptr; d.srcC[i] = v.C; d.srcld[i] = v.ld
@@ -1183,6 +1202,7 @@
     d.wpk = wpk.data_ptr()
     d.wpk_split = wpk_split.data_ptr() if wpk_split is not None else None
     d.wpk_frag = wpk_frag.data_ptr() if wpk_frag is not None else None
+    d.wpk_live = wpk_live.data_ptr() if wpk_live is not None else None
     if pad is not None:
         d.pad_h1, d.pad_w1 = pad[0] + 1, pad[1] + 1
     d.bias = bias.data_ptr() if bias is not None else None
diff --git a/include/fsraft.h b/include/fsraft.h
--- a/include/fsraft.h
+++ b/include/fsraft.h
@@ -102,6 +102,7 @@
   const float* wpk_frag;
   int pad_h1, pad_w1;
   float* ws; int64_t ws_floats;
+  const float* wpk_live;
 } fsraft_conv_desc;
 
 int fsraft_conv_ktot(const int* srcC, int nsrc, int KH, int KW);
@@ -125,6 +126,7 @@
   float scale; int accumulate;
 } fsraft_pack_job;
 int fsraft_pack_conv_weights(const fsraft_pack_job* jobs, int njobs, hipStream_t stream);
+int fsraft_s2d_live_blocks(int C, int* taps, int* chunks, int cap);
 
 int fsraft_conv_small_fwd(const float* x, int ld, int C, const float* w_oihw, const float* bias, float* out, int64_t obs,
                           int64_t ocs, int64_t ops, int N, int B, int H, int W, int KH, int KW, hipStream_t stream);
diff --git a/include/fsraft_tuning.h b/include/fsraft_tuning.h
--- a/include/fsraft_tuning.h
+++ b/include/fsraft_tuning.h
@@ -40,6 +40,10 @@
 int fsraft_conv_last_route(int which);
 int fsraft_set_wgrad_wide(int mode);
 int fsraft_conv_wgrad_last_tile(void);
+int fsraft_set_conv_live(int mode);
+int fsraft_conv_last_live_tiles(void);
+int fsraft_set_conv_patch96(int mode);
+int fsraft_conv_last_patch_cols(void);
 int fsraft_set_build_split(int on);
 int fsraft_set_build_kernel(int which);
 int fsraft_set_lookup_policy(int aux);
```

After: 111.2 image-pairs/s (median of 6 runs). No clear change (+0.7%).
